# qcNPU/LifeLong-CLIP

Hardware: AMD Instinct MI355X
Metric: images/sec/GPU (ViT-B/16 fwd+bwd, bs=256) + online A_AUC on CIFAR-100 (higher is better)
Workload: dtype bf16

## Files before the change

### include/lc_clip.h

```cpp
#ifndef LC_CLIP_H
#define LC_CLIP_H
#include <hip/hip_runtime_api.h>
#include <stdint.h>

#ifdef __cplusplus
extern "C" {
#endif

#define LC_OK 0
#define LC_EINVAL (-1)
#define LC_ELAUNCH (-2)
#define LC_EUNSUPPORTED (-3)

#define LC_EPI_BF16 0
#define LC_EPI_F32 1
#define LC_EPI_RESID 2
#define LC_EPI_GELU 3
#define LC_EPI_GELU_BWD 4
#define LC_EPI_BF16_F32 5
#define LC_EPI_GELU_D 6
#define LC_EPI_MUL 7
#define LC_EPI_GELU_D_Q8 12
#define LC_EPI_MUL_Q8 13
#define LC_EPI_RESID16 14
// ... 133 lines not shown
                             long ldq, int row, const void* O_row, const void* dO_row, long ldo,
                             const float* lse_row, void* dqkv, long lddq, int causal);
int lc_attn_bwd_fp8(hipStream_t stream, int n_seq, int L, int H, const void* qkv, long ldq,
                    const void* O, const void* dO, long ldo, const float* lse, void* dqkv, long lddq,
                    void* q_scale, long q_rows, int causal);

int lc_train_transform(hipStream_t stream, int n, int C, int Hin, int Win, const float* x, int R,
                       int pad, int crop_i, int crop_j, int flip, const float* mean_host,
                       const float* std_host, int quantize, int layout, int patch, void* out);

int lc_autoaugment(hipStream_t stream, int n, int C, int H, int W, const float* x, float* out,
                   int n_ops, const int* codes, const float* params);

int lc_autoaugment_ws(hipStream_t stream, int n, int C, int H, int W, const float* x, float* out,
                      int n_ops, const int* codes, const float* params, void* ws, long ws_bytes);

int lc_cast_bf16(hipStream_t stream, long n, const float* src, void* dst);

int lc_merge_weight(hipStream_t stream, int N, int K, int r, const float* W, const float* A,
                    const float* B, float scaling, void* out, void* outT);

#define LC_CAST_MAX 64
int lc_cast_weights_bf16(hipStream_t stream, int n, const float* const* W, const int* N,
                         const int* K, void* const* out, void* const* outT);

int lc_merge_weights_bf16(hipStream_t stream, int n, const float* const* W, const float* const* A,
                          const float* const* B, const int* r, const float* scaling, const int* N,
                          const int* K, void* const* out, void* const* outT);

int lc_lora_grad(hipStream_t stream, int M, int N, int K, int r, const void* dY, long ldy,
                 const void* X, long ldx, const float* A, const float* B, float scaling,
                 float* dA, float* dB);

int lc_lora_grad_ws(hipStream_t stream, int M, int N, int K, int r, const void* dY, long ldy,
                    const void* X, long ldx, const void* apad, long lda, const void* btpad,
                    long ldbt, float scaling, float* dA, float* dB, void* ws, long ws_bytes);
int lc_lora_grad_ws_unscaled(hipStream_t stream, int M, int N, int K, int r, const void* dY,
                             long ldy, const void* X, long ldx, const void* apad, long lda,
                             const void* btpad, long ldbt, float scaling, float* dA, float* dB,
                             void* ws, long ws_bytes, const float* gscale);

int lc_adapter_fwd(hipStream_t stream, int M, int D, const void* z, long ldz, const void* Wd,
                   const float* bd, const void* Wu, const float* bu, float scale, float keep,
                   unsigned long long seed, const unsigned long long* seed_dev,
                   const float* resid, float* xout, long ldx, void* h);

int lc_adapter_ln_fwd(hipStream_t stream, int M, int D, const void* z, long ldz, const void* Wd,
                      const float* bd, const void* Wu, const float* bu, float scale, float keep,
                      unsigned long long seed, const unsigned long long* seed_dev,
                      const float* resid, float* xout, long ldx, void* hout,
                      const float* gamma, const float* beta, void* y, long ldy, float* mean,
                      float* rstd);

int lc_adapter_fwd_rows(hipStream_t stream, int M, int D, const void* z, long ldz, const void* Wd,
                        const float* bd, const void* Wu, const float* bu, float scale, float keep,
                        unsigned long long seed, const unsigned long long* seed_dev,
                        const float* resid, float* xout, long ldx, void* h, long row_mul,
                        long row_add);
int lc_adapter_ln_fwd_rows(hipStream_t stream, int M, int D, const void* z, long ldz,
                           const void* Wd, const float* bd, const void* Wu, const float* bu,
                           float scale, float keep, unsigned long long seed,
                           const unsigned long long* seed_dev, const float* resid, float* xout,
                           long ldx, void* hout, const float* gamma, const float* beta, void* y,
                           long ldy, float* mean, float* rstd, long row_mul, long row_add);
int lc_adapter_ln_fwd_rows_x16(hipStream_t stream, int M, int D, const void* z, long ldz,
                               const void* Wd, const float* bd, const void* Wu, const float* bu,
                               float scale, float keep, unsigned long long seed,
                               const unsigned long long* seed_dev, const void* resid, void* xout,
                               long ldx, void* hout, const float* gamma, const float* beta,
                               void* y, long ldy, float* mean, float* rstd, long row_mul,
                               long row_add);
int lc_adapter_fwd_rows_f16(hipStream_t stream, int M, int D, const void* z, long ldz,
                            const void* Wd, const float* bd, const void* Wu, const float* bu,
                            float scale, float keep, unsigned long long seed,
                            const unsigned long long* seed_dev, const float* resid, float* xout,
                            long ldx, void* h, long row_mul, long row_add);
int lc_adapter_ln_fwd_rows_f16(hipStream_t stream, int M, int D, const void* z, long ldz,
                               const void* Wd, const float* bd, const void* Wu, const float* bu,
                               float scale, float keep, unsigned long long seed,
                               const unsigned long long* seed_dev, const float* resid,
                               float* xout, long ldx, void* hout, const float* gamma,
                               const float* beta, void* y, long ldy, float* mean, float* rstd,
                               long row_mul, long row_add);

int lc_adapter_bwd(hipStream_t stream, int M, int D, const void* gout, long ldg, const void* h,
                   const void* WuT, const void* WdT, float scale, float keep, void* dpre,
                   void* dz, long ldz);

int lc_adapter_bwd_set_form(int fused);

int lc_adapter_wgrad(hipStream_t stream, int M, int D, const void* gout, long ldg, const void* h,
                     const void* z, long ldz, const void* dpre, float scale, float* dWu,
                     float* dbu, float* dWd, float* dbd);
int lc_adapter_wgrad_ws(hipStream_t stream, int M, int D, const void* gout, long ldg,
                        const void* h, const void* z, long ldz, const void* dpre, float scale,
                        float* dWu, float* dbu, float* dWd, float* dbd, void* ws, long ws_bytes);

int lc_check_finite(hipStream_t stream, long n, const float* g, int* flag);

int lc_adamw(hipStream_t stream, long n, float* p, const float* g, float* m, float* v, float lr,
             float b1, float b2, float eps, float wd, int step, const int* skip,
             const long long* step_dev);

int lc_counter_add(hipStream_t stream, int n, long long* ctr, long long delta);

int lc_adam_step_advance(hipStream_t stream, long long* ctr, const int* skip);

int lc_l2norm_rows(hipStream_t stream, int R, int E, const float* f, long ldf, float* out,
                   float* norms);

int lc_clip_head(hipStream_t stream, int B, int C, int E, const float* img_n, const float* txt_n,
                 const float* logit_scale, const int64_t* labels, float* probs, float* dlogits,
                 float* loss);

int lc_head_feat_grad(hipStream_t stream, int R, int Co, int E, const float* dlogits, long sr,
                      long sc, const float* other_n, const float* self_n, const float* norms,
                      const float* logit_scale, const float* dn_ext, float* dF);

int lc_head_logits(hipStream_t stream, int B, int C, int E, const float* img_n, const float* txt_n,
                   const float* logit_scale, float* logits, float* probs);

int lc_softmax_bwd_rows(hipStream_t stream, int B, int C, const float* probs, const float* dprobs,
                        float* dlogits);

int lc_grad_pow2_normalize(hipStream_t stream, long n, float* x, float* scale, int target_exp);

int lc_add_unscaled(hipStream_t stream, long n, float* y, const float* x, const float* scale);

int lc_device_cu_count(int device, int* n_cu);
int lc_stream_create_cumask(int device, int first, int count, int stride, void** stream);
int lc_stream_destroy(void* stream);

int lc_gemm_nt_f16(hipStream_t stream, int epi, int M, int N, int K, const void* A, long lda,
                   const void* B, long ldb, const float* bias, float alpha, void* out0, long ldo0,
                   void* out1, long ldo1, const void* aux, long ldaux);
int lc_gemm_nt_ws_f16(hipStream_t stream, int epi, int M, int N, int K, const void* A, long lda,
                      const void* B, long ldb, const float* bias, float alpha, void* out0, long ldo0,
                      void* out1, long ldo1, const void* aux, long ldaux, void* ws, long ws_bytes);
int lc_gemm_nt_rows_f16(hipStream_t stream, int epi, int n, int N, int K, const void* A, long lda,
                        const void* B, long ldb, const float* bias, float alpha, void* out,
                        long ldo, int M_full, long mul, long add, void* ws, long ws_bytes);
int lc_gemm_tn_f16(hipStream_t stream, int M, int N1, int N2, const void* A, long lda, const void* B,
                   long ldb, float alpha, float* C, long ldc, float* colsum, float colsum_scale);
int lc_gemm_tn_ws_f16(hipStream_t stream, int M, int N1, int N2, const void* A, long lda,
                      const void* B, long ldb, float alpha, float* C, long ldc, float* colsum,
                      float colsum_scale, void* ws, long ws_bytes);
int lc_gemm_set_tile_f16(int tile);
int lc_gemm_set_streamk_f16(int mode);
int lc_layernorm_fwd_f16(hipStream_t stream, int rows, int D, const float* x, long ldx,
                         const int* row_idx, const float* gamma, const float* beta, void* y,
                         int y_f32, long ldy, float* mean, float* rstd);
int lc_layernorm_bwd_f16(hipStream_t stream, int rows, int D, const void* dy, int dy_f32, long ldy,
                         const float* x, long ldx, const float* mean, const float* rstd,
                         const float* gamma, const float* dres, float* dx, void* dx_bf16, long ldo,
                         const int* row_idx);
int lc_attn_fwd_f16(hipStream_t stream, int n_seq, int L, int H, const void* qkv, long ldq, void* O,
                    long ldo, float* lse, int causal);
int lc_attn_bwd_f16(hipStream_t stream, int n_seq, int L, int H, const void* qkv, long ldq,
                    const void* O, const void* dO, long ldo, const float* lse, void* dqkv, long lddq,
                    int causal);
int lc_attn_bwd_set_form_f16(int form);
int lc_cast_bf16_f16(hipStream_t stream, long n, const float* src, void* dst);
int lc_merge_weight_f16(hipStream_t stream, int N, int K, int r, const float* W, const float* A,
                        const float* B, float scaling, void* out, void* outT);
int lc_cast_weights_bf16_f16(hipStream_t stream, int n, const float* const* W, const int* N,
                             const int* K, void* const* out, void* const* outT);
int lc_merge_weights_bf16_f16(hipStream_t stream, int n, const float* const* W, const float* const* A,
                              const float* const* B, const int* r, const float* scaling, const int* N,
                              const int* K, void* const* out, void* const* outT);
int lc_lora_grad_f16(hipStream_t stream, int M, int N, int K, int r, const void* dY, long ldy,
                     const void* X, long ldx, const float* A, const float* B, float scaling,
                     float* dA, float* dB);
int lc_lora_grad_ws_f16(hipStream_t stream, int M, int N, int K, int r, const void* dY, long ldy,
                        const void* X, long ldx, const void* apad, long lda, const void* btpad,
                        long ldbt, float scaling, float* dA, float* dB, void* ws, long ws_bytes);
int lc_adapter_fwd_f16(hipStream_t stream, int M, int D, const void* z, long ldz, const void* Wd,
                       const float* bd, const void* Wu, const float* bu, float scale, float keep,
                       unsigned long long seed, const unsigned long long* seed_dev,
                       const float* resid, float* xout, long ldx, void* h);
// ... 74 lines not shown
```

### lifelong-clip_amd/csrc/gemm.hip

```cpp
#include "lc_common.h"
#include <stdlib.h>
#include <type_traits>

namespace {

constexpr int BK = 64;

template <int... Es>
struct EpiList {};
template <int... Es>
constexpr bool epi_in(EpiList<Es...>, int epi) { return ((epi == Es) || ...); }
template <class F, int... Es>
int dispatch_epi(EpiList<Es...>, int epi, F&& f) {
  int rc = LC_EINVAL;
  (void)((epi == Es && (rc = f(std::integral_constant<int, Es>{}), true)) || ...);
  return rc;
}

LC_DEV int swz(int row, int chunk) { return chunk ^ ((row >> 1) & 7); }

LC_DEV void tile_coords(int tile, int tiles_m, int tiles_n, int gm, int& tm, int& tn) {
  if (gm <= 1) {
    tm = tile / tiles_n;
    tn = tile % tiles_n;
// ... 157 lines not shown
      ep.q_scale[fp8_scale_index(m, n >> 5, ep.q_rows)] = (uint8_t)byte;
    }
  };
  auto bfv = [](const uint32_t* x, int i) { return bf2f((i & 1) ? (x[i >> 1] >> 16) : (x[i >> 1] & 0xffff)); };
  auto hfv = [](const uint32_t* x, int i) { return h2f((i & 1) ? (x[i >> 1] >> 16) : (x[i >> 1] & 0xffff)); };
  if constexpr (AUXF || AUXB) prefetch(0, 0);
  uint64_t seed = ep.seed;
  if constexpr (EPI == EPI_AD_DOWN)
    if (ep.seed_dev) seed += *ep.seed_dev * 0xD1B54A32D192ED03ull;
  const long row_mul = ep.row_mul ? ep.row_mul : 1;
#pragma unroll
  for (int pass = 0; pass < WT_M / PASS; ++pass) {
#pragma unroll
    for (int ii = 0; ii < PASS / 16; ++ii)
#pragma unroll
      for (int j = 0; j < TN; ++j)
        *reinterpret_cast<f32x4*>(stg + (ii * 16 + (lane & 15)) * LSTR + j * 16 + (lane >> 4) * 4) =
            acc[pass * (PASS / 16) + ii][j];
    if constexpr (AUXF || AUXB)
      if (pass + 1 < WT_M / PASS) prefetch(pass + 1, (pass + 1) & 1);
#pragma unroll
    for (int it = 0; it < NIT; ++it) {
      const int lr = it * RPI + lane / LPR;
      const long m = m0 + wm * WT_M + pass * PASS + lr;
      float v[CPL];
#pragma unroll
      for (int q = 0; q < NQ; ++q) {
        const f32x4 a4 = *reinterpret_cast<const f32x4*>(stg + lr * LSTR + lc + 4 * q);
#pragma unroll
        for (int r = 0; r < 4; ++r) v[4 * q + r] = epi_affine(a4[r], alpha, bb[4 * q + r]);
      }
      const float* xf = pf_f[pass & 1][it];
      const uint32_t* xb = pf_b[pass & 1][it];
#if defined(G8_NOSTORE) && G8_NOSTORE == 2
      if (ep.dbg == nullptr) continue;
#endif
      float w[CPL];
      if constexpr (EPI == EPI_BF16 || EPI == EPI_BF16_F32) {
        store_bf(rs0, ldo0, m, v);
        if constexpr (EPI == EPI_BF16_F32) store_f(rs1, ldo1, m, v);
      } else if constexpr (EPI == EPI_F32) {
        store_f(rs0, ldo0, m, v);
      } else if constexpr (EPI == EPI_RESID) {
#pragma unroll
        for (int i = 0; i < CPL; ++i) w[i] = xf[i] + v[i];
        store_f(rs0, ldo0, m, w);
      } else if constexpr (EPI == EPI_RESID16) {
        static_assert(CPL == 8, "8 halves (16 B) per lane");
#pragma unroll
        for (int i = 0; i < CPL; ++i) w[i] = hfv(xb, i) + v[i];
        __builtin_amdgcn_raw_buffer_store_b128(
            lc_u32x4{pack2h(w[0], w[1]), pack2h(w[2], w[3]), pack2h(w[4], w[5]), pack2h(w[6], w[7])},
            rs0, (int)(((m - m0) * ldo0 + n) * 2), 0, 0);
      } else if constexpr (EPI == EPI_GELU) {
        store_bf(rs0, ldo0, m, v);
#pragma unroll
        for (int i = 0; i < CPL; ++i) w[i] = quick_gelu(v[i]);
        store_bf(rs1, ldo1, m, w);
      } else if constexpr (EPI == EPI_GELU_BWD) {
#pragma unroll
        for (int i = 0; i < CPL; ++i) w[i] = v[i] * quick_gelu_grad(bfv(xb, i));
        store_bf(rs0, ldo0, m, w);
      } else if constexpr (EPI == EPI_GELU_D || EPI == EPI_GELU_D_Q8) {
#pragma unroll
        for (int i = 0; i < CPL; ++i) {
          const float sg = lc_sigmoid1702(v[i]);
          w[i] = v[i] * sg;
          v[i] = sg * __builtin_fmaf(1.702f * v[i], 1.0f - sg, 1.0f);
        }
        store_bf(rs0, ldo0, m, v);
        if constexpr (EPI == EPI_GELU_D_Q8)
          store_q8(out1, ldo1, m, w);
        else
          store_bf(rs1, ldo1, m, w);
      } else if constexpr (EPI == EPI_MUL || EPI == EPI_MUL_Q8) {
#pragma unroll
        for (int i = 0; i < CPL; ++i) w[i] = v[i] * bfv(xb, i);
        if constexpr (EPI == EPI_MUL_Q8)
          store_q8(out1, ldo1, m, w);
        else
          store_bf(rs0, ldo0, m, w);
      } else if constexpr (EPI == EPI_AD_DOWN) {
#pragma unroll
        for (int i = 0; i < CPL; ++i) w[i] = fmaxf(v[i], 0.f) * drop_mul(seed, m * row_mul + ep.row_add, n + i, ep.keep);
        store_bf(rs0, ldo0, m, w);
      } else if constexpr (EPI == EPI_AD_UP) {
#pragma unroll
        for (int i = 0; i < CPL; ++i) w[i] = xf[i] + bfv(xb, i) + ep.scale * v[i];
        store_f(rs0, ldo0, m, w);
      } else if constexpr (EPI == EPI_AD_MASK) {
        const float inv = 1.0f / ep.keep;
#pragma unroll
        for (int i = 0; i < CPL; ++i) w[i] = bfv(xb, i) > 0.f ? v[i] * inv : 0.f;
        store_bf(rs0, ldo0, m, w);
      } else if constexpr (EPI == EPI_AD_ADD) {
#pragma unroll
        for (int i = 0; i < CPL; ++i) w[i] = bfv(xb, i) + v[i];
        store_bf(rs0, ldo0, m, w);
      }
    }
  }
}

template <int BM, int BN, int WM, int WN, int STAGES, int EPI>
__global__ void __launch_bounds__(64 * WM * WN, (WM * WN == 4 ? 2 : 1))
gemm_nt_kernel(int M, int N, int K, const bf16_t* __restrict__ A, long lda,
               const bf16_t* __restrict__ B, long ldb, const float* __restrict__ bias,
               float alpha, void* __restrict__ out0, long ldo0, void* __restrict__ out1,
               long ldo1, const void* __restrict__ aux, long ldaux, EpiParams ep) {
  constexpr int NW = WM * WN;
  constexpr int TM = BM / WM / 16;
  constexpr int TN = BN / WN / 16;
  constexpr int STAGE_BYTES = (BM + BN) * 128;
  constexpr int LOADS = (BM + BN) / 8 / NW;
  constexpr int PASS_MAX = STAGES == 1 ? 16 : 32;
  constexpr int EPI_BYTES = NW * ((BM / WM) % PASS_MAX == 0 ? PASS_MAX : 16) * (BN / WN + 4) * 4;
  constexpr int SMEM = STAGES * STAGE_BYTES > EPI_BYTES ? STAGES * STAGE_BYTES : EPI_BYTES;
  __shared__ __attribute__((aligned(16))) char smem[SMEM];

  const int tid = threadIdx.x, lane = tid & 63, wave = tid >> 6;
  const int wm = wave / WN, wn = wave % WN;

  const int tiles_n = N / BN;
  const int tiles_m = (M + BM - 1) / BM;
  const int nwg = tiles_m * tiles_n;
  int bid = blockIdx.x;
  {
    int q = nwg / 8, r = nwg % 8, x = bid % 8, loc = bid / 8;
    bid = (x < r ? x * (q + 1) : r * (q + 1) + (x - r) * q) + loc;
  }
  const int tm = bid / tiles_n, tn = bid % tiles_n;
  const int m0 = tm * BM, n0 = tn * BN;

  f32x4 acc[TM][TN];
#pragma unroll
  for (int i = 0; i < TM; ++i)
#pragma unroll
    for (int j = 0; j < TN; ++j) acc[i][j] = f32x4{0.f, 0.f, 0.f, 0.f};

  const int nk = K / BK;
  constexpr int IA = BM / 8 / NW, IB = BN / 8 / NW;
  static_assert(IA * 8 * NW == BM && IB * 8 * NW == BN, "tile rows must split evenly over the waves");
  const __amdgpu_buffer_rsrc_t rsA = lc_rsrc(A + (long)m0 * lda, (long)min(M - m0, BM) * lda * 2);
  const __amdgpu_buffer_rsrc_t rsB = lc_rsrc(B + (long)n0 * ldb, (long)BN * ldb * 2);
  auto stage = [&](int buf, int kt) {
    char* s = smem + buf * STAGE_BYTES;
#pragma unroll
    for (int i = 0; i < IA; ++i) {
      const int r = (wave * IA + i) * 8 + (lane >> 3);
      __builtin_amdgcn_raw_ptr_buffer_load_lds(rsA, LDS_PTR(s + (wave * IA + i) * 1024), 16,
                                               (uint32_t)(r * lda * 2 + swz(r, lane & 7) * 16),
                                               kt * BK * 2, 0, 0);
    }
#pragma unroll
    for (int i = 0; i < IB; ++i) {
      const int r = (wave * IB + i) * 8 + (lane >> 3);
      __builtin_amdgcn_raw_ptr_buffer_load_lds(rsB, LDS_PTR(s + BM * 128 + (wave * IB + i) * 1024),
                                               16, (uint32_t)(r * ldb * 2 + swz(r, lane & 7) * 16),
                                               kt * BK * 2, 0, 0);
    }
  };

  auto compute = [&](const char* sa) {
    const char* sb = sa + BM * 128;
#pragma unroll
    for (int ks = 0; ks < 2; ++ks) {
      const int chunk = ks * 4 + (lane >> 4);
// ... 899 lines not shown
    if (do_cs) {
      const bf16_t* col = reinterpret_cast<const bf16_t*>(sa) + (tid & 63);
#pragma unroll
      for (int i = 0; i < 16; ++i) cs += bf2f(col[((tid >> 6) + 4 * i) * 64]);
    }
    const int g = lane >> 4, t = lane & 15;
#pragma unroll
    for (int ks = 0; ks < 2; ++ks) {
      bf16x8 fa[2], fb[2];
#pragma unroll
      for (int i = 0; i < 2; ++i) {
        const int row = ks * 32 + g * 8 + (t >> 2);
        const int cola = wa * 32 + i * 16 + (t & 3) * 4;
        bf16x4 lo = tr_read(sa, row, cola), hi = tr_read(sa, row + 4, cola);
        fa[i] = bf16x8{lo[0], lo[1], lo[2], lo[3], hi[0], hi[1], hi[2], hi[3]};
        const int colb = wb * 32 + i * 16 + (t & 3) * 4;
        bf16x4 lo2 = tr_read(sb, row, colb), hi2 = tr_read(sb, row + 4, colb);
        fb[i] = bf16x8{lo2[0], lo2[1], lo2[2], lo2[3], hi2[0], hi2[1], hi2[2], hi2[3]};
      }
#pragma unroll
      for (int i = 0; i < 2; ++i)
#pragma unroll
        for (int j = 0; j < 2; ++j) acc[i][j] = mfma16(fa[i], fb[j], acc[i][j]);
    }
    asm volatile("s_waitcnt vmcnt(0)" ::: "memory");
    __syncthreads();
  }
  if (do_cs) {
    red[tid] = cs;
    __syncthreads();
    if (tid < 64 && c1 + tid < N1)
      atomicAdd(colsum + c1 + tid, colsum_scale * (red[tid] + red[tid + 64] + red[tid + 128] + red[tid + 192]));
  }
  const int g = lane >> 4, t = lane & 15;
#pragma unroll
  for (int i = 0; i < 2; ++i)
#pragma unroll
    for (int j = 0; j < 2; ++j)
#pragma unroll
      for (int r = 0; r < 4; ++r) {
        const int n1 = c1 + wa * 32 + i * 16 + g * 4 + r;
        const int n2 = c2 + wb * 32 + j * 16 + t;
        if (n1 < N1 && n2 < N2) atomicAdd(C + (long)n1 * ldc + n2, acc[i][j][r] * alpha);
      }
}

struct TnProb {
  const bf16_t* W;
  long ldw;
  const bf16_t* S;
  long lds;
  float* C;
  long ldc;
  int Nw, ns, trans;
  float alpha;
  float* cs_w;
  float cs_w_scale;
  float* cs_s;
  float cs_s_scale;
  int M, n_chunks, n_tiles, wgs;
  float* part;
  int pw;
  const float* div;
  int w16;
};
LC_DEV float tn_unscale(const TnProb& p, float v) { return p.div ? v / *p.div : v; }

template <int PW>
struct TnGeom {
  static constexpr int ROWB = PW * 2;
  static constexpr int WB = 64 * ROWB;
  static constexpr int SLOT = WB + 64 * 128;
#ifndef TNW256_STAGES
#define TNW256_STAGES 3
#endif
  static constexpr int STAGES = PW == 256 ? TNW256_STAGES : 5;
  static constexpr int WPW = WB / 1024 / 8;
  static constexpr int LOADS = WPW + 1;
  static constexpr int TI = PW / 64;
};

__host__ __device__ inline int tn_pslot(int pw) { return pw * 64 + pw + 64; }

template <int PW>
__global__ void __launch_bounds__(512, 1)
gemm_tn_wide_kernel(TnProb p0, TnProb p1) {
  using Geo = TnGeom<PW>;
  constexpr int STAGES = Geo::STAGES, SLOT = Geo::SLOT, LOADS = Geo::LOADS, TI = Geo::TI;
  constexpr int ROWB = Geo::ROWB, LPRW = ROWB / 16, RPP = 64 / LPRW;
  constexpr int PSLOT = PW * 64 + PW + 64;
  __shared__ __attribute__((aligned(16))) char smem[STAGES * SLOT];
  const bool second = (int)blockIdx.x >= p0.wgs;
  const TnProb& p = second ? p1 : p0;
  const int bid = second ? blockIdx.x - p0.wgs : blockIdx.x;
  const int tid = threadIdx.x, lane = tid & 63;
  const int wave = __builtin_amdgcn_readfirstlane(tid >> 6);
  const int wn = wave & 3, wsv = wave >> 2;
  const int g = lane >> 4, t = lane & 15;
  const int tile = bid % p.n_tiles, cidx = bid / p.n_tiles;
  const int nblk = (p.M + 63) / 64;
  float* slot = p.part ? p.part + (long)(tile * p.n_chunks + cidx) * PSLOT : nullptr;
  if (cidx >= nblk) {
    if (slot)
      for (int e = tid; e < PSLOT; e += 512) slot[e] = 0.f;
    return;
  }
  const int nsteps = (nblk - 1 - cidx) / p.n_chunks + 1;
  auto blk_row = [&](int s) { return (cidx + s * p.n_chunks) * 64; };
  const int nw_pad = (p.Nw + 63) & ~63;
  const bool do_csw = p.cs_w != nullptr && wsv == 0;
  const bool do_css = p.cs_s != nullptr && tile == 0 && wn == 0;

  auto dma = [&](int s) {
    char* sl = smem + (s % STAGES) * SLOT;
    const int r0 = blk_row(s);
#pragma unroll
    for (int i = 0; i < Geo::WPW; ++i) {
      const int piece = wave * Geo::WPW + i;
      const int lr = piece * RPP + lane / LPRW;
      const int pc = lane % LPRW;
      const int c = (((pc >> 1) ^ swz_w(lr)) << 1) | (pc & 1);
      const int r = min(r0 + lr, p.M - 1);
      int col = tile * PW + c * 8;
      col = col < nw_pad ? col : col - 64;
      glds16(p.W + (long)r * p.ldw + col, sl + piece * 1024);
    }
    {
      const int piece = wave;
      const int lr = piece * 8 + (lane >> 3);
      const int pc = lane & 7;
      const int c = (((pc >> 1) ^ swz_s(lr)) << 1) | (pc & 1);
      const int r = min(r0 + lr, p.M - 1);
      glds16(p.S + (long)r * p.lds + c * 8, sl + Geo::WB + piece * 1024);
    }
  };

  f32x4 acc[TI][2], csw[TI], css[2];
#pragma unroll
  for (int i = 0; i < TI; ++i) {
    csw[i] = f32x4{0.f, 0.f, 0.f, 0.f};
#pragma unroll
    for (int j = 0; j < 2; ++j) acc[i][j] = f32x4{0.f, 0.f, 0.f, 0.f};
  }
  css[0] = css[1] = f32x4{0.f, 0.f, 0.f, 0.f};
  const short one = LC_ONE16;

#pragma unroll
  for (int s = 0; s < STAGES - 1; ++s)
    if (s < nsteps) dma(s);
  for (int s = 0; s < nsteps; ++s) {
    const int ahead = min(nsteps - 1 - s, STAGES - 2);
    if (STAGES > 4 && ahead >= 3) wait_vmcnt<3 * LOADS>();
    else if (STAGES > 3 && ahead == 2) wait_vmcnt<2 * LOADS>();
    else if (ahead >= 1) wait_vmcnt<LOADS>();
    else wait_vmcnt<0>();
    lds_barrier();
    if (s + STAGES - 1 < nsteps) dma(s + STAGES - 1);
    const uint32_t sw = lds_addr(smem + (s % STAGES) * SLOT);
    const uint32_t ss = sw + Geo::WB;
    const int valid = p.M - blk_row(s);
    bf16x8 fwk[2][TI], fsk[2][2];
#pragma unroll
    for (int ks = 0; ks < 2; ++ks) {
      const int row = ks * 32 + g * 8 + (t >> 2);
#pragma unroll
      for (int i = 0; i < TI; ++i)
        fwk[ks][i] = tr_frag_asm<ROWB>(sw, row, wn * (PW / 4) + i * 16 + (t & 3) * 4);
#pragma unroll
      for (int j = 0; j < 2; ++j)
        fsk[ks][j] = tr_frag_asm<128>(ss, row, wsv * 32 + j * 16 + (t & 3) * 4);
    }
    lds_wait0();
    if (p.w16) {
#pragma unroll
      for (int ks = 0; ks < 2; ++ks)
#pragma unroll
        for (int i = 0; i < TI; ++i) fwk[ks][i] = h2s8(fwk[ks][i]);
    }
#pragma unroll
    for (int ks = 0; ks < 2; ++ks) {
      const int kb = ks * 32 + g * 8;
      bf16x8* fw = fwk[ks];
      bf16x8* fs = fsk[ks];
      bf16x8 ones;
#pragma unroll
      for (int e = 0; e < 8; ++e) ones[e] = (kb + e < valid) ? one : (short)0;
      if (valid < 64) {
#pragma unroll
        for (int j = 0; j < 2; ++j)
#pragma unroll
          for (int e = 0; e < 8; ++e) fs[j][e] = (kb + e < valid) ? fs[j][e] : (short)0;
      }
#pragma unroll
      for (int i = 0; i < TI; ++i) {
#pragma unroll
        for (int j = 0; j < 2; ++j) acc[i][j] = mfma16(fw[i], fs[j], acc[i][j]);
        if (do_csw) csw[i] = mfma16(fw[i], ones, csw[i]);
      }
      if (do_css) {
#pragma unroll
        for (int j = 0; j < 2; ++j) css[j] = mfma16(ones, fs[j], css[j]);
      }
    }
  }
  if (slot) {
#pragma unroll
    for (int i = 0; i < TI; ++i)
#pragma unroll
      for (int r = 0; r < 4; ++r) {
        const int nl = wn * (PW / 4) + i * 16 + g * 4 + r;
#pragma unroll
        for (int jj = 0; jj < 2; ++jj) slot[nl * 64 + wsv * 32 + jj * 16 + t] = acc[i][jj][r];
        if (wsv == 0 && t == 0) slot[PW * 64 + nl] = do_csw ? csw[i][r] : 0.f;
      }
    if (wn == 0 && g == 0)
#pragma unroll
// ... 7 lines not shown
    for (int r = 0; r < 4; ++r) {
      const int n = tile * PW + wn * (PW / 4) + i * 16 + g * 4 + r;
      if (n >= p.Nw) continue;
#pragma unroll
      for (int jj = 0; jj < 2; ++jj) {
        const int j = wsv * 32 + jj * 16 + t;
        if (j < p.ns) {
          float* dst = p.trans ? p.C + (long)j * p.ldc + n : p.C + (long)n * p.ldc + j;
          atomicAdd(dst, tn_unscale(p, acc[i][jj][r] * p.alpha));
        }
      }
      if (do_csw && t == 0) atomicAdd(p.cs_w + n, tn_unscale(p, csw[i][r] * p.cs_w_scale));
    }
  if (do_css && g == 0) {
#pragma unroll
    for (int jj = 0; jj < 2; ++jj) {
      const int j = wsv * 32 + jj * 16 + t;
      if (j < p.ns) atomicAdd(p.cs_s + j, tn_unscale(p, css[jj][0] * p.cs_s_scale));
    }
  }
}

LC_DEV float sum_slots(const float* __restrict__ src, int n, long ps) {
  float v = 0.f;
  int c = 0;
  for (; c + 8 <= n; c += 8) {
    float t[8];
#pragma unroll
    for (int i = 0; i < 8; ++i) t[i] = src[(c + i) * ps];
    v += ((t[0] + t[1]) + (t[2] + t[3])) + ((t[4] + t[5]) + (t[6] + t[7]));
  }
  for (; c < n; ++c) v += src[c * ps];
  return v;
}

__global__ void __launch_bounds__(256)
tn_reduce_kernel(TnProb p0, TnProb p1) {
  const int np0 = p0.Nw * 64 + p0.Nw + 64;
  const int np1 = p1.part ? p1.Nw * 64 + p1.Nw + 64 : 0;
  for (int e = blockIdx.x * 256 + threadIdx.x; e < np0 + np1; e += gridDim.x * 256) {
    const bool second = e >= np0;
    const TnProb& p = second ? p1 : p0;
    const int k = second ? e - np0 : e;
    const int pw = p.pw;
    const long ps = tn_pslot(pw);
    if (k < p.Nw * 64) {
      const int n = k / 64, j = k % 64;
      if (j >= p.ns) continue;
      const int tile = n / pw, nl = n % pw;
      const float v = sum_slots(p.part + (long)tile * p.n_chunks * ps + nl * 64 + j, p.n_chunks, ps);
      float* dst = p.trans ? p.C + (long)j * p.ldc + n : p.C + (long)n * p.ldc + j;
      *dst += tn_unscale(p, v * p.alpha);
    } else if (k < p.Nw * 64 + p.Nw) {
      if (!p.cs_w) continue;
      const int n = k - p.Nw * 64, tile = n / pw, nl = n % pw;
      const float v = sum_slots(p.part + (long)tile * p.n_chunks * ps + pw * 64 + nl, p.n_chunks, ps);
      p.cs_w[n] += tn_unscale(p, v * p.cs_w_scale);
    } else {
      const int j = k - p.Nw * 64 - p.Nw;
      if (!p.cs_s || j >= p.ns) continue;
      const float v = sum_slots(p.part + pw * 64 + pw + j, p.n_chunks, ps);
      p.cs_s[j] += tn_unscale(p, v * p.cs_s_scale);
    }
  }
}

int cu_count();

void plan_tn(TnProb& p, int total_panels) {
  static int walkers = -1;
  if (walkers < 0) {
    const char* e = lc_diag_env("LC_TN_WALKERS");
    walkers = e ? atoi(e) : 0;
  }
  const int cus = walkers > 0 ? walkers : cu_count();
  const int nblk = (p.M + 63) / 64;
  int chunks = cus / total_panels;
  chunks = chunks < 1 ? 1 : chunks;
  chunks = chunks > nblk / 4 ? (nblk / 4 > 0 ? nblk / 4 : 1) : chunks;
  p.n_chunks = chunks;
  p.wgs = p.n_tiles * chunks;
}

int launch_tn_wide(hipStream_t stream, const TnProb& a, const TnProb& b) {
  const dim3 grid(a.wgs + b.wgs), block(512);
  if (a.pw == 256) hipLaunchKernelGGL(gemm_tn_wide_kernel<256>, grid, block, 0, stream, a, b);
  else hipLaunchKernelGGL(gemm_tn_wide_kernel<128>, grid, block, 0, stream, a, b);
  if (a.part) {
    const int outs = a.Nw * 64 + a.Nw + 64 + (b.part ? b.Nw * 64 + b.Nw + 64 : 0);
    hipLaunchKernelGGL(tn_reduce_kernel, dim3((outs + 255) / 256), dim3(256), 0, stream, a, b);
  }
  LC_LAUNCH_RET();
}

template <class AT, class Kern, class... Tail>
int launch(Kern kern, int grid, int block, const GemmArgs& g, long es, const EpiParams& ep,
           const Tail&... tail) {
  hipLaunchKernelGGL(kern, dim3(grid), dim3(block), 0, g.stream, g.M, g.N, g.K,
                     static_cast<const AT*>(g.A), g.lda * es, static_cast<const AT*>(g.B),
                     g.ldb * es, g.bias, g.alpha, g.out0, g.ldo0, g.out1, g.ldo1, g.aux, g.ldaux,
                     ep, tail...);
  LC_LAUNCH_RET();
}

template <int BM, int BN, int WM, int WN, int STAGES>
int launch_nt(const GemmArgs& g) {
  const int tiles = ((g.M + BM - 1) / BM) * (g.N / BN);
  return dispatch_epi(NtEpis{}, g.epi, [&](auto E) {
    return launch<bf16_t>(gemm_nt_kernel<BM, BN, WM, WN, STAGES, E()>, tiles, 64 * WM * WN, g, 1,
                          g.ep);
  });
}

int g_split_mode = -1;

int cu_count() {
  static int cus[64] = {0};
  int dev = 0;
  if (hipGetDevice(&dev) != hipSuccess || dev < 0 || dev >= 64) return 256;
  if (cus[dev] == 0) {
    int n = 0;
    if (hipDeviceGetAttribute(&n, hipDeviceAttributeMultiprocessorCount, dev) != hipSuccess || n <= 0)
      n = 256;
    cus[dev] = n;
  }
  return cus[dev];
}

SplitK plan_split(int tiles, int units, int min_units, void* ws, long ws_bytes, int per_cu = 1,
                  long slab_floats = 256 * 256) {
  SplitK sk{tiles, 1, nullptr, nullptr};
  if (g_split_mode < 0) {
    const char* e = lc_diag_env("LC_GEMM_SPLITK");
    g_split_mode = e ? atoi(e) : 1;
  }
  if (!g_split_mode || ws == nullptr) return sk;
  const int cus = cu_count() * per_cu;
  const int rem = tiles % cus;
  if (tiles < cus || rem == 0 || rem > cus / 2) return sk;
  int S = cus / rem;
  S = S > 4 ? 4 : S;
  if (S > units / min_units) S = units / min_units;
  if (S < 2) return sk;
  const long tick_bytes = LC_SPLITK_TICKET_BYTES;
  if ((long)rem * 4 > tick_bytes || tick_bytes + (long)rem * S * slab_floats * 4 > ws_bytes) return sk;
  sk.dp_tiles = tiles - rem;
  sk.splits = S;
  sk.tickets = static_cast<int*>(ws);
  sk.slabs = reinterpret_cast<float*>(static_cast<char*>(ws) + tick_bytes);
  return sk;
}

int g_sk_mode = 0;
bool plan_sk(int tiles, int units, void* ws, long ws_bytes, SplitK& sk, int& G, int panels = 0) {
  G = panels > 0 ? panels : cu_count();
  if (panels > 0 && tiles % panels == 0 && ws != nullptr) {
    sk.dp_tiles = 0;
    sk.splits = 1;
    sk.tickets = static_cast<int*>(ws);
    sk.slabs = reinterpret_cast<float*>(static_cast<char*>(ws) + LC_SPLITK_TICKET_BYTES);
    return true;
  }
  if (ws == nullptr || tiles <= G || tiles % G == 0) return false;
  if ((long)tiles * units / G < units) return false;
  if ((long)(G - 1) * 4 > LC_SPLITK_TICKET_BYTES ||
      LC_SPLITK_TICKET_BYTES + (long)(G - 1) * 256 * 256 * 4 > ws_bytes)
    return false;
  sk.dp_tiles = 0;
  sk.splits = 1;
  sk.tickets = static_cast<int*>(ws);
// ... 364 lines not shown
             aux, ldaux, default_epi(), ws, ws_bytes,
             Fp8Scales{static_cast<const uint8_t*>(sa), static_cast<const uint8_t*>(sb), sa_rows,
                       sb_rows}};
  if (int rc = check_launch(g)) return rc;
  g.ep.q_scale = q8 ? static_cast<uint8_t*>(q_scale) : nullptr;
  g.ep.q_rows = q_rows;
  return launch_g8<true>(
      g, Route{PATH_G8, false, false, g8_plan<true>(M, N, K, ws, ws_bytes), group_m(N), 0});
}

int lc_gemm_set_tile(int tile) {
  LC_CHECK_ARG(tile >= 0 && tile <= 11);
  g_force_tile = tile;
  return LC_OK;
}

int lc_gemm_set_streamk(int mode) {
  LC_CHECK_ARG(mode >= 0 && mode <= 4);
  g_sk_mode = mode;
  return LC_OK;
}

int lc_gemm_tn(hipStream_t stream, int M, int N1, int N2, const void* A, long lda, const void* B,
               long ldb, float alpha, float* C, long ldc, float* colsum, float colsum_scale) {
  return lc_gemm_tn_ws(stream, M, N1, N2, A, lda, B, ldb, alpha, C, ldc, colsum, colsum_scale,
                       nullptr, 0);
}

int lc_gemm_tn_ws(hipStream_t stream, int M, int N1, int N2, const void* A, long lda,
                  const void* B, long ldb, float alpha, float* C, long ldc, float* colsum,
                  float colsum_scale, void* ws, long ws_bytes) {
  LC_CHECK_ARG(M > 0 && N1 > 0 && N2 > 0);
  LC_CHECK_ARG(lda % 8 == 0 && ldb % 8 == 0 && lda >= (N1 + 63) / 64 * 64 &&
               ldb >= (N2 + 63) / 64 * 64 && ldc >= N2);
  if (N1 <= 64 || N2 <= 64) {
    const bool a_wide = N2 <= 64;
    TnProb p{};
    p.W = static_cast<const bf16_t*>(a_wide ? A : B);
    p.ldw = a_wide ? lda : ldb;
    p.S = static_cast<const bf16_t*>(a_wide ? B : A);
    p.lds = a_wide ? ldb : lda;
    p.C = C;
    p.ldc = ldc;
    p.Nw = a_wide ? N1 : N2;
    p.ns = a_wide ? N2 : N1;
    p.trans = a_wide ? 0 : 1;
    p.alpha = alpha;
    p.cs_w = a_wide ? colsum : nullptr;
    p.cs_w_scale = colsum_scale;
    p.cs_s = a_wide ? nullptr : colsum;
    p.cs_s_scale = colsum_scale;
    p.M = M;
    const bool wide = ws != nullptr && p.Nw % 256 == 0;
    p.pw = wide ? 256 : 128;
    p.n_tiles = (p.Nw + p.pw - 1) / p.pw;
    plan_tn(p, p.n_tiles);
    if (wide && ws_bytes >= LC_SPLITK_TICKET_BYTES + (long)p.wgs * tn_pslot(p.pw) * 4)
      p.part = reinterpret_cast<float*>(static_cast<char*>(ws) + LC_SPLITK_TICKET_BYTES);
    return launch_tn_wide(stream, p, TnProb{});
  }
  const int tiles = ((N1 + 63) / 64) * ((N2 + 63) / 64);
  int splits = (1024 + tiles - 1) / tiles;
  int chunk = (M + splits - 1) / splits;
  chunk = ((chunk + 63) / 64) * 64;
  if (chunk < 256) chunk = 256;
  splits = (M + chunk - 1) / chunk;
  dim3 grid(tiles, splits), block(256);
  hipLaunchKernelGGL(gemm_tn_kernel, grid, block, 0, stream, M, N1, N2, chunk,
                     static_cast<const bf16_t*>(A), lda, static_cast<const bf16_t*>(B), ldb, alpha,
                     C, ldc, colsum, colsum_scale);
  LC_LAUNCH_RET();
}

int lc_adapter_wgrad(hipStream_t stream, int M, int D, const void* gout, long ldg, const void* h,
                     const void* z, long ldz, const void* dpre, float scale, float* dWu,
                     float* dbu, float* dWd, float* dbd) {
  return lc_adapter_wgrad_ws(stream, M, D, gout, ldg, h, z, ldz, dpre, scale, dWu, dbu, dWd, dbd,
                             nullptr, 0);
}

static int adapter_wgrad(hipStream_t stream, int M, int D, const void* gout, long ldg,
                         const void* h, const void* z, long ldz, const void* dpre, float scale,
                         float* dWu, float* dbu, float* dWd, float* dbd, void* ws, long ws_bytes,
                         const float* div, int g16 = 0) {
  LC_CHECK_ARG(M > 0 && D > 0 && D % 64 == 0 && ldg % 8 == 0 && ldz % 8 == 0 && ldg >= D &&
               ldz >= D);
  LC_CHECK_ARG(dWu != nullptr && dWd != nullptr);
  TnProb up{}, down{};
  up.div = down.div = div;
  up.W = static_cast<const bf16_t*>(gout);
  up.w16 = g16;
  up.ldw = ldg;
  up.S = static_cast<const bf16_t*>(h);
  up.lds = 64;
  up.C = dWu;
  up.ldc = 64;
  up.Nw = D;
  up.ns = 64;
  up.trans = 0;
  up.alpha = scale;
  up.cs_w = dbu;
  up.cs_w_scale = scale;
  const int pw = D % 256 == 0 ? 256 : 128;
  up.pw = pw;
  up.M = M;
  up.n_tiles = (D + pw - 1) / pw;
  down.W = static_cast<const bf16_t*>(z);
  down.ldw = ldz;
  down.S = static_cast<const bf16_t*>(dpre);
  down.lds = 64;
  down.C = dWd;
  down.ldc = D;
  down.Nw = D;
  down.ns = 64;
  down.trans = 1;
  down.alpha = 1.0f;
  down.cs_s = dbd;
  down.cs_s_scale = 1.0f;
  down.pw = pw;
  down.M = M;
  down.n_tiles = (D + pw - 1) / pw;
  plan_tn(up, 2 * up.n_tiles);
  plan_tn(down, 2 * down.n_tiles);
#ifdef LC_DIAG_SKIP_WGRAD
  return LC_OK;
#endif
  const long need = (long)(up.wgs + down.wgs) * tn_pslot(pw) * 4;
  if (ws != nullptr && ws_bytes >= LC_SPLITK_TICKET_BYTES + need) {
    up.part = reinterpret_cast<float*>(static_cast<char*>(ws) + LC_SPLITK_TICKET_BYTES);
    down.part = up.part + (long)up.wgs * tn_pslot(pw);
  }
  return launch_tn_wide(stream, up, down);
}

int lc_adapter_wgrad_ws(hipStream_t stream, int M, int D, const void* gout, long ldg,
                        const void* h, const void* z, long ldz, const void* dpre, float scale,
                        float* dWu, float* dbu, float* dWd, float* dbd, void* ws, long ws_bytes) {
  return adapter_wgrad(stream, M, D, gout, ldg, h, z, ldz, dpre, scale, dWu, dbu, dWd, dbd, ws,
                       ws_bytes, nullptr);
}

#ifndef LC_F16
int lc_adapter_wgrad_ws_unscaled(hipStream_t stream, int M, int D, const void* gout, long ldg,
                                 const void* h, const void* z, long ldz, const void* dpre,
                                 float scale, float* dWu, float* dbu, float* dWd, float* dbd,
                                 void* ws, long ws_bytes, const float* gscale) {
  LC_CHECK_ARG(gscale != nullptr);
  return adapter_wgrad(stream, M, D, gout, ldg, h, z, ldz, dpre, scale, dWu, dbu, dWd, dbd, ws,
                       ws_bytes, gscale);
}

int lc_adapter_wgrad_ws_unscaled_g16(hipStream_t stream, int M, int D, const void* gout, long ldg,
                                     const void* h, const void* z, long ldz, const void* dpre,
                                     float scale, float* dWu, float* dbu, float* dWd, float* dbd,
                                     void* ws, long ws_bytes, const float* gscale) {
  LC_CHECK_ARG(gscale != nullptr);
  return adapter_wgrad(stream, M, D, gout, ldg, h, z, ldz, dpre, scale, dWu, dbu, dWd, dbd, ws,
                       ws_bytes, gscale, 1);
}
#endif

}
```

### lifelong-clip_amd/csrc/lc_common.h

```cpp
#pragma once
#include <hip/hip_runtime.h>
#include <stdint.h>
#include <stdlib.h>
#include "lc_clip.h"

inline const char* lc_diag_env(const char* name) {
#ifdef LC_DIAG_ENV
  return getenv(name);
#else
  (void)name;
  return nullptr;
#endif
}

typedef uint16_t bf16_t;
typedef short bf16x8 __attribute__((ext_vector_type(8)));
typedef short bf16x4 __attribute__((ext_vector_type(4)));
typedef float f32x4 __attribute__((ext_vector_type(4)));
typedef int i32x4 __attribute__((ext_vector_type(4)));
typedef int i32x8 __attribute__((ext_vector_type(8)));

__device__ __forceinline__ void st_nt16(void* p, uint32_t a, uint32_t b, uint32_t c, uint32_t d) {
  __builtin_nontemporal_store(i32x4{(int)a, (int)b, (int)c, (int)d}, reinterpret_cast<i32x4*>(p));
}
// ... 30 lines not shown
  __bf16 b = (__bf16)f;
  return *reinterpret_cast<bf16_t*>(&b);
}
typedef __bf16 lc_bf16x2 __attribute__((ext_vector_type(2)));
LC_DEV uint32_t pack2bf(float lo, float hi) {
  return __builtin_bit_cast(uint32_t, __builtin_convertvector((lc_f32x2){lo, hi}, lc_bf16x2));
}

LC_DEV f32x4 mfma16(const bf16x8& a, const bf16x8& b, const f32x4& c) {
  return __builtin_amdgcn_mfma_f32_16x16x32_bf16(a, b, c, 0, 0, 0);
}
#define LC_MFMA16_ASM "v_mfma_f32_16x16x32_bf16"
#define LC_ONE16 ((short)0x3F80)
#endif

typedef _Float16 lc_h16x2 __attribute__((ext_vector_type(2)));
typedef _Float16 lc_h16x4 __attribute__((ext_vector_type(4)));
LC_DEV float h2f(uint16_t h) { return (float)__builtin_bit_cast(_Float16, h); }
LC_DEV uint32_t pack2h(float lo, float hi) {
  return __builtin_bit_cast(uint32_t, __builtin_convertvector((lc_f32x2){lo, hi}, lc_h16x2));
}
template <typename XT>
LC_DEV float xround(float v) {
  if constexpr (sizeof(XT) == 2) return (float)(_Float16)v;
  else return v;
}

LC_DEV void glds16(const void* gsrc, void* lds_wave_base) {
  __builtin_amdgcn_global_load_lds(GLB_PTR(gsrc), LDS_PTR(lds_wave_base), 16, 0, 0);
}
LC_DEV void glds4(const void* gsrc, void* lds_wave_base) {
  __builtin_amdgcn_global_load_lds(GLB_PTR(gsrc), LDS_PTR(lds_wave_base), 4, 0, 0);
}

LC_DEV float wave_sum(float v) {
#pragma unroll
  for (int o = 32; o > 0; o >>= 1) v += __shfl_xor(v, o);
  return v;
}
LC_DEV float wave_max(float v) {
#pragma unroll
  for (int o = 32; o > 0; o >>= 1) v = fmaxf(v, __shfl_xor(v, o));
  return v;
}

constexpr float LC_GELU_K2 = -1.702f * 1.4426950408889634f;
LC_DEV float lc_sigmoid1702(float x) {
  return __builtin_amdgcn_rcpf(1.0f + __builtin_amdgcn_exp2f(LC_GELU_K2 * x));
}
LC_DEV float quick_gelu(float x) { return x * lc_sigmoid1702(x); }
LC_DEV float quick_gelu_grad(float x) {
  const float s = lc_sigmoid1702(x);
  const float t = 1.702f * x;
  return s * __builtin_fmaf(t, 1.0f - s, 1.0f);
}

LC_DEV uint32_t lc_hash(uint64_t seed, uint64_t idx) {
  uint64_t z = seed + 0x9E3779B97F4A7C15ull * (idx + 1);
  z = (z ^ (z >> 30)) * 0xBF58476D1CE4E5B9ull;
  z = (z ^ (z >> 27)) * 0x94D049BB133111EBull;
  z ^= z >> 31;
  return (uint32_t)(z >> 32);
}

LC_DEV float drop_mul(uint64_t seed, long m, int j, float keep) {
  if (keep >= 1.0f) return 1.0f;
  const uint32_t hsh = lc_hash(seed, (uint64_t)m * 64 + j);
  const float u = (hsh >> 8) * (1.0f / 16777216.0f);
  return u < keep ? 1.0f / keep : 0.0f;
}

struct EpiParams {
  const void* aux2;
  long ldaux2;
  float scale;
  float keep;
  uint64_t seed;
  unsigned long long* dbg;
  const unsigned long long* seed_dev;
  uint8_t* q_scale;
  long q_rows;
  int group_m;
  long row_mul, row_add;
};

struct Fp8Scales {
  const uint8_t* sa;
  const uint8_t* sb;
  long sa_rows, sb_rows;
};

LC_DEV uint32_t lc_amax_bits(uint32_t acc, float x) {
  const uint32_t b = __float_as_uint(x) & 0x7fffffffu;
  return acc > b ? acc : b;
}
LC_DEV uint32_t e8m0_of_bits(uint32_t amax_bits) {
  const int e = (int)(amax_bits >> 23);
  if (e == 0) return 0;
  if (e == 255) return 0xFF;
  const int b = e - 8;
  return (uint32_t)(b < 1 ? 1 : (b > 253 ? 253 : b));
}
LC_DEV uint32_t e8m0_of(float amax) { return e8m0_of_bits(__float_as_uint(amax) & 0x7fffffffu); }
LC_DEV float e8m0_inv(uint32_t byte) {
  if (byte == 0) return 0.f;
  if (byte == 0xFF) return __uint_as_float(0x7fc00000u);
  return __uint_as_float((uint32_t)(254 - byte) << 23);
}
LC_DEV uint32_t pack4_fp8(float a, float b, float c, float d) {
  const bool nan = (__float_as_uint(a) & 0x7fffffffu) > 0x7f800000u;
  a = fminf(fmaxf(a, -448.f), 448.f);
  b = fminf(fmaxf(b, -448.f), 448.f);
  c = fminf(fmaxf(c, -448.f), 448.f);
  d = fminf(fmaxf(d, -448.f), 448.f);
  uint32_t r = __builtin_amdgcn_cvt_pk_fp8_f32(a, b, 0, false);
  r = __builtin_amdgcn_cvt_pk_fp8_f32(c, d, r, true);
  return nan ? 0x7f7f7f7fu : r;
}

LC_DEV int swz_w(int r) { return (r & 3) | ((r >> 1) & 4); }
LC_DEV int swz_s(int r) { return ((r >> 1) & 1) | ((r >> 2) & 2); }

template <int ROWB>
LC_DEV bf16x8 tr_frag(const char* lds, int row, int col) {
  auto addr = [&](int r) {
    const int byte = col * 2;
    const int u = (byte >> 5) ^ (ROWB >= 256 ? swz_w(r) : swz_s(r));
    return lds + r * ROWB + u * 32 + (byte & 31);
  };
  const bf16x4 lo = __builtin_amdgcn_ds_read_tr16_b64_v4i16(
      (__attribute__((address_space(3))) bf16x4*)addr(row));
  const bf16x4 hi = __builtin_amdgcn_ds_read_tr16_b64_v4i16(
      (__attribute__((address_space(3))) bf16x4*)addr(row + 4));
  return bf16x8{lo[0], lo[1], lo[2], lo[3], hi[0], hi[1], hi[2], hi[3]};
}

LC_DEV __amdgpu_buffer_rsrc_t lc_rsrc(const void* p, long bytes) {
  const uint64_t a = (uint64_t)p;
  const uint32_t lo = __builtin_amdgcn_readfirstlane((uint32_t)a);
  const uint32_t hi = __builtin_amdgcn_readfirstlane((uint32_t)(a >> 32));
  const int n = __builtin_amdgcn_readfirstlane((int)bytes);
  return __builtin_amdgcn_make_buffer_rsrc((void*)(((uint64_t)hi << 32) | lo), 0, n, 0x00020000);
}
typedef unsigned int lc_u32x4 __attribute__((ext_vector_type(4)));
typedef unsigned int lc_u32x2 __attribute__((ext_vector_type(2)));

LC_DEV bf16x8 h2s8(bf16x8 v) {
#ifdef LC_F16
  return v;
#else
  const lc_u32x4 u = __builtin_bit_cast(lc_u32x4, v);
  const lc_f32x2 f0 = __builtin_convertvector(__builtin_bit_cast(lc_h16x2, (uint32_t)u.x), lc_f32x2);
  const lc_f32x2 f1 = __builtin_convertvector(__builtin_bit_cast(lc_h16x2, (uint32_t)u.y), lc_f32x2);
  const lc_f32x2 f2 = __builtin_convertvector(__builtin_bit_cast(lc_h16x2, (uint32_t)u.z), lc_f32x2);
  const lc_f32x2 f3 = __builtin_convertvector(__builtin_bit_cast(lc_h16x2, (uint32_t)u.w), lc_f32x2);
  return __builtin_bit_cast(bf16x8, (lc_u32x4{pack2bf(f0.x, f0.y), pack2bf(f1.x, f1.y),
                                              pack2bf(f2.x, f2.y), pack2bf(f3.x, f3.y)}));
#endif
}
LC_DEV bf16x8 b2h8(bf16x8 v) {
  const lc_u32x4 u = __builtin_bit_cast(lc_u32x4, v);
  auto cv = [](uint32_t w) {
    return pack2h(__uint_as_float(w << 16), __uint_as_float(w & 0xffff0000u));
  };
  return __builtin_bit_cast(bf16x8, (lc_u32x4{cv(u.x), cv(u.y), cv(u.z), cv(u.w)}));
}
LC_DEV f32x4 mfma16_h(const bf16x8& a, const bf16x8& b, const f32x4& c) {
// ... 85 lines not shown
```

### lifelong-clip_amd/csrc/lc_f16_names.h

```cpp
#pragma once
#define lc_attn_fwd lc_attn_fwd_f16
#define lc_attn_bwd_fp8 lc_attn_bwd_fp8_f16
#define lc_attn_bwd lc_attn_bwd_f16
#define lc_attn_bwd_set_form lc_attn_bwd_set_form_f16
#define lc_attn_row_fwd lc_attn_row_fwd_f16
#define lc_attn_row_bwd lc_attn_row_bwd_f16
#define lc_attn_bwd_live_row lc_attn_bwd_live_row_f16
#define lc_gemm_nt_ex lc_gemm_nt_ex_f16
#define lc_gemm_nt lc_gemm_nt_f16
#define lc_gemm_nt_ws lc_gemm_nt_ws_f16
#define lc_gemm_nt_rows lc_gemm_nt_rows_f16
#define lc_gemm_split_plan lc_gemm_split_plan_f16
#define lc_gemm_set_debug lc_gemm_set_debug_f16
#define lc_gemm_nt_fp8 lc_gemm_nt_fp8_f16
#define lc_gemm_set_tile lc_gemm_set_tile_f16
#define lc_gemm_set_streamk lc_gemm_set_streamk_f16
#define lc_gemm_tn lc_gemm_tn_f16
#define lc_gemm_tn_ws lc_gemm_tn_ws_f16
#define lc_adapter_wgrad lc_adapter_wgrad_f16
#define lc_adapter_wgrad_ws lc_adapter_wgrad_ws_f16
#define lc_layernorm_fwd lc_layernorm_fwd_f16
#define lc_layernorm_fwd_fp8 lc_layernorm_fwd_fp8_f16
#define lc_layernorm_bwd lc_layernorm_bwd_f16
#define lc_layernorm_bwd_fp8 lc_layernorm_bwd_fp8_f16
#define lc_patchify lc_patchify_f16
#define lc_vit_assemble lc_vit_assemble_f16
#define lc_vit_embed_ln lc_vit_embed_ln_f16
#define lc_text_embed lc_text_embed_f16
#define lc_eot_rows lc_eot_rows_f16
#define lc_cast_bf16 lc_cast_bf16_f16
#define lc_merge_weight lc_merge_weight_f16
#define lc_cast_weights_bf16 lc_cast_weights_bf16_f16
#define lc_merge_weights_bf16 lc_merge_weights_bf16_f16
#define lc_lora_grad lc_lora_grad_f16
#define lc_lora_grad_ws lc_lora_grad_ws_f16
#define lc_adapter_fwd lc_adapter_fwd_f16
#define lc_adapter_ln_fwd lc_adapter_ln_fwd_f16
#define lc_adapter_fwd_rows lc_adapter_fwd_rows_f16
#define lc_adapter_ln_fwd_rows lc_adapter_ln_fwd_rows_f16
#define lc_adapter_bwd_set_form lc_adapter_bwd_set_form_f16
#define lc_adapter_bwd lc_adapter_bwd_f16
#define lc_check_finite lc_check_finite_f16
#define lc_adamw lc_adamw_f16
#define lc_counter_add lc_counter_add_f16
#define lc_adam_step_advance lc_adam_step_advance_f16
```

### lifelong-clip_amd/csrc/peft.hip

```cpp
#include "lc_common.h"
#include <stdlib.h>

namespace {

__global__ void cast_bf16_kernel(long n, const float* __restrict__ src, bf16_t* __restrict__ dst) {
  for (long i = (blockIdx.x * (long)blockDim.x + threadIdx.x) * 4; i < n;
       i += (long)gridDim.x * blockDim.x * 4) {
    if (i + 3 < n) {
      const float4 v = *reinterpret_cast<const float4*>(src + i);
      *reinterpret_cast<uint2*>(dst + i) = uint2{pack2bf(v.x, v.y), pack2bf(v.z, v.w)};
    } else {
      for (long j = i; j < n; ++j) dst[j] = f2bf(src[j]);
    }
  }
}

constexpr int MERGE_RMAX = 8;
LC_DEV void merge_tile(int N, int K, int r, const float* __restrict__ W, const float* __restrict__ A,
                       const float* __restrict__ B, float s, bf16_t* __restrict__ out,
                       bf16_t* __restrict__ outT, int n0, int k0) {
  __shared__ float tile[64][65];
  __shared__ float As[MERGE_RMAX][64];
  __shared__ float Bs[64][MERGE_RMAX];
  const int tid = threadIdx.x;
// ... 686 lines not shown
  float* slot_p = part + (long)cidx * ((long)N * r + (long)r * K);
  if (t < r) {
#pragma unroll
    for (int c = 0; c < NC; ++c)
#pragma unroll
      for (int rr = 0; rr < 4; ++rr)
        slot_p[(c * 128 + wave * 16 + 4 * g + rr) * r + t] = accB[c][rr];
  }
#pragma unroll
  for (int j = 0; j < G::DAT; ++j)
#pragma unroll
    for (int rr = 0; rr < 4; ++rr)
      if (4 * g + rr < r)
        slot_p[(long)N * r + (4 * g + rr) * K + (wave * G::DAT + j) * 16 + t] = accA[j][rr];
}

__global__ void __launch_bounds__(256)
lora_reduce_kernel(const float* __restrict__ part, int walkers, long slot_floats, long nb,
                   float s, float* __restrict__ dA, float* __restrict__ dB,
                   const float* __restrict__ div) {
  __shared__ float red[8][33];
  const int lo = threadIdx.x & 31, wg = threadIdx.x >> 5;
  const long e = (long)blockIdx.x * 32 + lo;
  float v = 0.f;
  if (e < slot_floats) {
    int w = wg;
    for (; w + 56 < walkers; w += 64) {
      float q[8];
#pragma unroll
      for (int u = 0; u < 8; ++u) q[u] = part[(long)(w + 8 * u) * slot_floats + e];
      v += ((q[0] + q[1]) + (q[2] + q[3])) + ((q[4] + q[5]) + (q[6] + q[7]));
    }
    for (; w < walkers; w += 8) v += part[(long)w * slot_floats + e];
  }
  red[wg][lo] = v;
  __syncthreads();
  if (wg == 0 && e < slot_floats) {
    float tot = 0.f;
#pragma unroll
    for (int k = 0; k < 8; ++k) tot += red[k][lo];
    if (div) tot /= *div;
    if (e < nb) dB[e] += s * tot;
    else dA[e - nb] += s * tot;
  }
}


template <int D, int XB = 4>
struct AdLnLay {
  static constexpr int ZROW = D * 2;
  static constexpr int ZIMG = 16 * ZROW;
  static constexpr int ZP = ZIMG / 1024 / 8;
  static constexpr int XIMG = 16 * D * XB;
  static constexpr int XP = XIMG / 1024 / 8;
  static constexpr int Z_OFF = 0;
  static constexpr int X_OFF = ZIMG;
  static constexpr int PRM_OFF = X_OFF + 2 * XIMG;
  static constexpr int ST_OFF = PRM_OFF + (3 * D + 64) * 4;
  static constexpr int RED_OFF = ST_OFF + 2 * 8 * 16 * 4;
  static constexpr int H_OFF = RED_OFF + 16 * 64 * 4;
  static constexpr int YSTR = D * 2 + 16;
  static constexpr int Y_OFF = RED_OFF;
  static constexpr int BYTES = RED_OFF + (16 * YSTR > 16 * 64 * 6 ? 16 * YSTR : 16 * 64 * 6);
  static constexpr int KS = D / 32 / 2;
  static constexpr int NU = D / 8 / 16;
  static_assert(BYTES <= 160 * 1024, "LDS");
};

template <int N>
LC_DEV void vmcnt_le() {
  asm volatile("s_waitcnt vmcnt(%0)" ::"n"(N) : "memory");
}

template <int D, typename XT = float>
__global__ void __launch_bounds__(512, 1)
adapter_ln_fwd_kernel(int M, const bf16_t* __restrict__ z, long ldz, const bf16_t* __restrict__ Wd,
                      const float* __restrict__ bd, const bf16_t* __restrict__ Wu,
                      const float* __restrict__ bu, float scale, float keep, uint64_t seed,
                      const unsigned long long* __restrict__ seed_dev,
                      const XT* __restrict__ resid, XT* __restrict__ xout, long ldx,
                      bf16_t* __restrict__ hout, const float* __restrict__ gamma,
                      const float* __restrict__ beta, bf16_t* __restrict__ y, long ldy,
                      float* __restrict__ mean_out, float* __restrict__ rstd_out, long row_mul,
                      long row_add) {
  constexpr int XB = (int)sizeof(XT);
  using L = AdLnLay<D, XB>;
  constexpr int KS = L::KS, NU = L::NU;
  __shared__ __attribute__((aligned(16))) char smem[L::BYTES];
  const int tid = threadIdx.x, lane = tid & 63;
  const int wave = __builtin_amdgcn_readfirstlane(tid >> 6);
  const int g = lane >> 4, t = lane & 15;
  const int nd = wave & 3, kh = wave >> 2;
  const int nblk = (M + 15) / 16;
  if ((int)blockIdx.x >= nblk) return;
  if (seed_dev) seed += *seed_dev * 0xD1B54A32D192ED03ull;
  float* red = reinterpret_cast<float*>(smem + L::RED_OFF);
  bf16_t* hs = reinterpret_cast<bf16_t*>(smem + L::H_OFF);
  float* st = reinterpret_cast<float*>(smem + L::ST_OFF);
  float* prm = reinterpret_cast<float*>(smem + L::PRM_OFF);
  for (int e = tid; e < D; e += 512) {
    prm[e] = bu[e];
    prm[D + e] = gamma[e];
    prm[2 * D + e] = beta[e];
  }
  if (tid < 64) prm[3 * D + tid] = bd[tid];
  bf16x8 wdf[KS], wuf[NU][2];
#pragma unroll
  for (int k = 0; k < KS; ++k)
    asm volatile("global_load_dwordx4 %0, %1, off"
                 : "=v"(wdf[k])
                 : "v"(Wd + (long)(16 * nd + t) * D + (kh * KS + k) * 32 + 8 * g));
#pragma unroll
  for (int u = 0; u < NU; ++u)
#pragma unroll
    for (int k = 0; k < 2; ++k)
      asm volatile("global_load_dwordx4 %0, %1, off"
                   : "=v"(wuf[u][k])
                   : "v"(Wu + (long)(wave * (D / 8) + 16 * u + t) * 64 + 32 * k + 8 * g));
  asm volatile("s_waitcnt vmcnt(0)" ::: "memory");

  auto dma_z = [&](int b) {
    char* dst = smem + L::Z_OFF;
    const int r0 = b * 16;
#pragma unroll
    for (int pp = 0; pp < L::ZP; ++pp) {
      const int piece = wave * L::ZP + pp;
      const int idx = piece * 64 + lane;
      const int row = idx / (L::ZROW / 16), pc = idx % (L::ZROW / 16);
      const int c = (((pc >> 1) ^ swz_w(row)) << 1) | (pc & 1);
      const int m = min(r0 + row, M - 1);
      glds16(z + (long)m * ldz + c * 8, dst + piece * 1024);
    }
  };
  constexpr int EPC = 16 / XB;
  auto dma_x = [&](int b, int buf) {
    char* dst = smem + L::X_OFF + buf * L::XIMG;
#pragma unroll
    for (int pp = 0; pp < L::XP; ++pp) {
      const int piece = wave * L::XP + pp;
      const int idx = piece * 64 + lane;
      const int row = idx / (D / EPC), c = idx % (D / EPC);
      const int m = min(b * 16 + row, M - 1);
      glds16(resid + (long)m * ldx + c * EPC, dst + piece * 1024);
    }
  };
  const uint32_t lds0 = lds_addr(smem);
  auto zaddr = [&](int row, int byte) {
    const int u = (byte >> 5) ^ swz_w(row);
    return lds0 + L::Z_OFF + row * L::ZROW + u * 32 + (byte & 31);
  };
  constexpr int XPR = D * XB / 512;
#ifdef ADLN_KO
  constexpr int NST = ((ADLN_KO & 1) ? 0 : XPR) + ((ADLN_KO & 2) ? 0 : D / 256);
#else
  constexpr int NST = XPR + D / 256;
#endif
  const int tail = NST + (wave < 2 ? 1 : 0) + (wave == 0 ? 2 : 0);

  int b = blockIdx.x;
  dma_x(b, 0);
  dma_z(b);
  __syncthreads();
  bool prev_full = false;
#pragma unroll 1
  for (int k = 0; b < nblk; ++k, b += gridDim.x) {
    const int buf = k & 1;
    const int r0 = b * 16;
    if (prev_full) {
      if (tail == NST + 3) vmcnt_le<NST + 3>();
      else if (tail == NST + 1) vmcnt_le<NST + 1>();
      else vmcnt_le<NST>();
    } else {
      vmcnt_le<0>();
    }
    lds_barrier();
    const int bn = b + gridDim.x;
    if (bn < nblk) dma_x(bn, buf ^ 1);
    f32x4 pd = f32x4{0.f, 0.f, 0.f, 0.f};
    uint2 zz[NU];
    {
      constexpr int GK = KS / 2;
      bf16x8 za[KS];
#pragma unroll
      for (int ks = 0; ks < KS; ++ks)
        asm volatile("ds_read_b128 %0, %1"
                     : "=v"(za[ks]) : "v"(zaddr(t, ((kh * KS + ks) * 32 + 8 * g) * 2)));
#pragma unroll
      for (int u = 0; u < NU; ++u)
        asm volatile("ds_read_b64 %0, %1"
                     : "=v"(zz[u]) : "v"(zaddr(t, (wave * (D / 8) + 16 * u + 4 * g) * 2)));
      asm volatile("s_waitcnt lgkmcnt(%0)" ::"n"(NU + KS - GK) : "memory");
      __builtin_amdgcn_sched_barrier(0);
#pragma unroll
      for (int ks = 0; ks < GK; ++ks) pd = mfma16(za[ks], wdf[ks], pd);
      asm volatile("s_waitcnt lgkmcnt(%0)" ::"n"(NU) : "memory");
      __builtin_amdgcn_sched_barrier(0);
#pragma unroll
      for (int ks = GK; ks < KS; ++ks) pd = mfma16(za[ks], wdf[ks], pd);
    }
    if (kh == 1)
#pragma unroll
      for (int rr = 0; rr < 4; ++rr) red[(4 * g + rr) * 64 + 16 * nd + t] = pd[rr];
    lds_barrier();
    if (bn < nblk) dma_z(bn);
    if (kh == 0) {
      const int j = 16 * nd + t;
#pragma unroll
      for (int rr = 0; rr < 4; ++rr) {
        const int m = 4 * g + rr;
        float v = pd[rr] + red[m * 64 + j];
        v = fmaxf(v + prm[3 * D + j], 0.f) * drop_mul(seed, (long)(r0 + m) * row_mul + row_add, j, keep);
        hs[m * 64 + j] = f2bf(v);
      }
    }
    lds_barrier();
    const uint32_t hl = lds0 + L::H_OFF;
    if (wave < 2) {
      const int e = tid;
      uint4 v;
      asm volatile("ds_read_b128 %0, %1" : "=v"(v) : "v"(hl + e * 16));
      lds_wait0();
      if (r0 + (e >> 3) < M) *reinterpret_cast<uint4*>(hout + (long)r0 * 64 + e * 8) = v;
    }
    bf16x8 ha0, ha1;
    asm volatile("ds_read_b128 %0, %1" : "=v"(ha0) : "v"(hl + (t * 64 + 8 * g) * 2));
    asm volatile("ds_read_b128 %0, %1" : "=v"(ha1) : "v"(hl + (t * 64 + 32 + 8 * g) * 2));
    f32x4 xo[NU];
    float s1 = 0.f;
    f32x4 xr4[NU];
    uint2 xh4[NU];
#pragma unroll
    for (int u = 0; u < NU; ++u) {
      const int col = wave * (D / 8) + 16 * u + 4 * g;
      if constexpr (XB == 4)
        asm volatile("ds_read_b128 %0, %1"
                     : "=v"(xr4[u]) : "v"(lds0 + L::X_OFF + buf * L::XIMG + (t * D + col) * 4));
      else
        asm volatile("ds_read_b64 %0, %1"
                     : "=v"(xh4[u]) : "v"(lds0 + L::X_OFF + buf * L::XIMG + (t * D + col) * 2));
    }
    lds_wait0();
    if constexpr (XB == 2) {
#pragma unroll
      for (int u = 0; u < NU; ++u)
        xr4[u] = f32x4{h2f(xh4[u].x & 0xffff), h2f(xh4[u].x >> 16), h2f(xh4[u].y & 0xffff),
                       h2f(xh4[u].y >> 16)};
    }
#pragma unroll
    for (int u = 0; u < NU; ++u) {
      f32x4 acc = mfma16(wuf[u][0], ha0, f32x4{0.f, 0.f, 0.f, 0.f});
      acc = mfma16(wuf[u][1], ha1, acc);
      const int col = wave * (D / 8) + 16 * u + 4 * g;
      const float zf[4] = {bf2f(zz[u].x & 0xffff), bf2f(zz[u].x >> 16), bf2f(zz[u].y & 0xffff),
                           bf2f(zz[u].y >> 16)};
      const f32x4 xr = xr4[u];
#pragma unroll
      for (int rr = 0; rr < 4; ++rr) {
        const float v = acc[rr] + prm[col + rr];
        xo[u][rr] = xround<XT>(xr[rr] + zf[rr] + scale * v);
        s1 += xo[u][rr];
      }
    }
    s1 += __shfl_xor(s1, 16);
    s1 += __shfl_xor(s1, 32);
    if (g == 0) st[wave * 16 + t] = s1;
    lds_barrier();
    const bool live = r0 + t < M;
    const uint32_t xs = lds0 + L::X_OFF + buf * L::XIMG;
    const uint32_t ys = lds0 + L::Y_OFF;
    if constexpr (XB == 4) {
      static_assert((D / 32) % 8 == 0, "wave column block must be whole 128-B groups");
      const uint32_t xb = xs + t * D * 4 + wave * (D / 32) * 16;
      const uint32_t x0 = xb + ((g ^ t) & 7) * 16, x1 = xb + (((4 + g) ^ t) & 7) * 16 - 64;
#pragma unroll
      for (int u = 0; u < NU; ++u)
        asm volatile("ds_write_b128 %0, %1 offset:%2" ::"v"((u & 1) ? x1 : x0), "v"(xo[u]),
                     "n"(u * 64) : "memory");
    } else {
      const uint32_t xb = xs + t * D * 2 + (g & 1) * 8;
#pragma unroll
      for (int u = 0; u < NU; ++u) {
        const int c = wave * (D / 64) + 2 * u + (g >> 1);
        const uint32_t a = xb + ((c & ~7) | ((c ^ t) & 7)) * 16;
        asm volatile("ds_write_b64 %0, %1" ::"v"(a),
                     "v"(uint2{pack2h(xo[u][0], xo[u][1]), pack2h(xo[u][2], xo[u][3])}) : "memory");
      }
    }
    float mean = 0.f;
#pragma unroll
    for (int w = 0; w < 8; ++w) mean += st[w * 16 + t];
    mean *= 1.0f / D;
    float s2 = 0.f;
#pragma unroll
    for (int u = 0; u < NU; ++u)
// ... 129 lines not shown
    b.out[i] = static_cast<bf16_t*>(out[i]);
    b.outT[i] = static_cast<bf16_t*>(outT[i]);
    b.N[i] = N[i];
    b.K[i] = K[i];
    const int t = ((N[i] + 63) / 64) * ((K[i] + 63) / 64);
    tiles = t > tiles ? t : tiles;
  }
  hipLaunchKernelGGL(cast_batch_kernel, dim3(tiles, n), dim3(256), 0, st, b);
  LC_LAUNCH_RET();
}

int lc_lora_grad(hipStream_t st, int M, int N, int K, int r, const void* dY, long ldy,
                 const void* X, long ldx, const float* A, const float* B, float scaling,
                 float* dA, float* dB) {
  LC_CHECK_ARG(M > 0 && r == 4 && N <= 3072 && K <= 1024 && N > 0 && K > 0);
  const int groups = (M + 15) / 16;
  const int grid = groups < 512 ? groups : 512;
  if (N <= 1024)
    hipLaunchKernelGGL((lora_grad_kernel<4, 1024, 1024>), dim3(grid), dim3(256), 0, st, M, N, K,
                       (const bf16_t*)dY, ldy, (const bf16_t*)X, ldx, A, B, scaling, dA, dB);
  else
    hipLaunchKernelGGL((lora_grad_kernel<4, 3072, 1024>), dim3(grid), dim3(256), 0, st, M, N, K,
                       (const bf16_t*)dY, ldy, (const bf16_t*)X, ldx, A, B, scaling, dA, dB);
  LC_LAUNCH_RET();
}

static int lora_grad_ws(hipStream_t st, int M, int N, int K, int r, const void* dY, long ldy,
                        const void* X, long ldx, const void* apad, long lda, const void* btpad,
                        long ldbt, float scaling, float* dA, float* dB, void* ws, long ws_bytes,
                        const float* div) {
  LC_CHECK_ARG(M > 0 && r >= 1 && r <= 4 && dY && X && apad && btpad && dA && dB && ws);
  LC_CHECK_ARG(ldy % 8 == 0 && ldx % 8 == 0 && lda % 8 == 0 && ldbt % 8 == 0);
  LC_CHECK_ARG(ldy >= N && ldx >= K && lda >= K && ldbt >= N);
  const int nblk = (M + 31) / 32;
  int walkers = 0;
  {
    int dev = 0, cus = 256;
    if (hipGetDevice(&dev) != hipSuccess ||
        hipDeviceGetAttribute(&cus, hipDeviceAttributeMultiprocessorCount, dev) != hipSuccess)
      cus = 256;
    walkers = nblk < cus ? nblk : cus;
  }
  const long slot = (long)N * r + (long)r * K;
  LC_CHECK_ARG(ws_bytes >= LC_SPLITK_TICKET_BYTES + (long)walkers * slot * 4);
  float* part = reinterpret_cast<float*>(static_cast<char*>(ws) + LC_SPLITK_TICKET_BYTES);
#define LC_LG(KT, NC)                                                                           \
  if (K == KT * 32 && N == NC * 128) {                                                         \
    hipLaunchKernelGGL((lora_grad1p_kernel<KT, NC>), dim3(walkers), dim3(512), 0, st, M,        \
                       (const bf16_t*)X, ldx, (const bf16_t*)dY, ldy, (const bf16_t*)apad, lda, \
                       (const bf16_t*)btpad, ldbt, part, walkers, r);                          \
  } else
  LC_LG(24, 18) LC_LG(24, 6) LC_LG(16, 12) LC_LG(16, 4)
  { return LC_EINVAL; }
#undef LC_LG
  hipError_t e = hipGetLastError();
  if (e != hipSuccess) return LC_ELAUNCH;
  hipLaunchKernelGGL(lora_reduce_kernel, dim3((unsigned)((slot + 31) / 32)), dim3(256), 0, st,
                     part, walkers, slot, (long)N * r, scaling, dA, dB, div);
  LC_LAUNCH_RET();
}

int lc_lora_grad_ws(hipStream_t st, int M, int N, int K, int r, const void* dY, long ldy,
                    const void* X, long ldx, const void* apad, long lda, const void* btpad,
                    long ldbt, float scaling, float* dA, float* dB, void* ws, long ws_bytes) {
  return lora_grad_ws(st, M, N, K, r, dY, ldy, X, ldx, apad, lda, btpad, ldbt, scaling, dA, dB, ws,
                      ws_bytes, nullptr);
}

#ifndef LC_F16
int lc_lora_grad_ws_unscaled(hipStream_t st, int M, int N, int K, int r, const void* dY, long ldy,
                             const void* X, long ldx, const void* apad, long lda,
                             const void* btpad, long ldbt, float scaling, float* dA, float* dB,
                             void* ws, long ws_bytes, const float* gscale) {
  LC_CHECK_ARG(gscale != nullptr);
  return lora_grad_ws(st, M, N, K, r, dY, ldy, X, ldx, apad, lda, btpad, ldbt, scaling, dA, dB, ws,
                      ws_bytes, gscale);
}
#endif

static int adapter_fwd(hipStream_t st, int M, int D, const void* z, long ldz, const void* Wd,
                       const float* bd, const void* Wu, const float* bu, float scale, float keep,
                       unsigned long long seed, const unsigned long long* seed_dev,
                       const float* resid, float* xout, long ldx, void* hout, long row_mul,
                       long row_add) {
  LC_CHECK_ARG(M > 0 && D % 64 == 0 && ldz % 8 == 0 && ldx % 4 == 0);
  LC_CHECK_ARG(keep > 0.f && keep <= 1.f && row_mul >= 1 && row_add >= 0);
  EpiParams ep{z, ldz, scale, keep, (uint64_t)seed, nullptr, seed_dev};
  ep.row_mul = row_mul;
  ep.row_add = row_add;
  int rc = lc_gemm_nt_ex({st, EPI_AD_DOWN, M, AD_H, D, z, ldz, Wd, D, bd, 1.0f, hout, AD_H,
                          nullptr, 0, nullptr, 0, ep});
  if (rc) return rc;
  return lc_gemm_nt_ex({st, EPI_AD_UP, M, D, AD_H, hout, AD_H, Wu, AD_H, bu, 1.0f, xout, ldx,
                        nullptr, 0, resid, ldx, ep});
}

int lc_adapter_fwd(hipStream_t st, int M, int D, const void* z, long ldz, const void* Wd,
                   const float* bd, const void* Wu, const float* bu, float scale, float keep,
                   unsigned long long seed, const unsigned long long* seed_dev,
                   const float* resid, float* xout, long ldx, void* hout) {
  return adapter_fwd(st, M, D, z, ldz, Wd, bd, Wu, bu, scale, keep, seed, seed_dev, resid, xout,
                     ldx, hout, 1, 0);
}

int lc_adapter_fwd_rows(hipStream_t st, int M, int D, const void* z, long ldz, const void* Wd,
                        const float* bd, const void* Wu, const float* bu, float scale, float keep,
                        unsigned long long seed, const unsigned long long* seed_dev,
                        const float* resid, float* xout, long ldx, void* hout, long row_mul,
                        long row_add) {
  return adapter_fwd(st, M, D, z, ldz, Wd, bd, Wu, bu, scale, keep, seed, seed_dev, resid, xout,
                     ldx, hout, row_mul, row_add);
}

static int adapter_ln_fwd(hipStream_t st, int M, int D, const void* z, long ldz, const void* Wd,
                          const float* bd, const void* Wu, const float* bu, float scale,
                          float keep, unsigned long long seed,
                          const unsigned long long* seed_dev, const void* resid, void* xout,
                          long ldx, void* hout, const float* gamma, const float* beta, void* y,
                          long ldy, float* mean, float* rstd, int x16, long row_mul = 1,
                          long row_add = 0) {
  const int xb = x16 ? 2 : 4;
  LC_CHECK_ARG(row_mul >= 1 && row_add >= 0);
  LC_CHECK_ARG(M > 0 && (D == 768 || D == 512) && ldz % 8 == 0 && ldx % (16 / xb) == 0 &&
               ldy % 8 == 0);
  LC_CHECK_ARG(ldx < (1L << 24) && ldy < (1L << 24));
  LC_CHECK_ARG(((uintptr_t)xout & 15) == 0 && ((uintptr_t)y & 15) == 0 &&
               ((uintptr_t)resid & 15) == 0);
  LC_CHECK_ARG(ldz >= D && ldx >= D && ldy >= D && keep > 0.f && keep <= 1.f);
  LC_CHECK_ARG(z && Wd && bd && Wu && bu && resid && xout && hout && gamma && beta && y && mean && rstd);
  int dev = 0, cus = 256;
  if (hipGetDevice(&dev) != hipSuccess ||
      hipDeviceGetAttribute(&cus, hipDeviceAttributeMultiprocessorCount, dev) != hipSuccess)
    cus = 256;
  const int nblk = (M + 15) / 16;
  const int grid = nblk < cus ? nblk : cus;
#define LC_ALN(DD, XT)                                                                           \
  hipLaunchKernelGGL((adapter_ln_fwd_kernel<DD, XT>), dim3(grid), dim3(512), 0, st, M,           \
                     (const bf16_t*)z, ldz, (const bf16_t*)Wd, bd, (const bf16_t*)Wu, bu, scale,  \
                     keep, (uint64_t)seed, seed_dev, (const XT*)resid, (XT*)xout, ldx,           \
                     (bf16_t*)hout, gamma, beta, (bf16_t*)y, ldy, mean, rstd, row_mul, row_add)
  if (x16) {
    if (D == 768) LC_ALN(768, _Float16);
    else LC_ALN(512, _Float16);
  } else {
    if (D == 768) LC_ALN(768, float);
    else LC_ALN(512, float);
  }
#undef LC_ALN
  LC_LAUNCH_RET();
}

int lc_adapter_ln_fwd(hipStream_t st, int M, int D, const void* z, long ldz, const void* Wd,
                      const float* bd, const void* Wu, const float* bu, float scale, float keep,
                      unsigned long long seed, const unsigned long long* seed_dev,
                      const float* resid, float* xout, long ldx, void* hout,
                      const float* gamma, const float* beta, void* y, long ldy, float* mean,
                      float* rstd) {
  return adapter_ln_fwd(st, M, D, z, ldz, Wd, bd, Wu, bu, scale, keep, seed, seed_dev, resid, xout,
                        ldx, hout, gamma, beta, y, ldy, mean, rstd, 0);
}

int lc_adapter_ln_fwd_rows(hipStream_t st, int M, int D, const void* z, long ldz, const void* Wd,
                           const float* bd, const void* Wu, const float* bu, float scale,
                           float keep, unsigned long long seed,
                           const unsigned long long* seed_dev, const float* resid, float* xout,
                           long ldx, void* hout, const float* gamma, const float* beta, void* y,
                           long ldy, float* mean, float* rstd, long row_mul, long row_add) {
  return adapter_ln_fwd(st, M, D, z, ldz, Wd, bd, Wu, bu, scale, keep, seed, seed_dev, resid, xout,
                        ldx, hout, gamma, beta, y, ldy, mean, rstd, 0, row_mul, row_add);
}

#ifndef LC_F16
int lc_adapter_ln_fwd_rows_x16(hipStream_t st, int M, int D, const void* z, long ldz,
                               const void* Wd, const float* bd, const void* Wu, const float* bu,
                               float scale, float keep, unsigned long long seed,
                               const unsigned long long* seed_dev, const void* resid, void* xout,
                               long ldx, void* hout, const float* gamma, const float* beta,
                               void* y, long ldy, float* mean, float* rstd, long row_mul,
                               long row_add) {
  return adapter_ln_fwd(st, M, D, z, ldz, Wd, bd, Wu, bu, scale, keep, seed, seed_dev, resid, xout,
                        ldx, hout, gamma, beta, y, ldy, mean, rstd, 1, row_mul, row_add);
}

int lc_adapter_ln_fwd_x16(hipStream_t st, int M, int D, const void* z, long ldz, const void* Wd,
                          const float* bd, const void* Wu, const float* bu, float scale,
                          float keep, unsigned long long seed,
                          const unsigned long long* seed_dev, const void* resid, void* xout,
                          long ldx, void* hout, const float* gamma, const float* beta, void* y,
                          long ldy, float* mean, float* rstd) {
  return adapter_ln_fwd(st, M, D, z, ldz, Wd, bd, Wu, bu, scale, keep, seed, seed_dev, resid, xout,
                        ldx, hout, gamma, beta, y, ldy, mean, rstd, 1);
}
#endif

static int g_adapter_bwd_fused = 1;

int lc_adapter_bwd_set_form(int fused) {
  g_adapter_bwd_fused = fused != 0;
  return LC_OK;
}

#ifndef LC_F16
int lc_adapter_bwd_g16(hipStream_t st, int M, int D, const void* gout, long ldg, const void* h,
                       const void* WuT, const void* WdT, float scale, float keep, void* dpre,
                       void* dz, long ldz) {
  LC_CHECK_ARG(M > 0 && (D == 768 || D == 512) && ldg % 8 == 0 && ldz % 8 == 0);
  LC_CHECK_ARG(keep > 0.f && keep <= 1.f);
  LC_CHECK_ARG(((uintptr_t)gout & 15) == 0 && ((uintptr_t)h & 15) == 0 &&
               ((uintptr_t)WuT & 15) == 0 && ((uintptr_t)WdT & 15) == 0 &&
               (dz == nullptr || ((uintptr_t)dz & 15) == 0));
  const int nb = (M + AD_R - 1) / AD_R;
  const dim3 grid(nb < ad_cu_count() ? nb : ad_cu_count()), block(64 * AD_NW);
  auto G = static_cast<const bf16_t*>(gout);
  auto H = static_cast<const bf16_t*>(h);
  auto U = static_cast<const bf16_t*>(WuT);
  auto Wd = static_cast<const bf16_t*>(WdT);
  auto P = static_cast<bf16_t*>(dpre);
  auto Z = static_cast<bf16_t*>(dz);
#define LC_ADB(ND, DZ)                                                                            \
  hipLaunchKernelGGL((adapter_bwd_fused_kernel<ND, DZ, true>), grid, block, 0, st, M, G, ldg, H,  \
                     U, Wd, scale, keep, P, Z, ldz)
  if (D == 768) {
    if (dz) LC_ADB(12, true);
    else LC_ADB(12, false);
  } else {
    if (dz) LC_ADB(8, true);
    else LC_ADB(8, false);
  }
#undef LC_ADB
  LC_LAUNCH_RET();
}
#endif

int lc_adapter_bwd(hipStream_t st, int M, int D, const void* gout, long ldg, const void* h,
                   const void* WuT, const void* WdT, float scale, float keep, void* dpre,
                   void* dz, long ldz) {
  LC_CHECK_ARG(M > 0 && D % 64 == 0 && ldg % 8 == 0 && ldz % 8 == 0);
  LC_CHECK_ARG(keep > 0.f && keep <= 1.f);
  const bool fused = g_adapter_bwd_fused != 0;
  if (fused && dz != nullptr && (D == 768 || D == 512) && M >= 1024 && ((uintptr_t)gout & 15) == 0 &&
      ((uintptr_t)h & 15) == 0 && ((uintptr_t)WuT & 15) == 0 && ((uintptr_t)WdT & 15) == 0) {
    const int nb = (M + AD_R - 1) / AD_R;
    const dim3 grid(nb < ad_cu_count() ? nb : ad_cu_count()), block(64 * AD_NW);
    auto G = static_cast<const bf16_t*>(gout);
    auto H = static_cast<const bf16_t*>(h);
    auto U = static_cast<const bf16_t*>(WuT);
    auto Wd = static_cast<const bf16_t*>(WdT);
    auto P = static_cast<bf16_t*>(dpre);
    auto Z = static_cast<bf16_t*>(dz);
#define LC_ADB(ND, DZ)                                                                            \
  hipLaunchKernelGGL((adapter_bwd_fused_kernel<ND, DZ>), grid, block, 0, st, M, G, ldg, H, U, Wd, \
                     scale, keep, P, Z, ldz)
    if (D == 768) LC_ADB(12, true);
    else LC_ADB(8, true);
#undef LC_ADB
    LC_LAUNCH_RET();
  }
  EpiParams ep{nullptr, 0, scale, keep, 0, nullptr};
  int rc = lc_gemm_nt_ex({st, EPI_AD_MASK, M, AD_H, D, gout, ldg, WuT, D, nullptr, scale, dpre,
                          AD_H, nullptr, 0, h, AD_H, ep});
  if (rc) return rc;
  if (dz == nullptr) return LC_OK;
  return lc_gemm_nt_ex({st, EPI_AD_ADD, M, D, AD_H, dpre, AD_H, WdT, AD_H, nullptr, 1.0f, dz,
                        ldz, nullptr, 0, gout, ldg, ep});
// ... 35 lines not shown
```

### lifelong-clip_amd/lcclip/_lib.py

```python
from __future__ import annotations

import ctypes
import os
from ctypes import c_float, c_int, c_long, c_ulonglong, c_void_p

import torch

_HERE = os.path.dirname(os.path.abspath(__file__))
LIB_PATH = os.path.join(_HERE, "liblcclip.so")

P = c_void_p
SIGNATURES = {
    "lc_gemm_nt": [P, c_int, c_int, c_int, c_int, P, c_long, P, c_long, P, c_float, P, c_long, P,
                   c_long, P, c_long],
    "lc_gemm_nt_ws": [P, c_int, c_int, c_int, c_int, P, c_long, P, c_long, P, c_float, P, c_long,
                      P, c_long, P, c_long, P, c_long],
    "lc_gemm_nt_rows": [P, c_int, c_int, c_int, c_int, P, c_long, P, c_long, P, c_float, P, c_long,
                        c_int, c_long, c_long, P, c_long],
    "lc_gemm_split_plan": [c_int, c_int, c_int, c_long, P, P],
    "lc_gemm_nt_fp8": [P, c_int, c_int, c_int, c_int, P, c_long, P, c_long, P, c_long, P, c_long,
                       P, c_float, P, c_long, P, c_long, P, c_long, P, c_long, P, c_long],
    "lc_quant_fp8": [P, c_long, c_int, P, c_int, c_long, c_long, P, c_long, P, c_long],
    "lc_gemm_set_tile": [c_int],
    "lc_gemm_set_streamk": [c_int],
    "lc_gemm_set_debug": [P],
    "lc_adapter_bwd_set_form": [c_int],
    "lc_attn_bwd_set_form": [c_int],
    "lc_gemm_tn": [P, c_int, c_int, c_int, P, c_long, P, c_long, c_float, P, c_long, P, c_float],
    "lc_gemm_tn_ws": [P, c_int, c_int, c_int, P, c_long, P, c_long, c_float, P, c_long, P, c_float,
                      P, c_long],
    "lc_layernorm_fwd": [P, c_int, c_int, P, c_long, P, P, P, P, c_int, c_long, P, P],
    "lc_layernorm_fwd_fp8": [P, c_int, c_int, P, c_long, P, P, P, P, c_long, P, P, P, c_long, P,
                             c_long],
    "lc_layernorm_bwd": [P, c_int, c_int, P, c_int, c_long, P, c_long, P, P, P, P, P, P, c_long, P],
    "lc_layernorm_bwd_fp8": [P, c_int, c_int, P, c_int, c_long, P, c_long, P, P, P, P, P, P, c_long,
                             P, P, c_long, P, c_long],
    "lc_patchify": [P, c_int, c_int, c_int, P, P],
    "lc_vit_assemble": [P, c_int, c_int, c_int, P, P, P, P],
    "lc_vit_embed_ln": [P, c_int, c_int, c_int, P, P, P, P, P, P, P, P, P, P, P],
    "lc_text_embed": [P, c_int, c_int, c_int, P, P, P, P],
    "lc_eot_rows": [P, c_int, c_int, P, P],
    "lc_attn_fwd": [P, c_int, c_int, c_int, P, c_long, P, c_long, P, c_int],
    "lc_attn_bwd": [P, c_int, c_int, c_int, P, c_long, P, P, c_long, P, P, c_long, c_int],
    "lc_attn_row_fwd": [P, c_int, c_int, c_int, P, c_long, c_int, P, c_long, P, c_int],
    "lc_attn_row_bwd": [P, c_int, c_int, c_int, P, c_long, c_int, P, P, c_long, P, P, c_long, c_int],
    "lc_attn_bwd_live_row": [P, c_int, c_int, c_int, P, c_long, c_int, P, P, c_long, P, P, c_long,
                             c_int],
    "lc_attn_bwd_fp8": [P, c_int, c_int, c_int, P, c_long, P, P, c_long, P, P, c_long, P, c_long,
                        c_int],
    "lc_train_transform": [P, c_int, c_int, c_int, c_int, P, c_int, c_int, c_int, c_int, c_int, P,
                           P, c_int, c_int, c_int, P],
    "lc_autoaugment": [P, c_int, c_int, c_int, c_int, P, P, c_int, P, P],
    "lc_autoaugment_ws": [P, c_int, c_int, c_int, c_int, P, P, c_int, P, P, P, c_long],
    "lc_cast_bf16": [P, c_long, P, P],
    "lc_merge_weight": [P, c_int, c_int, c_int, P, P, P, c_float, P, P],
    "lc_cast_weights_bf16": [P, c_int, P, P, P, P, P],
    "lc_merge_weights_bf16": [P, c_int, P, P, P, P, P, P, P, P, P],
    "lc_lora_grad": [P, c_int, c_int, c_int, c_int, P, c_long, P, c_long, P, P, c_float, P, P],
    "lc_lora_grad_ws": [P, c_int, c_int, c_int, c_int, P, c_long, P, c_long, P, c_long, P, c_long,
                        c_float, P, P, P, c_long],
    "lc_adapter_fwd": [P, c_int, c_int, P, c_long, P, P, P, P, c_float, c_float, c_ulonglong, P, P,
                       P, c_long, P],
    "lc_adapter_ln_fwd": [P, c_int, c_int, P, c_long, P, P, P, P, c_float, c_float, c_ulonglong,
                          P, P, P, c_long, P, P, P, P, c_long, P, P],
    "lc_adapter_fwd_rows": [P, c_int, c_int, P, c_long, P, P, P, P, c_float, c_float, c_ulonglong,
                            P, P, P, c_long, P, c_long, c_long],
    "lc_adapter_ln_fwd_rows": [P, c_int, c_int, P, c_long, P, P, P, P, c_float, c_float,
                               c_ulonglong, P, P, P, c_long, P, P, P, P, c_long, P, P, c_long,
                               c_long],
    "lc_adapter_bwd": [P, c_int, c_int, P, c_long, P, P, P, c_float, c_float, P, P, c_long],
    "lc_adapter_wgrad": [P, c_int, c_int, P, c_long, P, P, c_long, P, c_float, P, P, P, P],
    "lc_adapter_wgrad_ws": [P, c_int, c_int, P, c_long, P, P, c_long, P, c_float, P, P, P, P, P,
                            c_long],
    "lc_check_finite": [P, c_long, P, P],
    "lc_adamw": [P, c_long, P, P, P, P, c_float, c_float, c_float, c_float, c_float, c_int, P, P],
    "lc_counter_add": [P, c_int, P, c_long],
    "lc_adam_step_advance": [P, P, P],
    "lc_l2norm_rows": [P, c_int, c_int, P, c_long, P, P],
    "lc_clip_head": [P, c_int, c_int, c_int, P, P, P, P, P, P, P],
    "lc_head_logits": [P, c_int, c_int, c_int, P, P, P, P, P],
    "lc_softmax_bwd_rows": [P, c_int, c_int, P, P, P],
    "lc_head_feat_grad": [P, c_int, c_int, c_int, P, c_long, c_long, P, P, P, P, P, P],
    "lc_grad_pow2_normalize": [P, c_long, P, P, c_int],
    "lc_add_unscaled": [P, c_long, P, P, P],
    "lc_mvp_select": [P, c_int, c_int, c_int, c_int, P, c_long, P, c_long, P, P, P, P, P, P],
    "lc_mvp_simloss": [P, c_int, c_int, c_int, c_int, c_int, P, c_long, P, P, P, P, P, P, P, P, P],
    "lc_mvp_simloss_bwd": [P, c_int, c_int, c_int, c_int, c_int, P, c_long, P, c_long, P, P, P, P,
                           P, P, P, P, P, P, c_long],
    "lc_pool_gather": [P, c_int, c_int, c_int, c_long, P, c_long, P, P, c_int],
    "lc_pool_gather_bwd": [P, c_int, c_int, c_int, c_long, P, P, c_long, c_int, c_float, P, c_long,
                           P, c_long],
    "lc_mvp_head_fwd": [P, c_int, c_int, c_int, P, P, P, P, c_long, P, P, P, P, P, P, P],
    "lc_mvp_loss_mean": [P, c_int, P, P, c_float, c_float, P, P, P],
    "lc_mvp_score_g": [P, c_int, c_int, c_int, P, P, P, P, c_long, P, P, c_float, P],
    "lc_mvp_score": [P, c_int, c_int, c_int, P, P, P, P, P, c_long, P, P, c_float, c_float, P, P,
                     P],
    "lc_mvp_afs": [P, c_int, c_int, P, P, P, P, P],
    "lc_mvp_head_bwd": [P, c_int, c_int, c_int, P, P, P, P, c_long, P, P, c_float, P, P, c_long],
    "lc_device_cu_count": [c_int, P],
    "lc_stream_create_cumask": [c_int, c_int, c_int, c_int, P],
    "lc_stream_destroy": [P],
}

F16_ENTRY_POINTS = ("lc_gemm_nt", "lc_gemm_nt_ws", "lc_gemm_nt_rows", "lc_gemm_tn", "lc_gemm_tn_ws",
                    "lc_gemm_set_tile", "lc_gemm_set_streamk",
                    "lc_layernorm_fwd", "lc_layernorm_bwd", "lc_attn_fwd", "lc_attn_bwd",
                    "lc_attn_bwd_set_form", "lc_attn_row_fwd", "lc_attn_row_bwd",
                    "lc_attn_bwd_live_row",
                    "lc_adapter_fwd_rows", "lc_adapter_ln_fwd_rows",
                    "lc_cast_bf16", "lc_merge_weight", "lc_cast_weights_bf16",
                    "lc_merge_weights_bf16", "lc_lora_grad", "lc_lora_grad_ws", "lc_adapter_fwd",
                    "lc_adapter_ln_fwd", "lc_adapter_bwd", "lc_adapter_wgrad",
                    "lc_adapter_wgrad_ws", "lc_patchify", "lc_vit_embed_ln")
SIGNATURES.update({n + "_f16": SIGNATURES[n] for n in F16_ENTRY_POINTS})
SIGNATURES.update({n + "_x16": SIGNATURES[n] for n in (
    "lc_layernorm_fwd", "lc_layernorm_bwd", "lc_vit_embed_ln", "lc_adapter_ln_fwd",
    "lc_adapter_ln_fwd_rows", "lc_layernorm_fwd_fp8", "lc_layernorm_bwd_fp8")})
SIGNATURES["lc_layernorm_bwd_g16"] = SIGNATURES["lc_layernorm_bwd"]
SIGNATURES["lc_adapter_wgrad_ws_unscaled"] = SIGNATURES["lc_adapter_wgrad_ws"] + [P]
SIGNATURES["lc_adapter_wgrad_ws_unscaled_g16"] = SIGNATURES["lc_adapter_wgrad_ws_unscaled"]
SIGNATURES["lc_adapter_bwd_g16"] = SIGNATURES["lc_adapter_bwd"]
SIGNATURES["lc_lora_grad_ws_unscaled"] = SIGNATURES["lc_lora_grad_ws"] + [P]

_lib = None


class LcError(RuntimeError):
    pass


def load(path: str = None):
    global _lib
    if _lib is not None:
        return _lib
    if path is None:
        path = os.environ.get("LCCLIP_LIB") or LIB_PATH
    if not os.path.exists(path):
        raise LcError(f"liblcclip.so not built at {path}; run `python __graft_entry__.py build` "
                      "(there is no CPU fallback)")
    lib = ctypes.CDLL(path)
    ab = path != LIB_PATH
    for name, argtypes in SIGNATURES.items():
        if ab and not hasattr(lib, name):
            continue
        fn = getattr(lib, name)
        fn.argtypes = argtypes
        fn.restype = c_int
    _lib = lib
    return lib


def exported_symbols(path: str = LIB_PATH):
    lib = ctypes.CDLL(path)
    return {n for n in SIGNATURES if hasattr(lib, n)}


def ptr(t):
    if t is None:
        return None
    return c_void_p(t.data_ptr())


def stream_of(t: torch.Tensor):
    if not t.is_cuda:
        raise LcError("lcclip ops require tensors on a HIP device (no CPU fallback)")
    return c_void_p(torch.cuda.current_stream(t.device).cuda_stream)


def call(name, *args):
    rc = getattr(load(), name)(*args)
    if rc != 0:
        kind = {-1: "invalid argument / shape", -2: "kernel launch failed"}.get(rc, "error")
        raise LcError(f"{name} returned {rc} ({kind})")
```

### lifelong-clip_amd/lcclip/engine.py

```python
from __future__ import annotations

import itertools
import os
from collections import namedtuple
from contextlib import nullcontext
from types import SimpleNamespace

import torch

from . import ops
from .ops import BF16, F16, F32, EPI_BF16, EPI_F32, EPI_GELU, EPI_GELU_D, EPI_MUL, EPI_RESID
from .ops import EPI_RESID16
from .ops import EPI_GELU_D_Q8, EPI_MUL_Q8

_seed_counter = itertools.count(1)


def _empty(shape, dtype, dev):
    return None if dtype is None else torch.empty(shape, dtype=dtype, device=dev)


def _rows(t, n):
    return None if t is None else t[:n]

# ... 283 lines not shown

    def _stage_fp8(self):
        for blk, st in zip(self.blocks, self.staged):
            D = blk.attn.in_proj_weight.shape[1]
            if D % 256:
                raise ValueError(f"precision='fp8' needs a width that is a multiple of 256 (got {D}): "
                                 "the fp8 GEMM tiles N in 256-column blocks")
            key = (st.frozen_key, st.peft_key, st.merge_epoch)
            if getattr(st, "q_key", None) == key:
                continue
            attn, mlp = blk.attn, blk.mlp
            if self.variant == "lora":
                src = {"wqkv": (st.wqkv, False), "wqkvT": (st.wqkvT, False)}
            else:
                w = attn.in_proj_weight.detach()
                src = {"wqkv": (w, False), "wqkvT": (w, True)}
            wf, wp = mlp.c_fc.weight.detach(), mlp.c_proj.weight.detach()
            src.update(wfc=(wf, False), wfcT=(wf, True), wpr=(wp, False), wprT=(wp, True))
            st.q = {name: ops.quant_fp8(t, transpose=tr) for name, (t, tr) in src.items()}
            st.q_key = key

    FUSE_Q8 = int(os.environ.get("LCCLIP_FP8_FUSE", "4"))
    FUSE_LN = os.environ.get("LCCLIP_FUSE_LN", "1") != "0"

    def _fused_q8(self, level=1):
        return self.precision == "fp8" and self.FUSE_Q8 >= level

    def _gemm(self, st, name, A, epi, out0, **kw):
        if self.precision == "fp8" and name in self.FP8_WEIGHTS:
            return ops.gemm_nt_fp8(ops.quant_fp8(A), st.q[name], epi, out0, **kw)
        return ops.gemm_nt(A, getattr(st, name), epi, out0, **kw)

    def _stage_lora(self, st, name, A, B, merges):
        r, K = A.shape
        N = B.shape[0]
        old = getattr(st, name, None)
        dev = A.device
        if old is None or old[0].shape[1] != K or old[1].shape[1] != N or old[0].dtype != self.dt:
            old = (torch.zeros((64, K), dtype=self.dt, device=dev),
                   torch.zeros((64, N), dtype=self.dt, device=dev),
                   _empty((N, r), self.dt, dev))
        a_pad, bt_pad, scratch = old
        merges.append((A.detach(), None, None, 0.0, a_pad[:r], None))
        merges.append((B.detach(), None, None, 0.0, scratch, bt_pad[:r]))
        return old

    @staticmethod
    def row_plan(n_blocks, P_of, R_of, stop, keep):
        n_run = n_blocks if stop is None else min(stop, n_blocks)
        plan, carried = [], 0
        for idx in range(n_run):
            P = P_of.get(idx, 0)
            kept = bool(keep and P and idx + 1 < n_run and P_of.get(idx + 1, 0) == P
                        and idx + 1 not in R_of)
            plan.append(_Rows(P, bool(P) and carried == P, kept, R_of.get(idx)))
            carried = P if kept else 0
        return plan

    @staticmethod
    def _rows_in(x, p, idx, n_seq, L, prompts, replace):
        D, Lx = x.shape[1], L + p.P
        if p.R is not None:
            if idx == 0:
                x = x.clone()
            x.view(n_seq, -1, D)[:, p.R[0]:p.R[0] + p.R[1]] = replace[idx][1]
        if p.inherit:
            x.view(n_seq, Lx, D)[:, L:] = prompts[idx]
        elif p.P:
            xe = _empty((n_seq * Lx, D), x.dtype, x.device)
            v = xe.view(n_seq, Lx, D)
            v[:, :L] = x.view(n_seq, L, D)
            v[:, L:] = prompts[idx]
            x = xe
        return x

    @staticmethod
    def _rows_out(x_out, p, n_seq, L):
        if not p.P or p.keep:
            return x_out
        D = x_out.shape[1]
        return x_out.view(n_seq, L + p.P, D)[:, :L].reshape(n_seq * L, D)

    def forward(self, x, n_seq: int, L: int, save: bool, training: bool = False, prompts=None,
                stop=None, replace=None, first_ln1=None, last_ln=None, last_rows=False):
        self.stage()
        D = x.shape[1]
        xdt = x.dtype
        dev = x.device
        P_of = {int(i): int(t.shape[1]) for i, t in (prompts or {}).items()}
        plan = self.row_plan(len(self.blocks), P_of, {i: (r0, pr.shape[-2]) for i, (r0, pr) in (
            replace or {}).items()}, stop, self.PROMPT_KEEP)
        Mmax = n_seq * (L + max(P_of.values(), default=0))
        c = SimpleNamespace(n_seq=n_seq, L=L, save=save, training=training, plan=plan,
                            e_resid=EPI_RESID16 if xdt == F16 else EPI_RESID)
        c.tmp_h = _empty((Mmax, D), self.dt, dev)
        c.q_g = ops.Fp8Mat(Mmax, 4 * D, dev) if self._fused_q8() else None
        c.q_h = ops.Fp8Mat(Mmax, D, dev) if self._fused_q8(2) else None
        c.tmp_g = _empty((Mmax, 4 * D), self.dt, dev) if c.q_g is None else None
        c.tmp_pre = None if save else _empty((Mmax, 4 * D), self.dt, dev)
        saved = [] if save else None
        c.fuse_ln = self._fuse_ln(D)
        if xdt != F32 and not (self.variant == "vanilla" or (
                c.q_g is None and c.q_h is None and not prompts and not replace and stop is None
                and ((c.fuse_ln and last_ln is not None) or self.variant == "lora"))):
            raise ValueError("a half residual stream runs the fused adapter tower (with its "
                             "closing LayerNorm fused: last_ln) or the LoRA tower, bf16, without "
                             "prompt rows, or the frozen (prompt) tower")
        if last_rows and not (self.rows_ok() and not prompts and not replace and stop is None):
            raise ValueError("last_rows: the bf16 adapter stack without prompt rows")
        c.last_ln = last_ln if (last_ln is not None
                                and self.last_ln_fused(D, prompts, stop)) else None
        ln1 = first_ln1 if plan and plan[0].plain else None
        for idx, p in enumerate(plan):
            s = SavedLayer(p, rows=last_rows and idx == len(self.blocks) - 1)
            x = self._rows_in(x, p, idx, n_seq, L, prompts, replace)
            ln2_done = self._fwd_attn(c, idx, s, x, ln1)
            x_out, ln1 = self._fwd_mlp(c, idx, s, ln2_done)
            if save:
                saved.append(s)
            x = self._rows_out(x_out, p, n_seq, L)
        return x, saved

    def _fuse_ln(self, D):
        return (self.variant == "adapter" and not self._fused_q8(2) and D in (512, 768)
                and self.FUSE_LN)

    def last_ln_fused(self, D, prompts=None, stop=None):
        last = len(self.blocks) - 1
        return (self._fuse_ln(D) and stop is None and last >= 0 and not any(
            int(i) == last and t.shape[1] for i, t in (prompts or {}).items()))

    def _fwd_attn(self, c, idx, s, x, ln1):
        blk, st = self.blocks[idx], self.staged[idx]
        n_seq, H, dev, xdt, D = c.n_seq, self.n_head, x.device, x.dtype, x.shape[1]
        Lx = c.L + s.P
        Mx = n_seq * Lx
        th = c.tmp_h[:Mx]
        mean1 = _empty((Mx,), F32, dev)
        rstd1 = _empty((Mx,), F32, dev)
        h1 = _empty((Mx, D), self.dt, dev) if (c.save and self.variant == "lora") else th
        qkv = _empty((Mx, 3 * D), self.dt, dev)
        if c.q_h is not None:
            qa = ops.layernorm_fwd_fp8(x, blk.ln_1.weight, blk.ln_1.bias, c.q_h.narrow(Mx),
                                       mean1, rstd1, y=None if h1 is th else h1)
            ops.gemm_nt_fp8(qa, st.q["wqkv"], EPI_BF16, qkv, bias=blk.attn.in_proj_bias)
        else:
            if ln1 is not None:
                h1, mean1, rstd1 = ln1
            else:
                ops.layernorm_fwd(x, blk.ln_1.weight, blk.ln_1.bias, h1, mean1, rstd1)
            self._gemm(st, "wqkv", h1, EPI_BF16, qkv, bias=blk.attn.in_proj_bias)
        Mr, xr, rid = Mx, x, None
        if s.rows:
            Mr, rid = n_seq, (Lx, 0)
            xr = _empty((Mr, D), xdt, dev)
            xr.copy_(x.view(n_seq, Lx, D)[:, 0])
            th = c.tmp_h[:Mr]
            O = _empty((Mr, D), self.dt, dev)
            lse = _empty((n_seq * H,), F32, dev)
            ops.attn_row_fwd(qkv, O, lse, n_seq, Lx, H, 0, self.causal)
        else:
            O = _empty((Mx, D), self.dt, dev)
            lse = _empty((n_seq * H, Lx), F32, dev)
            ops.attn_fwd(qkv, O, lse, n_seq, Lx, H, self.causal)
        x_mid = _empty((Mr, D), xdt, dev)
        ln2_done = False
        if self.variant == "adapter":
            ad = blk.adaptmlp
            s.keep = 1.0 - ad.dropout if (c.training and ad.dropout > 0) else 1.0
            seed1 = next(_seed_counter) * 0x9E3779B1
            s.z1 = _empty((Mr, D), self.dt, dev)
            ops.gemm_nt(O, st.wo, EPI_BF16, s.z1, bias=blk.attn.out_proj.bias)
            s.hd1 = _empty((Mr, ad.down_size), self.dt, dev)
            s.mean2 = _empty((Mr,), F32, dev)
            s.rstd2 = _empty((Mr,), F32, dev)
            if c.fuse_ln and c.q_g is None:
                ops.adapter_ln_fwd(s.z1, st.wd, ad.down_proj.bias, st.wu, ad.up_proj.bias,
                                   ad.scale, s.keep, seed1, xr, x_mid, s.hd1, blk.ln_2.weight,
                                   blk.ln_2.bias, th, s.mean2, s.rstd2, seed_dev=self.seed_dev,
                                   rows=rid)
                ln2_done = True
            else:
                ops.adapter_fwd(s.z1, st.wd, ad.down_proj.bias, st.wu, ad.up_proj.bias, ad.scale,
                                s.keep, seed1, xr, x_mid, s.hd1, seed_dev=self.seed_dev, rows=rid)
        else:
            ops.gemm_nt(O, st.wo, c.e_resid, x_mid, bias=blk.attn.out_proj.bias, aux=x)
            s.mean2 = _empty((Mx,), F32, dev)
            s.rstd2 = _empty((Mx,), F32, dev)
        s.x_in, s.mean1, s.rstd1, s.qkv, s.O, s.lse, s.x_mid = x, mean1, rstd1, qkv, O, lse, x_mid
        if self.variant == "lora":
            s.h1 = h1
        return ln2_done

    def _fwd_mlp(self, c, idx, s, ln2_done):
        blk, st = self.blocks[idx], self.staged[idx]
        x_mid, n_seq, save = s.x_mid, c.n_seq, c.save
        dev, xdt, D = x_mid.device, x_mid.dtype, x_mid.shape[1]
        Lx = c.L + s.P
        Mx = n_seq * Lx
        Mr, rid = (n_seq, (Lx, 0)) if s.rows else (Mx, None)
        th = c.tmp_h[:Mr]
        pre = _empty((Mr, 4 * D), self.dt, dev) if save else c.tmp_pre[:Mr]
        if c.q_g is not None:
            if c.q_h is not None:
                qa = ops.layernorm_fwd_fp8(x_mid, blk.ln_2.weight, blk.ln_2.bias,
                                           c.q_h.narrow(Mx), s.mean2, s.rstd2)
            else:
                ops.layernorm_fwd(x_mid, blk.ln_2.weight, blk.ln_2.bias, th, s.mean2, s.rstd2)
                qa = ops.quant_fp8(th)
            g_in = ops.gemm_nt_fp8(qa, st.q["wfc"], EPI_GELU_D_Q8, pre,
                                   bias=blk.mlp.c_fc.bias, q_out=c.q_g.narrow(Mx))
            wpr = lambda epi, out0, **kw: ops.gemm_nt_fp8(g_in, st.q["wpr"], epi, out0, **kw)
        else:
            if not ln2_done:
                ops.layernorm_fwd(x_mid, blk.ln_2.weight, blk.ln_2.bias, th, s.mean2, s.rstd2)
            self._gemm(st, "wfc", th, EPI_GELU_D if save else EPI_GELU, pre,
                       bias=blk.mlp.c_fc.bias, out1=c.tmp_g[:Mr])
            wpr = lambda epi, out0, **kw: (
                self._gemm_rows(st, "wpr", c.tmp_g, epi, out0, n_seq, Lx, **kw) if s.rows
                else self._gemm(st, "wpr", c.tmp_g[:Mr], epi, out0, **kw))
        s.gd = pre
        x_out = _empty((Mr, D), xdt, dev)
        if self.variant != "adapter":
            wpr(c.e_resid, x_out, bias=blk.mlp.c_proj.bias, aux=x_mid)
            return x_out, None
        ad = blk.adaptmlp
        seed2 = next(_seed_counter) * 0x9E3779B1
        s.z2 = _empty((Mr, D), self.dt, dev)
        wpr(EPI_BF16, s.z2, bias=blk.mlp.c_proj.bias)
        s.hd2 = _empty((Mr, ad.down_size), self.dt, dev)
        nxt, ln1 = idx + 1, None
        if c.fuse_ln and nxt < len(c.plan) and not s.P and c.plan[nxt].plain:
            nb = self.blocks[nxt]
            ln1 = (th, _empty((Mx,), F32, dev), _empty((Mx,), F32, dev))
            ops.adapter_ln_fwd(s.z2, st.wd, ad.down_proj.bias, st.wu, ad.up_proj.bias,
                               ad.scale, s.keep, seed2, x_mid, x_out, s.hd2,
                               nb.ln_1.weight, nb.ln_1.bias, *ln1, seed_dev=self.seed_dev)
        elif c.last_ln is not None and nxt == len(self.blocks):
            ll = c.last_ln
            ops.adapter_ln_fwd(s.z2, st.wd, ad.down_proj.bias, st.wu, ad.up_proj.bias,
                               ad.scale, s.keep, seed2, x_mid, x_out, s.hd2,
                               ll["w"], ll["b"], ll["y"], ll["mean"], ll["rstd"],
                               seed_dev=self.seed_dev, rows=rid)
        else:
            ops.adapter_fwd(s.z2, st.wd, ad.down_proj.bias, st.wu, ad.up_proj.bias, ad.scale,
                            s.keep, seed2, x_mid, x_out, s.hd2, seed_dev=self.seed_dev,
                            rows=rid)
        return x_out, ln1


    def backward(self, saved, dx, dxb, grads, n_seq: int, L: int, on_layer=None,
                 grad_stream=None, need_dx: bool = True, prompt_grads=None,
                 keep_input: bool = False, gscale=None, last_rows=None):
        M, D = dx.shape
        gdt = dx.dtype
        if gdt != F32 and (gscale is None or prompt_grads is not None
                           or any(s.P or s.R is not None for s in saved)):
            raise ValueError("a half residual gradient needs its gscale and no prompt rows")
        c = _Backward(grad_stream, gscale, grads, on_layer)
        c.n_seq, c.L = n_seq, L
        c.nocopy = nocopy = gdt != F32 and self.half_grad_direct()
        cdt = None if nocopy else self.dt
        dev = dx.device
        Mmax = n_seq * (L + max((s.P for s in saved), default=0))
        c.q_da = ops.Fp8Mat(Mmax, 4 * D, dev) if self._fused_q8() else None
        fuse_attn = self._fused_q8(3) and self.variant != "lora" and Mmax // n_seq <= 224
        c.q_dqkv = ops.Fp8Mat(Mmax, 3 * D, dev) if fuse_attn else None
        c.da = _empty((Mmax, 4 * D), self.dt, dev) if c.q_da is None else None
        c.dh = _empty((Mmax, D), self.dt, dev)
        c.dO = _empty((Mmax, D), self.dt, dev)
        c.dqkv = _empty((Mmax, 3 * D), self.dt, dev)
        c.dz = _empty((Mmax, D), self.dt, dev) if self.variant == "adapter" else None
        c.dx_mid = _empty((Mmax, D), gdt, dev)
        c.dx_midb = _empty((Mmax, D), cdt, dev)
        bufs = _GradBufs(dx, None if nocopy else dxb, n_seq, L, Mmax, cdt, keep_input,
                         torch.cuda.current_stream(dev))
        c.fuse_ln_q = self._fused_q8(4) and self.variant != "adapter" and D % 256 == 0
        ev = None
        for li in range(len(self.blocks) - 1, -1, -1):
            s = saved[li]
            if ev is not None:
                bufs.main.wait_event(ev)
            Mx = n_seq * (L + s.P)
            if s.P and not s.pkeep:
                bufs.expand(s.P)
            gx, gxb = bufs.current(Mx)
            if bool(s.rows) != (last_rows is not None and li == len(self.blocks) - 1):
                raise ValueError("last_rows: the forward's compact last block and its gradient")
            if s.rows:
                gx, gxb = last_rows
            ox, oxb = bufs.output(s.P)
            self._bwd_mlp(c, li, s, gx, gxb, bufs.pop_q(Mx))
            more = self._bwd_attn(c, li, s, ox, oxb, bufs, first=li == 0 and not need_dx)
            ev = c.layer_done(li)
            if not more:
                break
            bufs.take_replaced(li, s.R, prompt_grads)
            bufs.advance(li, s.P, s.inherit, ev, prompt_grads)
        c.join()
        if not need_dx:
            return None, None
        return bufs.result()

    def _bwd_mlp(self, c, li, s, gx, gxb, qdy):
        blk, st = self.blocks[li], self.staged[li]
        n_seq, Lx = c.n_seq, c.L + s.P
        Mx = n_seq * Lx
        Mr = n_seq if s.rows else Mx
        if self.variant == "adapter":
            dY = self._adapter_bwd(c, blk, st, gx if c.nocopy else gxb, s.hd2, s.z2, s.keep,
                                   c.dz[:Mr], pad=(n_seq, Lx) if s.rows else None)
        else:
            dY = gxb
        if c.q_da is not None:
            if qdy is None:
                qdy = ops.quant_fp8(dY)
            q = ops.gemm_nt_fp8(qdy, st.q["wprT"], EPI_MUL_Q8, None, aux=s.gd,
                                q_out=c.q_da.narrow(Mx))
            ops.gemm_nt_fp8(q, st.q["wfcT"], EPI_BF16, c.dh[:Mx])
        else:
            self._gemm(st, "wprT", dY, EPI_MUL, c.da[:Mr], aux=s.gd)
            if s.rows:
                self._gemm_rows(st, "wfcT", c.da, EPI_BF16, c.dh[:Mr], n_seq, Lx, scratch=c.dh)
            else:
                self._gemm(st, "wfcT", c.da[:Mr], EPI_BF16, c.dh[:Mr])
        ops.layernorm_bwd(c.dh[:Mr], s.x_mid, s.mean2, s.rstd2, blk.ln_2.weight,
                          c.dx_mid[:Mr], _rows(c.dx_midb, Mr), dres=gx)

    def _bwd_attn(self, c, li, s, ox, oxb, bufs, first):
        blk, st, attn = self.blocks[li], self.staged[li], self.blocks[li].attn
        n_seq, H, Lx = c.n_seq, self.n_head, c.L + s.P
        Mx = n_seq * Lx
        Mr = n_seq if s.rows else Mx
        dh, dO, dqkv, dx_mid = c.dh, c.dO, c.dqkv, c.dx_mid
        if self.variant == "adapter":
            dY = self._adapter_bwd(c, blk, st, dx_mid[:Mr] if c.nocopy else c.dx_midb[:Mr],
                                   s.hd1, s.z1, s.keep, None if first else c.dz[:Mr],
                                   pad=(n_seq, Lx) if s.rows else None)
        else:
            dY = c.dx_midb[:Mx]
        if first and self.variant != "lora":
            return False
        ops.gemm_nt(dY, st.woT, EPI_BF16, dO[:Mr])
        if self.variant == "lora":
            self._lora_grad(c, dY, s.O, attn.out_proj.lora_A, attn.out_proj.lora_B,
                            attn.scaling, st.lora_out)
        if s.rows:
            qd = self._attn_bwd_rows(s, dO[:Mr], dqkv[:Mx], n_seq, Lx, c.da, dh)
        elif c.q_dqkv is not None and not first:
            qd = ops.attn_bwd_fp8(s.qkv, s.O, dO[:Mx], s.lse, c.q_dqkv.narrow(Mx), n_seq,
                                  Lx, H, self.causal)
        else:
            qd = None
            ops.attn_bwd(s.qkv, s.O, dO[:Mx], s.lse, dqkv[:Mx], n_seq, Lx, H, self.causal)
        if self.variant == "lora":
            self._lora_grad(c, dqkv[:Mx], s.h1, attn.in_proj_weight_lora_A,
                            attn.in_proj_weight_lora_B, attn.scaling, st.lora_in)
        if first:
            return False
        if qd is not None:
            ops.gemm_nt_fp8(qd, st.q["wqkvT"], EPI_BF16, dh[:Mx])
        else:
            self._gemm(st, "wqkvT", dqkv[:Mx], EPI_BF16, dh[:Mx])
        dres1 = dx_mid[:Mx]
        if s.rows:
            dres1 = self._spread(dx_mid[:Mr], n_seq, Lx, dst=bufs.incoming(Mx), fill=None)
        if c.fuse_ln_q and s.R is None and not s.P:
            bufs.set_q(ops.layernorm_bwd_fp8(dh[:Mx], s.x_in, s.mean1, s.rstd1, blk.ln_1.weight,
                                             ox, oxb, bufs.q_mat(Mx), dres=dx_mid[:Mx]))
        else:
            bufs.set_q(None)
            ops.layernorm_bwd(dh[:Mx], s.x_in, s.mean1, s.rstd1, blk.ln_1.weight, ox, oxb,
                              dres=dres1)
        return True

    def _adapter_bwd(self, c, blk, st, gout, h, z, keep, dz, pad=None):
        ad = blk.adaptmlp
        M = gout.shape[0]
        dpre = _empty((M, ad.down_size), self.dt, gout.device)
        ops.adapter_bwd(gout, h, st.wuT, st.wdT, ad.scale, keep, dpre, dz)
        with c.side():
            if c.gs is not None:
                dpre.record_stream(c.gs)
            if pad is not None:
                gout, h, z, dpre = self._wgrad_rows(*pad, gout, h, z, dpre)
            ops.adapter_wgrad(gout, h, z, dpre, ad.scale, *(c.grad(p) for p in (
                ad.up_proj.weight, ad.up_proj.bias, ad.down_proj.weight, ad.down_proj.bias)),
                gscale=c.gscale)
        return dz

    ROWS_EXACT = os.environ.get("LCCLIP_ROWS_EXACT", "1") != "0"
    ROW_BWD = os.environ.get("LCCLIP_ROW_BWD", "0") == "1"

    def rows_ok(self):
        return self.variant == "adapter" and self.precision == "bf16"

    @staticmethod
    def _spread(src, n, L, dst=None, fill=0):
        if dst is None:
            dst = torch.empty((n * L, src.shape[1]), dtype=src.dtype, device=src.device)
        elif _same_storage(src, dst):
            src = src.clone()
        if fill is not None:
            dst.zero_() if fill == 0 else dst.fill_(fill)
        dst.view(n, L, -1)[:, 0] = src
        return dst

    @staticmethod
    def _gather(full, n, L, out):
        live = full.view(n, L, -1)[:, 0]
        out.copy_(live.clone() if _same_storage(full, out) else live)

    def _gemm_rows(self, st, name, buf, epi, out, n_seq, L, scratch=None, **kw):
        A, Mx = buf[:n_seq], n_seq * L
        if self.ROW_BWD:
            self._gemm(st, name, A, epi, out, **kw)
        elif not (self.ROWS_EXACT and not set(kw) - {"bias"} and ops.gemm_nt_rows(
                A, getattr(st, name), epi, out, Mx, L, 0, **kw)):
            full = out.new_empty((Mx, out.shape[1])) if scratch is None else scratch[:Mx]
            self._gemm(st, name, self._spread(A, n_seq, L, dst=buf[:Mx]), epi, full, **kw)
            self._gather(full, n_seq, L, out)

    def _attn_bwd_rows(self, s, dO, dqkv, n_seq, L, da, dh):
        H, Mx = self.n_head, n_seq * L
        args = (s.qkv, s.O, dO, s.lse, dqkv, n_seq, L, H, 0, self.causal)
        if self.ROW_BWD:
            ops.attn_row_bwd(*args)
        elif not (self.ROWS_EXACT and ops.attn_bwd_live_row(*args)):
            Of = self._spread(s.O, n_seq, L, dst=dh[:Mx])
            dOf = self._spread(dO, n_seq, L, dst=da.view(-1)[:Mx * dO.shape[1]].view(Mx, -1))
            lsef = self._spread(s.lse.view(-1, 1), n_seq * H, L, fill=1e30).view(-1, L)
            ops.attn_bwd(s.qkv, Of, dOf, lsef, dqkv, n_seq, L, H, self.causal)

    def _wgrad_rows(self, n_seq, L, *operands):
        return operands if self.ROW_BWD else tuple(self._spread(t, n_seq, L) for t in operands)

    HALF_GRAD_DIRECT = os.environ.get("LCCLIP_HALF_GRAD_DIRECT", "1") != "0"

    def half_grad_direct(self):
        return self.variant == "adapter" and self.HALF_GRAD_DIRECT

    PROMPT_KEEP = os.environ.get("LCCLIP_PROMPT_KEEP", "1") != "0"
    MERGE_BATCH = os.environ.get("LCCLIP_MERGE_BATCH", "1") != "0"
    LORA_1P = os.environ.get("LCCLIP_LORA_1P", "1") != "0"

    def _lora_1p(self, r, K, N):
        return self.LORA_1P and r <= 4 and (K, N) in ((768, 2304), (768, 768), (512, 1536),
                                                      (512, 512))

    def lora_half_grad_ok(self):
        for blk in self.blocks:
            a = blk.attn
            for A, B in ((a.in_proj_weight_lora_A, a.in_proj_weight_lora_B),
                         (a.out_proj.lora_A, a.out_proj.lora_B)):
                if not self._lora_1p(A.shape[0], A.shape[1], B.shape[0]):
                    return False
        return True

    def _lora_grad(self, c, dY, X, A, B, scaling, padded):
        a_pad, bt_pad, _ = padded
        M = dY.shape[0]
        r, K = A.shape
        N = B.shape[0]
        gsc = c.gscale
        if self._lora_1p(r, K, N):
            with c.side():
                ops.lora_grad_1p(dY, X, a_pad, bt_pad, r, scaling, c.grad(A), c.grad(B),
                                 gscale=gsc)
            return
        if gsc is not None:
            raise ValueError("a scaled LoRA gradient runs the one-pass kernel only")
        with c.side():
            xa = _empty((M, 64), self.dt, dY.device)
            dyb = _empty((M, 64), self.dt, dY.device)
            if c.gs is not None:
                xa.record_stream(c.gs)
                dyb.record_stream(c.gs)
            ops.gemm_nt(X, a_pad, EPI_BF16, xa)
            ops.gemm_nt(dY, bt_pad, EPI_BF16, dyb)
            ops.gemm_tn(dY, xa, c.grad(B), alpha=scaling)
            ops.gemm_tn(dyb, X, c.grad(A), alpha=scaling)


class ScaledGrads:

    def __init__(self, stack, df, target_exp=10):
        dev = df.device
        self.stack = stack
        self.df = df.contiguous().float().clone()
        self.scale = _empty((1,), F32, dev)
        ops.grad_pow2_normalize(self.df, self.scale, target_exp=target_exp)
        params = stack.trainable_params()
        self.flat = torch.zeros(sum(p.numel() for p in params), dtype=F32, device=dev)
        self.grads, off = {}, 0
        for p in params:
            self.grads[p] = self.flat[off:off + p.numel()].view_as(p)
            off += p.numel()

    def add_to(self, dst):
        params = self.stack.trainable_params()
        if not params:
            return
        views = [dst[p] for p in params]
        first = views[0]
        contiguous = True
        off = 0
        for v in views:
            if not v.is_contiguous() or v.data_ptr() != first.data_ptr() + off * 4:
                contiguous = False
                break
            off += v.numel()
        if contiguous:
            span = torch.as_strided(first, (self.flat.numel(),), (1,))
            ops.add_unscaled(span, self.flat, self.scale)
            return
        for p in params:
            ops.add_unscaled(dst[p], self.grads[p], self.scale)

# ... 195 lines not shown
        else:
            lnp, cls_idx, mean, rstd = self._ln_post(x, n, L, self.stack.dt)
        f = _empty((n, self.projT.shape[0]), F32, x.device)
        ops.gemm_nt(lnp, self.projT, EPI_F32, f)
        ctx = dict(saved=saved, x=x, cls_idx=cls_idx, mean=mean, rstd=rstd, n=n, L=L, rows=rows,
                   prompt_layers=sorted(int(k) for k in (prompts or {}))) if save else None
        return f, ctx

    def backward(self, ctx, df, grads, on_layer=None, grad_stream=None, prompt_grads=None,
                 need_dx=False):
        v = self.visual
        dev = df.device
        n, L = ctx["n"], ctx["L"]
        D = v.width
        dt = self.stack.dt
        var = self.stack.variant
        half = ctx["x"].dtype == F16 and self.HALF_GRAD and (
            var == "adapter" or (var == "lora" and self.stack.lora_half_grad_ok()))
        gsc = sg = None
        out_grads, out_pg = grads, prompt_grads
        if half:
            df = df.contiguous().float().clone()
            if self._gsc is None or self._gsc.device != dev:
                self._gsc = torch.ones(1, dtype=F32, device=dev)
            gsc = self._gsc
            ops.grad_pow2_normalize(df, gsc, target_exp=self.GRAD_EXP)
        elif dt == F16:
            sg = ScaledGrads(self.stack, df, target_exp=self.GRAD_EXP)
            df, grads = sg.df, sg.grads
            prompt_grads = {} if prompt_grads is not None else None
        dfb = _empty(df.shape, dt, dev)
        ops.cast_bf16(df.contiguous(), dfb)
        dln = _empty((n, D), F32, dev)
        ops.gemm_nt(dfb, self.proj, EPI_F32, dln)
        dx, dxb = self._grad_in.get(n * L, D, dev, ctx["cls_idx"], key=(n, L),
                                    dt=dt, gdt=F16 if half else F32)
        if half and self.stack.half_grad_direct():
            dxb = None
        last_rows = None
        if ctx.get("rows"):
            gc = _empty((n, D), dx.dtype, dev)
            gcb = None if dxb is None else _empty((n, D), dt, dev)
            ops.layernorm_bwd(dln, ctx["x"], ctx["mean"], ctx["rstd"], v.ln_post.weight, gc, gcb)
            last_rows = (gc, gcb)
        else:
            ops.layernorm_bwd(dln, ctx["x"], ctx["mean"], ctx["rstd"], v.ln_post.weight, dx, dxb,
                              row_idx=ctx["cls_idx"])
        gx, _ = self.stack.backward(ctx["saved"], dx, dxb, grads, n, L, on_layer, grad_stream,
                                    need_dx=need_dx or 0 in ctx["prompt_layers"],
                                    prompt_grads=prompt_grads, keep_input=True, gscale=gsc,
                                    last_rows=last_rows)
        if sg is not None:
            sg.add_to(out_grads)
            if out_pg is not None:
                for k, t in prompt_grads.items():
                    out_pg[k] = sg.unscaled(t)
            gx = sg.unscaled(gx)
        elif half and gx is not None:
            out = torch.zeros(gx.shape, dtype=F32, device=dev)
            ops.add_unscaled(out.view(-1), gx.float().contiguous().view(-1), gsc)
            gx = out
        return gx if need_dx else None


class TextTower:

    def __init__(self, clip, stack: BlockStack):
        self.clip = clip
        self.stack = stack
        self._key = None
        self._grad_in = RowGrad()

    def _stage(self):
        c = self.clip
        key = _key(c.text_projection) + (self.stack.dt,)
        if key != self._key:
            P = c.text_projection
            dev = P.device
            self.projT = _empty((P.shape[1], P.shape[0]), self.stack.dt, dev)
            self.proj = _empty(tuple(P.shape), self.stack.dt, dev)
            ops.merge_weight(P.detach(), None, None, 0.0, self.proj, self.projT)
            self._key = key

    def forward(self, tokens, save: bool, training: bool = False, x0=None, replace=None):
        c = self.clip
        self._stage()
        dev = tokens.device
        tokens = tokens.contiguous().to(torch.int64)
        C, L = tokens.shape
        D = c.transformer.width
        if x0 is None:
            x0 = _empty((C * L, D), F32, dev)
            ops.text_embed(tokens, c.token_embedding.weight, c.positional_embedding, x0)
        x, saved = self.stack.forward(x0, C, L, save, training, replace=replace)
        eot = _empty((C,), torch.int32, dev)
        ops.eot_rows(tokens, eot)
        lnf = _empty((C, D), self.stack.dt, dev)
        mean = _empty((C,), F32, dev)
        rstd = _empty((C,), F32, dev)
        ops.layernorm_fwd(x, c.ln_final.weight, c.ln_final.bias, lnf, mean, rstd, row_idx=eot)
        f = _empty((C, self.projT.shape[0]), F32, dev)
        ops.gemm_nt(lnf, self.projT, EPI_F32, f)
        ctx = dict(saved=saved, x=x, eot=eot, mean=mean, rstd=rstd, C=C, L=L) if save else None
        return f, ctx

    def backward(self, ctx, df, grads, on_layer=None, prompt_grads=None, need_dx=False):
        c = self.clip
        dev = df.device
        C, L = ctx["C"], ctx["L"]
        D = c.transformer.width
        dt = self.stack.dt
        sg = None
        df = df.contiguous()
        out_grads = grads
        if dt == F16:
            sg = ScaledGrads(self.stack, df)
            df, grads = sg.df, sg.grads
        dfb = _empty(df.shape, dt, dev)
        ops.cast_bf16(df, dfb)
        dln = _empty((C, D), F32, dev)
        ops.gemm_nt(dfb, self.proj, EPI_F32, dln)
        dx, dxb = self._grad_in.get(C * L, D, dev, ctx["eot"], dt=dt)
        ops.layernorm_bwd(dln, ctx["x"], ctx["mean"], ctx["rstd"], c.ln_final.weight, dx, dxb,
                          row_idx=ctx["eot"])
        pg = {} if (sg is not None and prompt_grads is not None) else prompt_grads
        gx, _ = self.stack.backward(ctx["saved"], dx, dxb, grads, C, L, on_layer,
                                    need_dx=need_dx, prompt_grads=pg, keep_input=True)
        if sg is not None:
            sg.add_to(out_grads)
            gx = sg.unscaled(gx)
            if prompt_grads is not None:
                for k, v in pg.items():
                    prompt_grads[k] = sg.unscaled(v)
        return gx
```

### lifelong-clip_amd/lcclip/ops.py

```python
from __future__ import annotations

import ctypes

import torch

from ._lib import LcError, call, load, ptr, stream_of

BF16 = torch.bfloat16
F16 = torch.float16
F32 = torch.float32
HALF = (BF16, F16)

EPI_BF16, EPI_F32, EPI_RESID, EPI_GELU, EPI_GELU_BWD, EPI_BF16_F32, EPI_GELU_D, EPI_MUL = range(8)
EPI_RESID16 = 14
EPI_GELU_D_Q8, EPI_MUL_Q8 = 12, 13


def _rowmajor(t, dtype, name):
    if (t.dtype not in HALF) if dtype == HALF else (t.dtype != dtype):
        raise TypeError(f"{name}: expected {dtype}, got {t.dtype}")
    if t.dim() != 2 or t.stride(1) != 1:
        raise ValueError(f"{name}: expected a 2-D row-major view, got shape {tuple(t.shape)} "
                         f"strides {t.stride()}")

# ... 393 lines not shown
def cast_weights(items):
    import ctypes
    for i in range(0, len(items), CAST_MAX):
        chunk = items[i:i + CAST_MAX]
        n = len(chunk)
        for W, out, outT in chunk:
            if W.dtype != F32 or not W.is_contiguous() or out.dtype not in HALF or not out.is_contiguous():
                raise ValueError("cast_weights: W must be contiguous f32, out contiguous bf16 / float16")
            if out.shape != W.shape or (outT is not None and outT.shape != W.shape[::-1]):
                raise ValueError("cast_weights: shape mismatch")
        ws = (ctypes.c_void_p * n)(*[ptr(W) for W, _, _ in chunk])
        Ns = (ctypes.c_int * n)(*[W.shape[0] for W, _, _ in chunk])
        Ks = (ctypes.c_int * n)(*[W.shape[1] for W, _, _ in chunk])
        outs = (ctypes.c_void_p * n)(*[ptr(o) for _, o, _ in chunk])
        outTs = (ctypes.c_void_p * n)(*[ptr(t) for _, _, t in chunk])
        call(_sym16("lc_cast_weights_bf16", *[t for c in chunk for t in c[1:]]),
             stream_of(chunk[0][0]), n, ws, Ns, Ks, outs, outTs)


def merge_weights(items):
    import ctypes
    for i in range(0, len(items), CAST_MAX):
        chunk = items[i:i + CAST_MAX]
        n = len(chunk)
        for W, A, B, _, out, outT in chunk:
            if W.dtype != F32 or not W.is_contiguous() or out.dtype not in HALF or not out.is_contiguous():
                raise ValueError("merge_weights: W must be contiguous f32, out contiguous bf16 / float16")
            if out.shape != W.shape or (outT is not None and (outT.shape != W.shape[::-1]
                                                              or not outT.is_contiguous())):
                raise ValueError("merge_weights: shape mismatch")
            if A is not None:
                r = A.shape[0]
                if (A.dtype != F32 or B.dtype != F32 or not A.is_contiguous() or not B.is_contiguous()
                        or A.shape[1] != W.shape[1] or tuple(B.shape) != (W.shape[0], r) or r > 8):
                    raise ValueError("merge_weights: A [r, K] / B [N, r] f32 contiguous, r <= 8")
        P = ctypes.c_void_p
        ws = (P * n)(*[ptr(c[0]) for c in chunk])
        As = (P * n)(*[ptr(c[1]) for c in chunk])
        Bs = (P * n)(*[ptr(c[2]) for c in chunk])
        rs = (ctypes.c_int * n)(*[0 if c[1] is None else c[1].shape[0] for c in chunk])
        ss = (ctypes.c_float * n)(*[float(c[3]) for c in chunk])
        Ns = (ctypes.c_int * n)(*[c[0].shape[0] for c in chunk])
        Ks = (ctypes.c_int * n)(*[c[0].shape[1] for c in chunk])
        outs = (P * n)(*[ptr(c[4]) for c in chunk])
        outTs = (P * n)(*[ptr(c[5]) for c in chunk])
        call(_sym16("lc_merge_weights_bf16", *[t for c in chunk for t in c[4:]]),
             stream_of(chunk[0][0]), n, ws, As, Bs, rs, ss, Ns, Ks, outs,
             outTs)


def lora_grad(dY, X, A, B, scaling, dA, dB):
    M, N = dY.shape
    K = X.shape[1]
    call(_sym16("lc_lora_grad", dY, X), stream_of(dY), M, N, K, A.shape[0], ptr(dY), dY.stride(0), ptr(X),
         X.stride(0), ptr(A), ptr(B), float(scaling), ptr(dA), ptr(dB))


def lora_grad_1p(dY, X, a_pad, bt_pad, r, scaling, dA, dB, gscale=None):
    _rowmajor(dY, HALF, "dY")
    _rowmajor(X, HALF, "X")
    _rowmajor(a_pad, HALF, "a_pad")
    _rowmajor(bt_pad, HALF, "bt_pad")
    M, N = dY.shape
    K = X.shape[1]
    if X.shape[0] != M or a_pad.shape[1] != K or bt_pad.shape[1] != N or a_pad.shape[0] < 16 \
            or bt_pad.shape[0] < 16 or tuple(dA.shape) != (r, K) or tuple(dB.shape) != (N, r):
        raise ValueError("lora_grad_1p: shape mismatch")
    for t, name in ((dA, "dA"), (dB, "dB")):
        if t.dtype != F32 or not t.is_contiguous() or not t.is_cuda:
            raise ValueError(f"lora_grad_1p: {name} must be a contiguous f32 device tensor")
    ws = splitk_workspace(torch.cuda.current_stream(dY.device))
    name = _sym16("lc_lora_grad_ws", dY, X, a_pad, bt_pad)
    extra = ()
    if gscale is not None:
        if name != "lc_lora_grad_ws" or gscale.dtype != F32 or gscale.numel() != 1 \
                or not gscale.is_cuda:
            raise TypeError("lora_grad_1p: gscale is a device f32 [1] of the bf16 build")
        name, extra = "lc_lora_grad_ws_unscaled", (ptr(gscale),)
    call(name, stream_of(dY), M, N, K, r, ptr(dY), dY.stride(0), ptr(X), X.stride(0),
         ptr(a_pad), a_pad.stride(0), ptr(bt_pad), bt_pad.stride(0), float(scaling), ptr(dA),
         ptr(dB), ptr(ws), ws.numel(), *extra)


def _row_ids(rows):
    mul, add = (int(v) for v in rows)
    if mul < 1 or add < 0:
        raise ValueError("rows: (mul >= 1, add >= 0)")
    return mul, add


def adapter_fwd(z, Wd, bd, Wu, bu, scale, keep, seed, resid, xout, h, seed_dev=None, rows=None):
    M, D = z.shape
    if resid.dtype != F32 or xout.dtype != F32:
        raise TypeError("adapter_fwd: resid and xout must be f32")
    if tuple(resid.shape) != (M, D) or tuple(xout.shape) != (M, D) or resid.stride() != xout.stride() \
            or xout.stride(1) != 1:
        raise ValueError("adapter_fwd: resid and xout must be row-major [M, D] views of one stride")
    name = "lc_adapter_fwd" if rows is None else "lc_adapter_fwd_rows"
    call(_sym16(name, z, Wd, Wu, h), stream_of(z), M, D, ptr(z), z.stride(0), ptr(Wd), ptr(bd), ptr(Wu),
         ptr(bu), float(scale), float(keep), int(seed) & 0xFFFFFFFFFFFFFFFF, ptr(seed_dev),
         ptr(resid), ptr(xout), xout.stride(0), ptr(h), *(() if rows is None else _row_ids(rows)))


def adapter_ln_fwd(z, Wd, bd, Wu, bu, scale, keep, seed, resid, xout, h, gamma, beta, y, mean,
                   rstd, seed_dev=None, rows=None):
    M, D = z.shape
    if y.dtype != z.dtype or tuple(y.shape) != (M, D) or y.stride(1) != 1:
        raise ValueError("adapter_ln_fwd: y must be a [M, D] row-major view of z's 16-bit type")
    if resid.dtype != xout.dtype or tuple(resid.shape) != (M, D) or tuple(xout.shape) != (M, D) \
            or resid.stride() != xout.stride():
        raise ValueError("adapter_ln_fwd: resid and xout must be [M, D] views of one dtype and stride")
    if xout.dtype == F16 and (xout.stride(0) % 8 or xout.data_ptr() % 16 or resid.data_ptr() % 16):
        raise ValueError("adapter_ln_fwd: half xout / resid rows must be 16-B aligned pieces")
    name = "lc_adapter_ln_fwd" if rows is None else "lc_adapter_ln_fwd_rows"
    call(_x16(name, xout, z, Wd, Wu, h, y), stream_of(z), M, D, ptr(z), z.stride(0), ptr(Wd), ptr(bd), ptr(Wu),
         ptr(bu), float(scale), float(keep), int(seed) & 0xFFFFFFFFFFFFFFFF, ptr(seed_dev),
         ptr(resid), ptr(xout), xout.stride(0), ptr(h), ptr(gamma), ptr(beta), ptr(y),
         y.stride(0), ptr(mean), ptr(rstd), *(() if rows is None else _row_ids(rows)))


def _g16(name, gout, *ts):
    if gout.dtype == F16 and any(t is not None and t.dtype == BF16 for t in ts):
        if any(t is not None and t.dtype == F16 for t in ts):
            raise TypeError(f"{name}: a float16 gout takes bf16 partners")
        if gout.stride(-1) != 1 or gout.stride(0) % 8 or gout.data_ptr() % 16:
            raise ValueError(f"{name}: half gout must be row-major, 16-B aligned, row stride % 8")
        return name + "_g16"
    return _sym16(name, gout, *ts)


def adapter_bwd(gout, h, WuT, WdT, scale, keep, dpre, dz):
    M, D = gout.shape
    call(_g16("lc_adapter_bwd", gout, h, WuT, WdT, dpre, dz), stream_of(gout), M, D, ptr(gout),
         gout.stride(0), ptr(h), ptr(WuT), ptr(WdT), float(scale), float(keep), ptr(dpre),
         ptr(dz), dz.stride(0) if dz is not None else D)


def adapter_wgrad(gout, h, z, dpre, scale, dWu, dbu, dWd, dbd, gscale=None):
    M, D = gout.shape
    for t, name in ((gout, "gout"), (z, "z")):
        _rowmajor(t, HALF, name)
    for t, name in ((h, "h"), (dpre, "dpre")):
        if t.dtype not in HALF or not t.is_contiguous() or t.shape != (M, 64):
            raise ValueError(f"{name} must be contiguous 16-bit [M, 64]")
    if z.shape != (M, D) or dWu.shape != (D, 64) or dWd.shape != (64, D):
        raise ValueError("adapter_wgrad shape mismatch")
    for t in (dWu, dWd, dbu, dbd):
        if t is not None and (t.dtype != F32 or not t.is_contiguous()):
            raise ValueError("gradient buffers must be contiguous f32")
    ws = splitk_workspace(torch.cuda.current_stream(gout.device))
    if gscale is not None:
        name = _g16("lc_adapter_wgrad_ws_unscaled", gout, h, z, dpre)
        if (h.dtype != BF16 or z.dtype != BF16 or dpre.dtype != BF16 or gscale.dtype != F32
                or gscale.numel() != 1):
            raise TypeError("adapter_wgrad: gscale takes bf16 partners and an f32 device scalar")
        call(name, stream_of(gout), M, D, ptr(gout), gout.stride(0),
             ptr(h), ptr(z), z.stride(0), ptr(dpre), float(scale), ptr(dWu), ptr(dbu), ptr(dWd),
             ptr(dbd), ptr(ws), ws.numel(), ptr(gscale))
        return
    if gout.dtype != h.dtype:
        raise TypeError("adapter_wgrad: a float16 gout beside bf16 operands needs its gscale")
    call(_sym16("lc_adapter_wgrad_ws", gout, h, z, dpre), stream_of(gout), M, D, ptr(gout), gout.stride(0), ptr(h), ptr(z),
         z.stride(0), ptr(dpre), float(scale), ptr(dWu), ptr(dbu), ptr(dWd), ptr(dbd), ptr(ws),
         ws.numel())


def check_finite(g, flag):
    call("lc_check_finite", stream_of(g), g.numel(), ptr(g), ptr(flag))


def adamw(p, g, m, v, lr, b1, b2, eps, wd, step, skip=None, step_dev=None):
    call("lc_adamw", stream_of(p), p.numel(), ptr(p), ptr(g), ptr(m), ptr(v), float(lr), float(b1),
         float(b2), float(eps), float(wd), int(step), ptr(skip), ptr(step_dev))


def counter_add(ctr, delta=1):
    if ctr.dtype != torch.int64 or not ctr.is_contiguous():
        raise ValueError("counters must be a contiguous int64 tensor")
    call("lc_counter_add", stream_of(ctr), ctr.numel(), ptr(ctr), int(delta))


def adam_step_advance(ctr, skip=None):
    if ctr.dtype != torch.int64 or ctr.numel() != 1:
        raise ValueError("the AdamW step counter must be one int64 element")
    call("lc_adam_step_advance", stream_of(ctr), ptr(ctr), ptr(skip))


def l2norm_rows(f, out, norms):
    R, E = f.shape
    call("lc_l2norm_rows", stream_of(f), R, E, ptr(f), f.stride(0), ptr(out), ptr(norms))


def clip_head(img_n, txt_n, logit_scale, labels, probs, dlogits, loss):
    B, E = img_n.shape
    C = txt_n.shape[0]
    call("lc_clip_head", stream_of(img_n), B, C, E, ptr(img_n), ptr(txt_n), ptr(logit_scale),
         ptr(labels), ptr(probs), ptr(dlogits), ptr(loss))


def head_logits(img_n, txt_n, logit_scale, logits, probs=None):
    B, E = img_n.shape
    C = txt_n.shape[0]
    call("lc_head_logits", stream_of(img_n), B, C, E, ptr(img_n), ptr(txt_n), ptr(logit_scale),
         ptr(logits), ptr(probs))


def softmax_bwd_rows(probs, dprobs, dlogits):
    B, C = probs.shape
    call("lc_softmax_bwd_rows", stream_of(probs), B, C, ptr(probs), ptr(dprobs), ptr(dlogits))


def head_feat_grad(dlogits, sr, sc, other_n, self_n, norms, logit_scale, dF, dn_ext=None):
    R, E = self_n.shape
    Co = other_n.shape[0]
    call("lc_head_feat_grad", stream_of(dlogits), R, Co, E, ptr(dlogits), sr, sc, ptr(other_n),
         ptr(self_n), ptr(norms), ptr(logit_scale), ptr(dn_ext), ptr(dF))


def grad_pow2_normalize(x, scale, target_exp=10):
    if x.dtype != F32 or not x.is_contiguous() or scale.dtype != F32 or scale.numel() < 1:
        raise ValueError("grad_pow2_normalize: contiguous f32 x and an f32 scale slot")
    call("lc_grad_pow2_normalize", stream_of(x), x.numel(), ptr(x), ptr(scale), int(target_exp))
    return x


def add_unscaled(y, x, scale):
    if (y.dtype != F32 or x.dtype != F32 or not y.is_contiguous() or not x.is_contiguous()
            or y.numel() != x.numel()):
        raise ValueError("add_unscaled: contiguous f32 tensors of one size")
    call("lc_add_unscaled", stream_of(y), y.numel(), ptr(y), ptr(x), ptr(scale))
    return y


I64 = torch.int64


def _f32c(t, name, shape=None):
    if t is None:
        return
    if t.dtype != F32 or not t.is_contiguous():
        raise TypeError(f"{name}: expected a contiguous float32 tensor, got {t.dtype} "
                        f"strides {t.stride()}")
    if shape is not None and tuple(t.shape) != tuple(shape):
        raise ValueError(f"{name}: expected shape {tuple(shape)}, got {tuple(t.shape)}")


def _i64c(t, name, shape=None):
# ... 220 lines not shown
```

### lifelong-clip_amd/lcclip/textcache.py

```python
from __future__ import annotations

import torch


class TokenFeatureCache:
    def __init__(self):
        self._entry = None

    def clear(self):
        self._entry = None

    def get(self, tokens, weights_key):
        e = self._entry
        if e is None:
            return None
        tok, ver, wkey, feats = e
        if wkey != weights_key:
            return None
        if tokens is tok and tokens._version == ver:
            return feats
        if tokens.shape != tok.shape or tokens.device != tok.device or tokens.dtype != tok.dtype:
            return None
        if tokens is tok:
            return None
        if not torch.equal(tokens, tok):
            return None
        self._entry = (tokens, tokens._version, wkey, feats)
        return feats

    def put(self, tokens, weights_key, feats):
        tok = tokens.clone()
        self._entry = (tok, tok._version, weights_key, feats)

    def __bool__(self):
        return self._entry is not None
```

### lifelong-clip_amd/lcclip/trainer.py

```python
from __future__ import annotations

import os
from contextlib import nullcontext

import torch

from . import ops
from .dp import DataParallel, layer_ranges
from .adapter_clip import freeze_backbone
from .ops import F32
from .textcache import TokenFeatureCache


def remap_labels(labels, class_list=None):
    class_list = [] if class_list is None else list(class_list)
    ys = labels.tolist()
    for y in ys:
        if y not in class_list:
            class_list.append(y)
    return torch.tensor([class_list.index(y) for y in ys], dtype=torch.long), class_list


class OnlineTrainer:
    def __init__(self, adapter_clip, lr=5e-4, weight_decay=1e-5, betas=(0.9, 0.999), eps=1e-8,
                 process_group=None, distributed=None, shard_text=True, bucket_layers=4,
                 overlap_text=True, overlap_grads=True, side_cus=None):
        self.wrapper = adapter_clip
        self.clip = adapter_clip.model
        freeze_backbone(self.wrapper)
        self.img = self.clip.visual.tower
        self.txt = self.clip.text_tower
        self.lr, self.wd, self.betas, self.eps = lr, weight_decay, betas, eps
        self.dp = DataParallel(process_group, distributed)
        self.distributed = self.dp.active
        self.shard_text = shard_text and self.distributed
        self.bucket_layers = max(1, int(bucket_layers))
        img_params = self.img.stack.trainable_params()
        params = img_params + self.txt.stack.trainable_params()
        n_img = sum(p.numel() for p in img_params)
        self.img_ranges = layer_ranges(self.img.stack) if img_params else []
        self.txt_range = (n_img, sum(p.numel() for p in params))
        dev = self.clip.logit_scale.device
        n = sum(p.numel() for p in params)
        self.numel = n
        self.flat_p = torch.empty(n, dtype=F32, device=dev)
        self.flat_g = torch.zeros(n, dtype=F32, device=dev)
        self.m = torch.zeros(n, dtype=F32, device=dev)
        self.v = torch.zeros(n, dtype=F32, device=dev)
        self.grads = {}
        off = 0
        with torch.no_grad():
            for p in params:
                k = p.numel()
                self.flat_p[off:off + k].copy_(p.detach().reshape(-1))
                p.data = self.flat_p[off:off + k].view_as(p)
                self.grads[p] = self.flat_g[off:off + k].view_as(p)
                off += k
        self.params = params
        if self.distributed:
            self.replicate()
        self.skip = torch.zeros(1, dtype=torch.int32, device=dev)
        self.adam_step = torch.zeros(1, dtype=torch.int64, device=dev)
        self.step_count = 0
        self.graph = None
        self.overlap_text = bool(overlap_text)
        self.overlap_grads = bool(overlap_grads)
        self._side = None
        self._gstream = None
        env = os.environ.get("LCCLIP_SIDE_CUS")
        if side_cus is None and env:
            side_cus = tuple(int(v) for v in env.split(","))
        self.side_cus = None if side_cus is None else (tuple(side_cus) + (1, 0)[len(side_cus) - 1:])[:3]
        self._masked = []
        self._txt_cache = TokenFeatureCache()
        self.logit_scale = self.clip.logit_scale.detach().reshape(1)

    def replicate(self):
        peft = {id(p) for p in self.params}
        frozen = [p for p in self.wrapper.parameters() if id(p) not in peft]
        bufs = [b for b in self.wrapper.buffers() if b.is_floating_point() or b.dtype == torch.int64]
        self.dp.broadcast_from_root([self.flat_p] + [p.data for p in frozen] + bufs)
        for st in (self.img.stack, self.txt.stack):
            st.invalidate_all()
        self.img._key = None
        self.txt._key = None

    def reset_optimizer(self):
        self.m.zero_()
        self.v.zero_()
        self.step_count = 0
        self.adam_step.zero_()

    def forward_backward(self, images, labels, tokens):
        dev = self.flat_g.device
        self.flat_g.zero_()
        dp = self.dp
        C = tokens.shape[0]
        main = torch.cuda.current_stream(dev)
        side = self._side_stream(dev)
        if side is not None:
            side.wait_stream(main)
        if not labels.is_cuda and labels.numel() and (int(labels.min()) < 0 or int(labels.max()) >= C):
            raise ValueError(f"labels must index the {C} prompts (remap them against the global "
                             "class list, trainer.remap_labels)")
        tok_in = dp.shard_tokens(tokens) if self.shard_text else tokens
        cached = self._cached_text(tokens)
        if cached is None:
            train_t = bool(self.txt.stack.trainable_params())
            with torch.cuda.stream(side) if side is not None else nullcontext():
                f_t, ct = self.txt.forward(tok_in, save=train_t, training=True)
        f_i, ci = self.img.forward(images, save=True, training=True)
        if side is not None:
            main.wait_stream(side)
        if cached is not None:
            f_t, ct = cached, None
        else:
            if self.shard_text:
                f_t = dp.gather_rows(f_t, C).contiguous()
            self._store_text(tokens, f_t)
        B, E = f_i.shape
        img_n = torch.empty_like(f_i)
        txt_n = torch.empty_like(f_t)
        ni = torch.empty(B, dtype=F32, device=dev)
        nt = torch.empty(C, dtype=F32, device=dev)
        ops.l2norm_rows(f_i, img_n, ni)
        ops.l2norm_rows(f_t, txt_n, nt)
        probs = torch.empty(B, C, dtype=F32, device=dev)
        dlog = torch.empty(B, C, dtype=F32, device=dev)
        loss = torch.zeros(1, dtype=F32, device=dev)
        labels = labels.to(dev, torch.int64).contiguous()
        ops.clip_head(img_n, txt_n, self.logit_scale, labels, probs, dlog, loss)
        d_i = torch.empty_like(f_i)
        lo, hi, per = dp.prompt_slice(C) if self.shard_text else (0, C, C)
        d_tp = torch.zeros(per * dp.world if self.shard_text else C, E, dtype=F32, device=dev)
        ops.head_feat_grad(dlog, C, 1, txt_n, img_n, ni, self.logit_scale, d_i)
        train_txt = ct is not None and bool(self.txt.stack.trainable_params())
        if train_txt:
            if side is not None:
                side.wait_stream(main)
            with torch.cuda.stream(side) if side is not None else nullcontext():
                ops.head_feat_grad(dlog, 1, C, img_n, txt_n, nt, self.logit_scale, d_tp[:C])
                w_dt = dp.sum_async(d_tp) if self.shard_text else None
                if w_dt is not None:
                    w_dt.wait()
                self.txt.backward(ct, d_tp[lo:hi].contiguous(), self.grads)
        if self.img.stack.trainable_params():
            gs = self._grad_stream(dev)
            self.img.backward(ci, d_i, self.grads, on_layer=self._img_bucket_hook(gs),
                              grad_stream=gs)
        if side is not None:
            main.wait_stream(side)
        dp.launch_bucket(self.flat_g, *self.txt_range)
        return loss, probs

    def _weights_key(self):
        c = self.clip
        return (tuple(p._version for p in c.transformer.parameters()),
                c.token_embedding.weight._version, c.text_projection._version,
                c.ln_final.weight._version)

    def _cacheable(self):
        return not (self.txt.stack.trainable_params() or torch.cuda.is_current_stream_capturing())

    def _cached_text(self, tokens):
        if not self._cacheable():
            return None
        return self._txt_cache.get(tokens, self._weights_key())

    def _store_text(self, tokens, f_t):
        if self._cacheable():
            self._txt_cache.put(tokens, self._weights_key(), f_t)
        else:
            self._txt_cache.clear()

    def _grad_stream(self, dev):
        if not self.overlap_grads:
            return None
        if self._merge_side_streams():
            side = self._side_stream(dev)
            if side is not None:
                return side
        if self._gstream is None:
            self._gstream = self._new_stream(dev)
        return self._gstream

    def _new_stream(self, dev):
        if self.side_cus is None:
            return torch.cuda.Stream(device=dev)
        count, stride, first = self.side_cus
        ms = ops.CUMaskedStream(dev, count, stride, first)
        self._masked.append(ms)
        return ms.stream

# ... 112 lines not shown
```

Measured before the change: 10650.

## Run text encoder only over live token rows up to the longest EOT

Computes the live sequence length from the tokens (max EOT position + 1, cached per token tensor) and runs the text tower only on those rows. Adapter forward gets a row map that keeps dropout seeds tied to the original row ids, and the weight-gradient GEMM gets a mapped buffer-load path that reads only live rows. The intent is to skip the padded tail of the 77-token text sequences in the text side-stream work. Costs are a host sync for the argmax on each cache miss, extra index arithmetic in the loads, and new entry points.

```diff
diff --git a/include/lc_clip.h b/include/lc_clip.h
--- a/include/lc_clip.h
+++ b/include/lc_clip.h
@@ -239,6 +239,38 @@
                                float* xout, long ldx, void* hout, const float* gamma,
                                const float* beta, void* y, long ldy, float* mean, float* rstd,
                                long row_mul, long row_add);
+int lc_adapter_fwd_rowmap(hipStream_t stream, int M, int D, const void* z, long ldz,
+                          const void* Wd, const float* bd, const void* Wu, const float* bu,
+                          float scale, float keep, unsigned long long seed,
+                          const unsigned long long* seed_dev, const float* resid, float* xout,
+                          long ldx, void* h, long row_live, long row_mul, long row_add);
+int lc_adapter_ln_fwd_rowmap(hipStream_t stream, int M, int D, const void* z, long ldz,
+                             const void* Wd, const float* bd, const void* Wu, const float* bu,
+                             float scale, float keep, unsigned long long seed,
+                             const unsigned long long* seed_dev, const float* resid, float* xout,
+                             long ldx, void* hout, const float* gamma, const float* beta, void* y,
+                             long ldy, float* mean, float* rstd, long row_live, long row_mul,
+                             long row_add);
+int lc_adapter_ln_fwd_rowmap_x16(hipStream_t stream, int M, int D, const void* z, long ldz,
+                                 const void* Wd, const float* bd, const void* Wu, const float* bu,
+                                 float scale, float keep, unsigned long long seed,
+                                 const unsigned long long* seed_dev, const void* resid,
+                                 void* xout, long ldx, void* hout, const float* gamma,
+                                 const float* beta, void* y, long ldy, float* mean, float* rstd,
+                                 long row_live, long row_mul, long row_add);
+int lc_adapter_fwd_rowmap_f16(hipStream_t stream, int M, int D, const void* z, long ldz,
+                              const void* Wd, const float* bd, const void* Wu, const float* bu,
+                              float scale, float keep, unsigned long long seed,
+                              const unsigned long long* seed_dev, const float* resid,
+                              float* xout, long ldx, void* h, long row_live, long row_mul,
+                              long row_add);
+int lc_adapter_ln_fwd_rowmap_f16(hipStream_t stream, int M, int D, const void* z, long ldz,
+                                 const void* Wd, const float* bd, const void* Wu, const float* bu,
+                                 float scale, float keep, unsigned long long seed,
+                                 const unsigned long long* seed_dev, const float* resid,
+                                 float* xout, long ldx, void* hout, const float* gamma,
+                                 const float* beta, void* y, long ldy, float* mean, float* rstd,
+                                 long row_live, long row_mul, long row_add);
 
 int lc_adapter_bwd(hipStream_t stream, int M, int D, const void* gout, long ldg, const void* h,
                    const void* WuT, const void* WdT, float scale, float keep, void* dpre,
@@ -252,6 +284,24 @@
 int lc_adapter_wgrad_ws(hipStream_t stream, int M, int D, const void* gout, long ldg,
                         const void* h, const void* z, long ldz, const void* dpre, float scale,
                         float* dWu, float* dbu, float* dWd, float* dbd, void* ws, long ws_bytes);
+int lc_adapter_wgrad_ws_map(hipStream_t stream, int M, int D, const void* gout, long ldg,
+                            const void* h, const void* z, long ldz, const void* dpre, float scale,
+                            float* dWu, float* dbu, float* dWd, float* dbd, void* ws,
+                            long ws_bytes, int live, int full);
+int lc_adapter_wgrad_ws_map_f16(hipStream_t stream, int M, int D, const void* gout, long ldg,
+                                const void* h, const void* z, long ldz, const void* dpre,
+                                float scale, float* dWu, float* dbu, float* dWd, float* dbd,
+                                void* ws, long ws_bytes, int live, int full);
+int lc_adapter_wgrad_ws_unscaled_map(hipStream_t stream, int M, int D, const void* gout, long ldg,
+                                     const void* h, const void* z, long ldz, const void* dpre,
+                                     float scale, float* dWu, float* dbu, float* dWd, float* dbd,
+                                     void* ws, long ws_bytes, const float* gscale, int live,
+                                     int full);
+int lc_adapter_wgrad_ws_unscaled_g16_map(hipStream_t stream, int M, int D, const void* gout,
+                                         long ldg, const void* h, const void* z, long ldz,
+                                         const void* dpre, float scale, float* dWu, float* dbu,
+                                         float* dWd, float* dbd, void* ws, long ws_bytes,
+                                         const float* gscale, int live, int full);
 
 int lc_check_finite(hipStream_t stream, long n, const float* g, int* flag);
 
diff --git a/lifelong-clip_amd/csrc/gemm.hip b/lifelong-clip_amd/csrc/gemm.hip
--- a/lifelong-clip_amd/csrc/gemm.hip
+++ b/lifelong-clip_amd/csrc/gemm.hip
@@ -263,7 +263,7 @@
           store_bf(rs0, ldo0, m, w);
       } else if constexpr (EPI == EPI_AD_DOWN) {
 #pragma unroll
-        for (int i = 0; i < CPL; ++i) w[i] = fmaxf(v[i], 0.f) * drop_mul(seed, m * row_mul + ep.row_add, n + i, ep.keep);
+        for (int i = 0; i < CPL; ++i) w[i] = fmaxf(v[i], 0.f) * drop_mul(seed, drop_row_id(m, ep.row_live, row_mul, ep.row_add), n + i, ep.keep);
         store_bf(rs0, ldo0, m, w);
       } else if constexpr (EPI == EPI_AD_UP) {
 #pragma unroll
@@ -1329,9 +1329,14 @@
 
 __host__ __device__ inline int tn_pslot(int pw) { return pw * 64 + pw + 64; }
 
-template <int PW>
+LC_DEV uint32_t tn_map_off(int v, int live, int full, long ld, int col) {
+  const int sq = v / full, t = v - sq * full;
+  return t < live ? (uint32_t)(((long)(sq * live + t) * ld + col) * 2) : 0x80000000u;
+}
+
+template <int PW, bool MAP = false>
 __global__ void __launch_bounds__(512, 1)
-gemm_tn_wide_kernel(TnProb p0, TnProb p1) {
+gemm_tn_wide_kernel(TnProb p0, TnProb p1, int live, int full) {
   using Geo = TnGeom<PW>;
   constexpr int STAGES = Geo::STAGES, SLOT = Geo::SLOT, LOADS = Geo::LOADS, TI = Geo::TI;
   constexpr int ROWB = Geo::ROWB, LPRW = ROWB / 16, RPP = 64 / LPRW;
@@ -1358,6 +1363,9 @@
   const bool do_csw = p.cs_w != nullptr && wsv == 0;
   const bool do_css = p.cs_s != nullptr && tile == 0 && wn == 0;
 
+  const int crows = MAP ? (p.M / full) * live : 1;
+  const __amdgpu_buffer_rsrc_t rsW = lc_rsrc(p.W, ((long)(crows - 1) * p.ldw + nw_pad) * 2);
+  const __amdgpu_buffer_rsrc_t rsS = lc_rsrc(p.S, ((long)(crows - 1) * p.lds + 64) * 2);
   auto dma = [&](int s) {
     char* sl = smem + (s % STAGES) * SLOT;
     const int r0 = blk_row(s);
@@ -1370,7 +1378,11 @@
       const int r = min(r0 + lr, p.M - 1);
       int col = tile * PW + c * 8;
       col = col < nw_pad ? col : col - 64;
-      glds16(p.W + (long)r * p.ldw + col, sl + piece * 1024);
+      if constexpr (MAP)
+        __builtin_amdgcn_raw_ptr_buffer_load_lds(rsW, LDS_PTR(sl + piece * 1024), 16,
+                                                 tn_map_off(r, live, full, p.ldw, col), 0, 0, 0);
+      else
+        glds16(p.W + (long)r * p.ldw + col, sl + piece * 1024);
     }
     {
       const int piece = wave;
@@ -1378,7 +1390,11 @@
       const int pc = lane & 7;
       const int c = (((pc >> 1) ^ swz_s(lr)) << 1) | (pc & 1);
       const int r = min(r0 + lr, p.M - 1);
-      glds16(p.S + (long)r * p.lds + c * 8, sl + Geo::WB + piece * 1024);
+      if constexpr (MAP)
+        __builtin_amdgcn_raw_ptr_buffer_load_lds(rsS, LDS_PTR(sl + Geo::WB + piece * 1024), 16,
+                                                 tn_map_off(r, live, full, p.lds, c * 8), 0, 0, 0);
+      else
+        glds16(p.S + (long)r * p.lds + c * 8, sl + Geo::WB + piece * 1024);
     }
   };
 
@@ -1552,10 +1568,19 @@
   p.wgs = p.n_tiles * chunks;
 }
 
-int launch_tn_wide(hipStream_t stream, const TnProb& a, const TnProb& b) {
+int launch_tn_wide(hipStream_t stream, const TnProb& a, const TnProb& b, int live = 0,
+                   int full = 0) {
   const dim3 grid(a.wgs + b.wgs), block(512);
-  if (a.pw == 256) hipLaunchKernelGGL(gemm_tn_wide_kernel<256>, grid, block, 0, stream, a, b);
-  else hipLaunchKernelGGL(gemm_tn_wide_kernel<128>, grid, block, 0, stream, a, b);
+  if (full > 0) {
+    if (a.pw == 256)
+      hipLaunchKernelGGL((gemm_tn_wide_kernel<256, true>), grid, block, 0, stream, a, b, live, full);
+    else
+      hipLaunchKernelGGL((gemm_tn_wide_kernel<128, true>), grid, block, 0, stream, a, b, live, full);
+  } else if (a.pw == 256) {
+    hipLaunchKernelGGL((gemm_tn_wide_kernel<256>), grid, block, 0, stream, a, b, 0, 0);
+  } else {
+    hipLaunchKernelGGL((gemm_tn_wide_kernel<128>), grid, block, 0, stream, a, b, 0, 0);
+  }
   if (a.part) {
     const int outs = a.Nw * 64 + a.Nw + 64 + (b.part ? b.Nw * 64 + b.Nw + 64 : 0);
     hipLaunchKernelGGL(tn_reduce_kernel, dim3((outs + 255) / 256), dim3(256), 0, stream, a, b);
@@ -2086,10 +2111,16 @@
 static int adapter_wgrad(hipStream_t stream, int M, int D, const void* gout, long ldg,
                          const void* h, const void* z, long ldz, const void* dpre, float scale,
                          float* dWu, float* dbu, float* dWd, float* dbd, void* ws, long ws_bytes,
-                         const float* div, int g16 = 0) {
+                         const float* div, int g16 = 0, int live = 0, int full = 0) {
   LC_CHECK_ARG(M > 0 && D > 0 && D % 64 == 0 && ldg % 8 == 0 && ldz % 8 == 0 && ldg >= D &&
                ldz >= D);
   LC_CHECK_ARG(dWu != nullptr && dWd != nullptr);
+  if (full > 0) {
+    LC_CHECK_ARG(live >= 1 && live <= full && M % full == 0);
+    const long crows = (long)(M / full) * live;
+    LC_CHECK_ARG(crows * (ldg > ldz ? ldg : ldz) * 2 < 0x7fffffffL);
+    LC_CHECK_ARG((((uintptr_t)gout | (uintptr_t)h | (uintptr_t)z | (uintptr_t)dpre) & 15) == 0);
+  }
   TnProb up{}, down{};
   up.div = down.div = div;
   up.W = static_cast<const bf16_t*>(gout);
@@ -2134,7 +2165,7 @@
     up.part = reinterpret_cast<float*>(static_cast<char*>(ws) + LC_SPLITK_TICKET_BYTES);
     down.part = up.part + (long)up.wgs * tn_pslot(pw);
   }
-  return launch_tn_wide(stream, up, down);
+  return launch_tn_wide(stream, up, down, live, full);
 }
 
 int lc_adapter_wgrad_ws(hipStream_t stream, int M, int D, const void* gout, long ldg,
@@ -2144,7 +2175,36 @@
                        ws_bytes, nullptr);
 }
 
+int lc_adapter_wgrad_ws_map(hipStream_t stream, int M, int D, const void* gout, long ldg,
+                            const void* h, const void* z, long ldz, const void* dpre, float scale,
+                            float* dWu, float* dbu, float* dWd, float* dbd, void* ws,
+                            long ws_bytes, int live, int full) {
+  LC_CHECK_ARG(full > 0);
+  return adapter_wgrad(stream, M, D, gout, ldg, h, z, ldz, dpre, scale, dWu, dbu, dWd, dbd, ws,
+                       ws_bytes, nullptr, 0, live, full);
+}
+
 #ifndef LC_F16
+int lc_adapter_wgrad_ws_unscaled_map(hipStream_t stream, int M, int D, const void* gout, long ldg,
+                                     const void* h, const void* z, long ldz, const void* dpre,
+                                     float scale, float* dWu, float* dbu, float* dWd, float* dbd,
+                                     void* ws, long ws_bytes, const float* gscale, int live,
+                                     int full) {
+  LC_CHECK_ARG(gscale != nullptr && full > 0);
+  return adapter_wgrad(stream, M, D, gout, ldg, h, z, ldz, dpre, scale, dWu, dbu, dWd, dbd, ws,
+                       ws_bytes, gscale, 0, live, full);
+}
+
+int lc_adapter_wgrad_ws_unscaled_g16_map(hipStream_t stream, int M, int D, const void* gout,
+                                         long ldg, const void* h, const void* z, long ldz,
+                                         const void* dpre, float scale, float* dWu, float* dbu,
+                                         float* dWd, float* dbd, void* ws, long ws_bytes,
+                                         const float* gscale, int live, int full) {
+  LC_CHECK_ARG(gscale != nullptr && full > 0);
+  return adapter_wgrad(stream, M, D, gout, ldg, h, z, ldz, dpre, scale, dWu, dbu, dWd, dbd, ws,
+                       ws_bytes, gscale, 1, live, full);
+}
+
 int lc_adapter_wgrad_ws_unscaled(hipStream_t stream, int M, int D, const void* gout, long ldg,
                                  const void* h, const void* z, long ldz, const void* dpre,
                                  float scale, float* dWu, float* dbu, float* dWd, float* dbd,
diff --git a/lifelong-clip_amd/csrc/lc_common.h b/lifelong-clip_amd/csrc/lc_common.h
--- a/lifelong-clip_amd/csrc/lc_common.h
+++ b/lifelong-clip_amd/csrc/lc_common.h
@@ -136,7 +136,16 @@
   long q_rows;
   int group_m;
   long row_mul, row_add;
+  long row_live;
 };
+
+LC_DEV long drop_row_id(long m, long row_live, long row_mul, long row_add) {
+  if (row_live > 1) {
+    const uint32_t q = (uint32_t)m / (uint32_t)row_live;
+    return (long)q * row_mul + ((uint32_t)m - q * (uint32_t)row_live) + row_add;
+  }
+  return m * row_mul + row_add;
+}
 
 struct Fp8Scales {
   const uint8_t* sa;
diff --git a/lifelong-clip_amd/csrc/lc_f16_names.h b/lifelong-clip_amd/csrc/lc_f16_names.h
--- a/lifelong-clip_amd/csrc/lc_f16_names.h
+++ b/lifelong-clip_amd/csrc/lc_f16_names.h
@@ -38,6 +38,9 @@
 #define lc_adapter_ln_fwd lc_adapter_ln_fwd_f16
 #define lc_adapter_fwd_rows lc_adapter_fwd_rows_f16
 #define lc_adapter_ln_fwd_rows lc_adapter_ln_fwd_rows_f16
+#define lc_adapter_fwd_rowmap lc_adapter_fwd_rowmap_f16
+#define lc_adapter_ln_fwd_rowmap lc_adapter_ln_fwd_rowmap_f16
+#define lc_adapter_wgrad_ws_map lc_adapter_wgrad_ws_map_f16
 #define lc_adapter_bwd_set_form lc_adapter_bwd_set_form_f16
 #define lc_adapter_bwd lc_adapter_bwd_f16
 #define lc_check_finite lc_check_finite_f16
diff --git a/lifelong-clip_amd/csrc/peft.hip b/lifelong-clip_amd/csrc/peft.hip
--- a/lifelong-clip_amd/csrc/peft.hip
+++ b/lifelong-clip_amd/csrc/peft.hip
@@ -792,7 +792,7 @@
                       bf16_t* __restrict__ hout, const float* __restrict__ gamma,
                       const float* __restrict__ beta, bf16_t* __restrict__ y, long ldy,
                       float* __restrict__ mean_out, float* __restrict__ rstd_out, long row_mul,
-                      long row_add) {
+                      long row_add, long row_live) {
   constexpr int XB = (int)sizeof(XT);
   using L = AdLnLay<D, XB>;
   constexpr int KS = L::KS, NU = L::NU;
@@ -919,7 +919,7 @@
       for (int rr = 0; rr < 4; ++rr) {
         const int m = 4 * g + rr;
         float v = pd[rr] + red[m * 64 + j];
-        v = fmaxf(v + prm[3 * D + j], 0.f) * drop_mul(seed, (long)(r0 + m) * row_mul + row_add, j, keep);
+        v = fmaxf(v + prm[3 * D + j], 0.f) * drop_mul(seed, drop_row_id(r0 + m, row_live, row_mul, row_add), j, keep);
         hs[m * 64 + j] = f2bf(v);
       }
     }
@@ -1215,12 +1215,14 @@
                        const float* bd, const void* Wu, const float* bu, float scale, float keep,
                        unsigned long long seed, const unsigned long long* seed_dev,
                        const float* resid, float* xout, long ldx, void* hout, long row_mul,
-                       long row_add) {
+                       long row_add, long row_live = 1) {
   LC_CHECK_ARG(M > 0 && D % 64 == 0 && ldz % 8 == 0 && ldx % 4 == 0);
   LC_CHECK_ARG(keep > 0.f && keep <= 1.f && row_mul >= 1 && row_add >= 0);
+  LC_CHECK_ARG(row_live >= 1 && row_live <= row_mul && row_live < (1L << 31));
   EpiParams ep{z, ldz, scale, keep, (uint64_t)seed, nullptr, seed_dev};
   ep.row_mul = row_mul;
   ep.row_add = row_add;
+  ep.row_live = row_live;
   int rc = lc_gemm_nt_ex({st, EPI_AD_DOWN, M, AD_H, D, z, ldz, Wd, D, bd, 1.0f, hout, AD_H,
                           nullptr, 0, nullptr, 0, ep});
   if (rc) return rc;
@@ -1245,15 +1247,25 @@
                      ldx, hout, row_mul, row_add);
 }
 
+int lc_adapter_fwd_rowmap(hipStream_t st, int M, int D, const void* z, long ldz, const void* Wd,
+                          const float* bd, const void* Wu, const float* bu, float scale,
+                          float keep, unsigned long long seed,
+                          const unsigned long long* seed_dev, const float* resid, float* xout,
+                          long ldx, void* hout, long row_live, long row_mul, long row_add) {
+  return adapter_fwd(st, M, D, z, ldz, Wd, bd, Wu, bu, scale, keep, seed, seed_dev, resid, xout,
+                     ldx, hout, row_mul, row_add, row_live);
+}
+
 static int adapter_ln_fwd(hipStream_t st, int M, int D, const void* z, long ldz, const void* Wd,
                           const float* bd, const void* Wu, const float* bu, float scale,
                           float keep, unsigned long long seed,
                           const unsigned long long* seed_dev, const void* resid, void* xout,
                           long ldx, void* hout, const float* gamma, const float* beta, void* y,
                           long ldy, float* mean, float* rstd, int x16, long row_mul = 1,
-                          long row_add = 0) {
+                          long row_add = 0, long row_live = 1) {
   const int xb = x16 ? 2 : 4;
   LC_CHECK_ARG(row_mul >= 1 && row_add >= 0);
+  LC_CHECK_ARG(row_live >= 1 && row_live <= row_mul && row_live < (1L << 31));
   LC_CHECK_ARG(M > 0 && (D == 768 || D == 512) && ldz % 8 == 0 && ldx % (16 / xb) == 0 &&
                ldy % 8 == 0);
   LC_CHECK_ARG(ldx < (1L << 24) && ldy < (1L << 24));
@@ -1271,7 +1283,8 @@
   hipLaunchKernelGGL((adapter_ln_fwd_kernel<DD, XT>), dim3(grid), dim3(512), 0, st, M,           \
                      (const bf16_t*)z, ldz, (const bf16_t*)Wd, bd, (const bf16_t*)Wu, bu, scale,  \
                      keep, (uint64_t)seed, seed_dev, (const XT*)resid, (XT*)xout, ldx,           \
-                     (bf16_t*)hout, gamma, beta, (bf16_t*)y, ldy, mean, rstd, row_mul, row_add)
+                     (bf16_t*)hout, gamma, beta, (bf16_t*)y, ldy, mean, rstd, row_mul, row_add,   \
+                     row_live)
   if (x16) {
     if (D == 768) LC_ALN(768, _Float16);
     else LC_ALN(512, _Float16);
@@ -1301,6 +1314,17 @@
                            long ldy, float* mean, float* rstd, long row_mul, long row_add) {
   return adapter_ln_fwd(st, M, D, z, ldz, Wd, bd, Wu, bu, scale, keep, seed, seed_dev, resid, xout,
                         ldx, hout, gamma, beta, y, ldy, mean, rstd, 0, row_mul, row_add);
+}
+
+int lc_adapter_ln_fwd_rowmap(hipStream_t st, int M, int D, const void* z, long ldz, const void* Wd,
+                             const float* bd, const void* Wu, const float* bu, float scale,
+                             float keep, unsigned long long seed,
+                             const unsigned long long* seed_dev, const float* resid, float* xout,
+                             long ldx, void* hout, const float* gamma, const float* beta, void* y,
+                             long ldy, float* mean, float* rstd, long row_live, long row_mul,
+                             long row_add) {
+  return adapter_ln_fwd(st, M, D, z, ldz, Wd, bd, Wu, bu, scale, keep, seed, seed_dev, resid, xout,
+                        ldx, hout, gamma, beta, y, ldy, mean, rstd, 0, row_mul, row_add, row_live);
 }
 
 #ifndef LC_F16
@@ -1313,6 +1337,17 @@
                                long row_add) {
   return adapter_ln_fwd(st, M, D, z, ldz, Wd, bd, Wu, bu, scale, keep, seed, seed_dev, resid, xout,
                         ldx, hout, gamma, beta, y, ldy, mean, rstd, 1, row_mul, row_add);
+}
+
+int lc_adapter_ln_fwd_rowmap_x16(hipStream_t st, int M, int D, const void* z, long ldz,
+                                 const void* Wd, const float* bd, const void* Wu, const float* bu,
+                                 float scale, float keep, unsigned long long seed,
+                                 const unsigned long long* seed_dev, const void* resid,
+                                 void* xout, long ldx, void* hout, const float* gamma,
+                                 const float* beta, void* y, long ldy, float* mean, float* rstd,
+                                 long row_live, long row_mul, long row_add) {
+  return adapter_ln_fwd(st, M, D, z, ldz, Wd, bd, Wu, bu, scale, keep, seed, seed_dev, resid, xout,
+                        ldx, hout, gamma, beta, y, ldy, mean, rstd, 1, row_mul, row_add, row_live);
 }
 
 int lc_adapter_ln_fwd_x16(hipStream_t st, int M, int D, const void* z, long ldz, const void* Wd,
diff --git a/lifelong-clip_amd/lcclip/_lib.py b/lifelong-clip_amd/lcclip/_lib.py
--- a/lifelong-clip_amd/lcclip/_lib.py
+++ b/lifelong-clip_amd/lcclip/_lib.py
@@ -68,10 +68,17 @@
     "lc_adapter_ln_fwd_rows": [P, c_int, c_int, P, c_long, P, P, P, P, c_float, c_float,
                                c_ulonglong, P, P, P, c_long, P, P, P, P, c_long, P, P, c_long,
                                c_long],
+    "lc_adapter_fwd_rowmap": [P, c_int, c_int, P, c_long, P, P, P, P, c_float, c_float,
+                              c_ulonglong, P, P, P, c_long, P, c_long, c_long, c_long],
+    "lc_adapter_ln_fwd_rowmap": [P, c_int, c_int, P, c_long, P, P, P, P, c_float, c_float,
+                                 c_ulonglong, P, P, P, c_long, P, P, P, P, c_long, P, P, c_long,
+                                 c_long, c_long],
     "lc_adapter_bwd": [P, c_int, c_int, P, c_long, P, P, P, c_float, c_float, P, P, c_long],
     "lc_adapter_wgrad": [P, c_int, c_int, P, c_long, P, P, c_long, P, c_float, P, P, P, P],
     "lc_adapter_wgrad_ws": [P, c_int, c_int, P, c_long, P, P, c_long, P, c_float, P, P, P, P, P,
                             c_long],
+    "lc_adapter_wgrad_ws_map": [P, c_int, c_int, P, c_long, P, P, c_long, P, c_float, P, P, P, P,
+                                P, c_long, c_int, c_int],
     "lc_check_finite": [P, c_long, P, P],
     "lc_adamw": [P, c_long, P, P, P, P, c_float, c_float, c_float, c_float, c_float, c_int, P, P],
     "lc_counter_add": [P, c_int, P, c_long],
@@ -108,6 +115,7 @@
                     "lc_attn_bwd_set_form", "lc_attn_row_fwd", "lc_attn_row_bwd",
                     "lc_attn_bwd_live_row",
                     "lc_adapter_fwd_rows", "lc_adapter_ln_fwd_rows",
+                    "lc_adapter_fwd_rowmap", "lc_adapter_ln_fwd_rowmap", "lc_adapter_wgrad_ws_map",
                     "lc_cast_bf16", "lc_merge_weight", "lc_cast_weights_bf16",
                     "lc_merge_weights_bf16", "lc_lora_grad", "lc_lora_grad_ws", "lc_adapter_fwd",
                     "lc_adapter_ln_fwd", "lc_adapter_bwd", "lc_adapter_wgrad",
@@ -115,10 +123,14 @@
 SIGNATURES.update({n + "_f16": SIGNATURES[n] for n in F16_ENTRY_POINTS})
 SIGNATURES.update({n + "_x16": SIGNATURES[n] for n in (
     "lc_layernorm_fwd", "lc_layernorm_bwd", "lc_vit_embed_ln", "lc_adapter_ln_fwd",
-    "lc_adapter_ln_fwd_rows", "lc_layernorm_fwd_fp8", "lc_layernorm_bwd_fp8")})
+    "lc_adapter_ln_fwd_rows", "lc_adapter_ln_fwd_rowmap", "lc_layernorm_fwd_fp8",
+    "lc_layernorm_bwd_fp8")})
 SIGNATURES["lc_layernorm_bwd_g16"] = SIGNATURES["lc_layernorm_bwd"]
 SIGNATURES["lc_adapter_wgrad_ws_unscaled"] = SIGNATURES["lc_adapter_wgrad_ws"] + [P]
 SIGNATURES["lc_adapter_wgrad_ws_unscaled_g16"] = SIGNATURES["lc_adapter_wgrad_ws_unscaled"]
+SIGNATURES["lc_adapter_wgrad_ws_unscaled_map"] = (
+    SIGNATURES["lc_adapter_wgrad_ws_unscaled"] + [c_int, c_int])
+SIGNATURES["lc_adapter_wgrad_ws_unscaled_g16_map"] = SIGNATURES["lc_adapter_wgrad_ws_unscaled_map"]
 SIGNATURES["lc_adapter_bwd_g16"] = SIGNATURES["lc_adapter_bwd"]
 SIGNATURES["lc_lora_grad_ws_unscaled"] = SIGNATURES["lc_lora_grad_ws"] + [P]
 
diff --git a/lifelong-clip_amd/lcclip/engine.py b/lifelong-clip_amd/lcclip/engine.py
--- a/lifelong-clip_amd/lcclip/engine.py
+++ b/lifelong-clip_amd/lcclip/engine.py
@@ -389,7 +389,8 @@
         return x_out.view(n_seq, L + p.P, D)[:, :L].reshape(n_seq * L, D)
 
     def forward(self, x, n_seq: int, L: int, save: bool, training: bool = False, prompts=None,
-                stop=None, replace=None, first_ln1=None, last_ln=None, last_rows=False):
+                stop=None, replace=None, first_ln1=None, last_ln=None, last_rows=False,
+                live_of=None):
         self.stage()
         D = x.shape[1]
         xdt = x.dtype
@@ -400,6 +401,10 @@
         Mmax = n_seq * (L + max(P_of.values(), default=0))
         c = SimpleNamespace(n_seq=n_seq, L=L, save=save, training=training, plan=plan,
                             e_resid=EPI_RESID16 if xdt == F16 else EPI_RESID)
+        if live_of is not None and not (self.live_ok() and L <= live_of and not prompts
+                                        and not replace and stop is None and not last_rows):
+            raise ValueError("live_of: the causal adapter stack without prompt rows (live_ok)")
+        c.rid = None if live_of is None else (live_of, 0, L)
         c.tmp_h = _empty((Mmax, D), self.dt, dev)
         c.q_g = ops.Fp8Mat(Mmax, 4 * D, dev) if self._fused_q8() else None
         c.q_h = ops.Fp8Mat(Mmax, D, dev) if self._fused_q8(2) else None
@@ -457,7 +462,7 @@
             else:
                 ops.layernorm_fwd(x, blk.ln_1.weight, blk.ln_1.bias, h1, mean1, rstd1)
             self._gemm(st, "wqkv", h1, EPI_BF16, qkv, bias=blk.attn.in_proj_bias)
-        Mr, xr, rid = Mx, x, None
+        Mr, xr, rid = Mx, x, c.rid
         if s.rows:
             Mr, rid = n_seq, (Lx, 0)
             xr = _empty((Mr, D), xdt, dev)
@@ -505,7 +510,7 @@
         dev, xdt, D = x_mid.device, x_mid.dtype, x_mid.shape[1]
         Lx = c.L + s.P
         Mx = n_seq * Lx
-        Mr, rid = (n_seq, (Lx, 0)) if s.rows else (Mx, None)
+        Mr, rid = (n_seq, (Lx, 0)) if s.rows else (Mx, c.rid)
         th = c.tmp_h[:Mr]
         pre = _empty((Mr, 4 * D), self.dt, dev) if save else c.tmp_pre[:Mr]
         if c.q_g is not None:
@@ -542,7 +547,8 @@
             ln1 = (th, _empty((Mx,), F32, dev), _empty((Mx,), F32, dev))
             ops.adapter_ln_fwd(s.z2, st.wd, ad.down_proj.bias, st.wu, ad.up_proj.bias,
                                ad.scale, s.keep, seed2, x_mid, x_out, s.hd2,
-                               nb.ln_1.weight, nb.ln_1.bias, *ln1, seed_dev=self.seed_dev)
+                               nb.ln_1.weight, nb.ln_1.bias, *ln1, seed_dev=self.seed_dev,
+                               rows=rid)
         elif c.last_ln is not None and nxt == len(self.blocks):
             ll = c.last_ln
             ops.adapter_ln_fwd(s.z2, st.wd, ad.down_proj.bias, st.wu, ad.up_proj.bias,
@@ -558,7 +564,7 @@
 
     def backward(self, saved, dx, dxb, grads, n_seq: int, L: int, on_layer=None,
                  grad_stream=None, need_dx: bool = True, prompt_grads=None,
-                 keep_input: bool = False, gscale=None, last_rows=None):
+                 keep_input: bool = False, gscale=None, last_rows=None, live_of=None):
         M, D = dx.shape
         gdt = dx.dtype
         if gdt != F32 and (gscale is None or prompt_grads is not None
@@ -566,6 +572,10 @@
             raise ValueError("a half residual gradient needs its gscale and no prompt rows")
         c = _Backward(grad_stream, gscale, grads, on_layer)
         c.n_seq, c.L = n_seq, L
+        if live_of is not None and not (self.live_ok() and L <= live_of and not any(
+                s.P or s.R is not None or s.rows for s in saved)):
+            raise ValueError("live_of: the causal adapter stack without prompt rows (live_ok)")
+        c.rowmap = None if live_of is None else (L, live_of)
         c.nocopy = nocopy = gdt != F32 and self.half_grad_direct()
         cdt = None if nocopy else self.dt
         dev = dx.device
@@ -689,11 +699,17 @@
         with c.side():
             if c.gs is not None:
                 dpre.record_stream(c.gs)
+            wgrad = lambda *operands, **kw: ops.adapter_wgrad(
+                *operands, ad.scale, *(c.grad(p) for p in (
+                    ad.up_proj.weight, ad.up_proj.bias, ad.down_proj.weight, ad.down_proj.bias)),
+                gscale=c.gscale, **kw)
             if pad is not None:
-                gout, h, z, dpre = self._wgrad_rows(*pad, gout, h, z, dpre)
-            ops.adapter_wgrad(gout, h, z, dpre, ad.scale, *(c.grad(p) for p in (
-                ad.up_proj.weight, ad.up_proj.bias, ad.down_proj.weight, ad.down_proj.bias)),
-                gscale=c.gscale)
+                self._wgrad_rows(wgrad, *pad, gout, h, z, dpre)
+            elif c.rowmap is not None:
+                if not wgrad(gout, h, z, dpre, rowmap=c.rowmap):
+                    raise ops.LcError("the row-mapped adapter weight gradient is missing")
+            else:
+                wgrad(gout, h, z, dpre)
         return dz
 
     ROWS_EXACT = os.environ.get("LCCLIP_ROWS_EXACT", "1") != "0"
@@ -739,8 +755,34 @@
             lsef = self._spread(s.lse.view(-1, 1), n_seq * H, L, fill=1e30).view(-1, L)
             ops.attn_bwd(s.qkv, Of, dOf, lsef, dqkv, n_seq, L, H, self.causal)
 
-    def _wgrad_rows(self, n_seq, L, *operands):
-        return operands if self.ROW_BWD else tuple(self._spread(t, n_seq, L) for t in operands)
+    def _wgrad_rows(self, wgrad, n_seq, L, *operands):
+        if self.ROW_BWD:
+            wgrad(*operands)
+        elif not (self.ROWS_EXACT and wgrad(*operands, rowmap=(1, L))):
+            wgrad(*(self._spread(t, n_seq, L) for t in operands))
+
+    TEXT_LIVE = os.environ.get("LCCLIP_TEXT_LIVE", "1") != "0"
+
+    def live_ok(self):
+        return (self.TEXT_LIVE and self.causal and self.variant == "adapter"
+                and self.precision == "bf16" and ops.rowmap_ok(self.dt)
+                and not torch.cuda.is_current_stream_capturing())
+
+    _whole = {}
+
+    @classmethod
+    def live_gemms_whole(cls, n_seq, L, live_of, D):
+        key = (n_seq, L, live_of, D)
+        if key not in cls._whole:
+            try:
+                cls._whole[key] = all(
+                    ops.gemm_split_plan(n_seq * rows, N, K)[1] == 1
+                    for rows in (L, live_of)
+                    for N, K in ((3 * D, D), (D, D), (4 * D, D), (D, 4 * D), (D, 3 * D),
+                                 (64, D), (D, 64)))
+            except ops.LcError:
+                return False
+        return cls._whole[key]
 
     HALF_GRAD_DIRECT = os.environ.get("LCCLIP_HALF_GRAD_DIRECT", "1") != "0"
 
@@ -1102,17 +1144,23 @@
             ops.merge_weight(P.detach(), None, None, 0.0, self.proj, self.projT)
             self._key = key
 
-    def forward(self, tokens, save: bool, training: bool = False, x0=None, replace=None):
+    def forward(self, tokens, save: bool, training: bool = False, x0=None, replace=None,
+                live_len=None):
         c = self.clip
         self._stage()
         dev = tokens.device
         tokens = tokens.contiguous().to(torch.int64)
         C, L = tokens.shape
         D = c.transformer.width
+        live_of = None
+        if (live_len is not None and live_len < L and x0 is None and replace is None
+                and self.stack.live_ok() and self.stack.live_gemms_whole(C, int(live_len), L, D)):
+            live_of, L = L, int(live_len)
+            tokens = tokens[:, :L].contiguous()
         if x0 is None:
             x0 = _empty((C * L, D), F32, dev)
             ops.text_embed(tokens, c.token_embedding.weight, c.positional_embedding, x0)
-        x, saved = self.stack.forward(x0, C, L, save, training, replace=replace)
+        x, saved = self.stack.forward(x0, C, L, save, training, replace=replace, live_of=live_of)
         eot = _empty((C,), torch.int32, dev)
         ops.eot_rows(tokens, eot)
         lnf = _empty((C, D), self.stack.dt, dev)
@@ -1121,7 +1169,8 @@
         ops.layernorm_fwd(x, c.ln_final.weight, c.ln_final.bias, lnf, mean, rstd, row_idx=eot)
         f = _empty((C, self.projT.shape[0]), F32, dev)
         ops.gemm_nt(lnf, self.projT, EPI_F32, f)
-        ctx = dict(saved=saved, x=x, eot=eot, mean=mean, rstd=rstd, C=C, L=L) if save else None
+        ctx = dict(saved=saved, x=x, eot=eot, mean=mean, rstd=rstd, C=C, L=L,
+                   live_of=live_of) if save else None
         return f, ctx
 
     def backward(self, ctx, df, grads, on_layer=None, prompt_grads=None, need_dx=False):
@@ -1144,8 +1193,14 @@
         ops.layernorm_bwd(dln, ctx["x"], ctx["mean"], ctx["rstd"], c.ln_final.weight, dx, dxb,
                           row_idx=ctx["eot"])
         pg = {} if (sg is not None and prompt_grads is not None) else prompt_grads
+        live_of = ctx.get("live_of")
         gx, _ = self.stack.backward(ctx["saved"], dx, dxb, grads, C, L, on_layer,
-                                    need_dx=need_dx, prompt_grads=pg, keep_input=True)
+                                    need_dx=need_dx, prompt_grads=pg, keep_input=True,
+                                    live_of=live_of)
+        if gx is not None and live_of is not None:
+            full = gx.new_zeros((C, live_of, D))
+            full[:, :L] = gx.view(C, L, D)
+            gx = full.view(C * live_of, D)
         if sg is not None:
             sg.add_to(out_grads)
             gx = sg.unscaled(gx)
diff --git a/lifelong-clip_amd/lcclip/ops.py b/lifelong-clip_amd/lcclip/ops.py
--- a/lifelong-clip_amd/lcclip/ops.py
+++ b/lifelong-clip_amd/lcclip/ops.py
@@ -499,11 +499,26 @@
          ptr(dB), ptr(ws), ws.numel(), *extra)
 
 
+def has_entry(name):
+    fn = getattr(load(), name, None)
+    return fn is not None and fn.argtypes is not None
+
+
 def _row_ids(rows):
-    mul, add = (int(v) for v in rows)
-    if mul < 1 or add < 0:
-        raise ValueError("rows: (mul >= 1, add >= 0)")
-    return mul, add
+    mul, add, *live = (int(v) for v in rows)
+    if mul < 1 or add < 0 or len(live) > 1 or (live and not 1 <= live[0] <= mul):
+        raise ValueError("rows: (mul >= 1, add >= 0[, 1 <= live <= mul])")
+    return (live[0], mul, add) if live else (mul, add)
+
+
+def _rows_name(name, rows):
+    return name if rows is None else name + ("_rows" if len(rows) == 2 else "_rowmap")
+
+
+def rowmap_ok(dtype):
+    sfx = "_f16" if dtype == F16 else ""
+    return all(has_entry(n + sfx) for n in (
+        "lc_adapter_fwd_rowmap", "lc_adapter_ln_fwd_rowmap", "lc_adapter_wgrad_ws_map"))
 
 
 def adapter_fwd(z, Wd, bd, Wu, bu, scale, keep, seed, resid, xout, h, seed_dev=None, rows=None):
@@ -513,7 +528,7 @@
     if tuple(resid.shape) != (M, D) or tuple(xout.shape) != (M, D) or resid.stride() != xout.stride() \
             or xout.stride(1) != 1:
         raise ValueError("adapter_fwd: resid and xout must be row-major [M, D] views of one stride")
-    name = "lc_adapter_fwd" if rows is None else "lc_adapter_fwd_rows"
+    name = _rows_name("lc_adapter_fwd", rows)
     call(_sym16(name, z, Wd, Wu, h), stream_of(z), M, D, ptr(z), z.stride(0), ptr(Wd), ptr(bd), ptr(Wu),
          ptr(bu), float(scale), float(keep), int(seed) & 0xFFFFFFFFFFFFFFFF, ptr(seed_dev),
          ptr(resid), ptr(xout), xout.stride(0), ptr(h), *(() if rows is None else _row_ids(rows)))
@@ -529,7 +544,7 @@
         raise ValueError("adapter_ln_fwd: resid and xout must be [M, D] views of one dtype and stride")
     if xout.dtype == F16 and (xout.stride(0) % 8 or xout.data_ptr() % 16 or resid.data_ptr() % 16):
         raise ValueError("adapter_ln_fwd: half xout / resid rows must be 16-B aligned pieces")
-    name = "lc_adapter_ln_fwd" if rows is None else "lc_adapter_ln_fwd_rows"
+    name = _rows_name("lc_adapter_ln_fwd", rows)
     call(_x16(name, xout, z, Wd, Wu, h, y), stream_of(z), M, D, ptr(z), z.stride(0), ptr(Wd), ptr(bd), ptr(Wu),
          ptr(bu), float(scale), float(keep), int(seed) & 0xFFFFFFFFFFFFFFFF, ptr(seed_dev),
          ptr(resid), ptr(xout), xout.stride(0), ptr(h), ptr(gamma), ptr(beta), ptr(y),
@@ -553,8 +568,14 @@
          ptr(dz), dz.stride(0) if dz is not None else D)
 
 
-def adapter_wgrad(gout, h, z, dpre, scale, dWu, dbu, dWd, dbd, gscale=None):
+def adapter_wgrad(gout, h, z, dpre, scale, dWu, dbu, dWd, dbd, gscale=None, rowmap=None):
     M, D = gout.shape
+    tail = ()
+    if rowmap is not None:
+        live, full = (int(v) for v in rowmap)
+        if not 1 <= live <= full or M % live:
+            raise ValueError("adapter_wgrad rowmap: (1 <= live <= full), live rows per sequence")
+        tail = (live, full)
     for t, name in ((gout, "gout"), (z, "z")):
         _rowmajor(t, HALF, name)
     for t, name in ((h, "h"), (dpre, "dpre")):
@@ -566,20 +587,27 @@
         if t is not None and (t.dtype != F32 or not t.is_contiguous()):
             raise ValueError("gradient buffers must be contiguous f32")
     ws = splitk_workspace(torch.cuda.current_stream(gout.device))
+    Mv = M // tail[0] * tail[1] if tail else M
     if gscale is not None:
-        name = _g16("lc_adapter_wgrad_ws_unscaled", gout, h, z, dpre)
+        name = _g16("lc_adapter_wgrad_ws_unscaled", gout, h, z, dpre) + ("_map" if tail else "")
+        if tail and not has_entry(name):
+            return False
         if (h.dtype != BF16 or z.dtype != BF16 or dpre.dtype != BF16 or gscale.dtype != F32
                 or gscale.numel() != 1):
             raise TypeError("adapter_wgrad: gscale takes bf16 partners and an f32 device scalar")
-        call(name, stream_of(gout), M, D, ptr(gout), gout.stride(0),
+        call(name, stream_of(gout), Mv, D, ptr(gout), gout.stride(0),
              ptr(h), ptr(z), z.stride(0), ptr(dpre), float(scale), ptr(dWu), ptr(dbu), ptr(dWd),
-             ptr(dbd), ptr(ws), ws.numel(), ptr(gscale))
-        return
+             ptr(dbd), ptr(ws), ws.numel(), ptr(gscale), *tail)
+        return True
     if gout.dtype != h.dtype:
         raise TypeError("adapter_wgrad: a float16 gout beside bf16 operands needs its gscale")
-    call(_sym16("lc_adapter_wgrad_ws", gout, h, z, dpre), stream_of(gout), M, D, ptr(gout), gout.stride(0), ptr(h), ptr(z),
+    name = _sym16("lc_adapter_wgrad_ws_map" if tail else "lc_adapter_wgrad_ws", gout, h, z, dpre)
+    if tail and not has_entry(name):
+        return False
+    call(name, stream_of(gout), Mv, D, ptr(gout), gout.stride(0), ptr(h), ptr(z),
          z.stride(0), ptr(dpre), float(scale), ptr(dWu), ptr(dbu), ptr(dWd), ptr(dbd), ptr(ws),
-         ws.numel())
+         ws.numel(), *tail)
+    return True
 
 
 def check_finite(g, flag):
diff --git a/lifelong-clip_amd/lcclip/textcache.py b/lifelong-clip_amd/lcclip/textcache.py
--- a/lifelong-clip_amd/lcclip/textcache.py
+++ b/lifelong-clip_amd/lcclip/textcache.py
@@ -34,3 +34,19 @@
 
     def __bool__(self):
         return self._entry is not None
+
+
+class LiveLength:
+
+    def __init__(self):
+        self._entry = None
+        self.misses = 0
+
+    def get(self, tokens):
+        e = self._entry
+        if e is not None and tokens is e[0] and tokens._version == e[1]:
+            return e[2]
+        self.misses += 1
+        length = int(tokens.argmax(dim=1).max()) + 1
+        self._entry = (tokens, tokens._version, length)
+        return length
diff --git a/lifelong-clip_amd/lcclip/trainer.py b/lifelong-clip_amd/lcclip/trainer.py
--- a/lifelong-clip_amd/lcclip/trainer.py
+++ b/lifelong-clip_amd/lcclip/trainer.py
@@ -9,7 +9,7 @@
 from .dp import DataParallel, layer_ranges
 from .adapter_clip import freeze_backbone
 from .ops import F32
-from .textcache import TokenFeatureCache
+from .textcache import LiveLength, TokenFeatureCache
 
 
 def remap_labels(labels, class_list=None):
@@ -73,6 +73,7 @@
         self.side_cus = None if side_cus is None else (tuple(side_cus) + (1, 0)[len(side_cus) - 1:])[:3]
         self._masked = []
         self._txt_cache = TokenFeatureCache()
+        self._live_len = LiveLength()
         self.logit_scale = self.clip.logit_scale.detach().reshape(1)
 
     def replicate(self):
@@ -108,7 +109,8 @@
         if cached is None:
             train_t = bool(self.txt.stack.trainable_params())
             with torch.cuda.stream(side) if side is not None else nullcontext():
-                f_t, ct = self.txt.forward(tok_in, save=train_t, training=True)
+                live = self._live_len.get(tokens) if self.txt.stack.live_ok() else None
+                f_t, ct = self.txt.forward(tok_in, save=train_t, training=True, live_len=live)
         f_i, ci = self.img.forward(images, save=True, training=True)
         if side is not None:
             main.wait_stream(side)
diff --git a/profiles/text_live/compare.py b/profiles/text_live/compare.py
--- /dev/null
+++ b/profiles/text_live/compare.py
@@ -0,0 +1,39 @@
+import glob
+import itertools
+import json
+import os
+import sys
+
+import numpy as np
+
+out = sys.argv[1]
+for c in (10, 100):
+    legs = {}
+    for leg in ("tree", "parent", "full"):
+        runs = []
+        for log in sorted(glob.glob(f"{out}/c{c}.{leg}.*.log")):
+            line = [ln for ln in open(log) if ln.startswith("{") and '"value"' in ln][-1]
+            r = json.loads(line)
+            d = log[:-4]
+            runs.append((r["ms_per_step"], r["value"], np.load(f"{d}/loss.npy"),
+                         np.load(f"{d}/probs.npy")))
+        legs[leg] = runs
+    print(f"## C = {c}")
+    for leg, runs in legs.items():
+        ms = [r[0] for r in runs]
+        print(f"{leg:7s} ms/step {', '.join(f'{m:.3f}' for m in ms)}  img/s "
+              f"{', '.join(f'{r[1]:.1f}' for r in runs)}  mean {np.mean(ms):.3f} ms = "
+              f"{np.mean([r[1] for r in runs]):.1f} img/s  max-min {max(ms) - min(ms):.3f} ms")
+    t, p = (np.mean([r[0] for r in legs[k]]) for k in ("tree", "parent"))
+    spread = max(max(r[0] for r in legs[k]) - min(r[0] for r in legs[k]) for k in ("tree", "parent"))
+    print(f"tree - parent {t - p:+.3f} ms ({(p / t - 1) * 100:+.2f} % img/s), "
+          f"{abs(t - p) / spread:.1f} x the larger spread ({spread:.3f} ms)")
+    ref = legs["parent"][0][3]
+    for leg, runs in legs.items():
+        same = all(np.array_equal(r[3].view(np.uint32), ref.view(np.uint32)) for r in runs)
+        print(f"probs {leg}: {'bit-identical to' if same else 'DIFFER from'} the parent's first run")
+    own = [abs(float(a[2]) - float(b[2])) for a, b in itertools.combinations(legs["parent"], 2)]
+    print(f"loss: parent runs among themselves {', '.join(f'{v:.2g}' for v in own)}")
+    for leg in ("tree", "full"):
+        d = [abs(float(a[2]) - float(b[2])) for a in legs[leg] for b in legs["parent"]]
+        print(f"loss: {leg} vs parent runs {min(d):.2g} ... {max(d):.2g}")
diff --git a/profiles/text_live/loss_order.py b/profiles/text_live/loss_order.py
--- /dev/null
+++ b/profiles/text_live/loss_order.py
@@ -0,0 +1,22 @@
+import sys
+
+import numpy as np
+import torch
+
+probs = np.load(sys.argv[1] + "/probs.npy").astype(np.float32)
+B, C = probs.shape
+seed = int(sys.argv[2]) if len(sys.argv) > 2 else 1234
+y = torch.randint(0, C, (B,), generator=torch.Generator().manual_seed(seed)).numpy()
+m = probs.max(1, keepdims=True)
+lse = (np.log(np.exp(probs - m).sum(1, dtype=np.float32)) + m[:, 0]).astype(np.float32)
+terms = ((lse - probs[np.arange(B), y]) * np.float32(1.0 / B)).astype(np.float32)
+rng = np.random.default_rng(0)
+sums = []
+for _ in range(2000):
+    acc = np.float32(0)
+    for t in terms[rng.permutation(B)]:
+        acc = np.float32(acc + t)
+    sums.append(float(acc))
+print(f"dumped loss {np.load(sys.argv[1] + '/loss.npy').item():.9f}; 2000 random orders: "
+      f"min {min(sums):.9f} max {max(sums):.9f} (range {max(sums) - min(sums):.3g}, "
+      f"std {np.std(sums):.3g})")
```

Result: no change. 10700 (median of 6 runs) (+0.4%).
